# TurakhiaLab/TWILIGHT

Hardware: AMD Instinct MI355X
Metric: DP band cells/s, TALCO-XDrop progressive profile-profile alignment (bit-exact vs reference CPU path) (higher is better)
Workload: dtype f32

## Files before the change

### include/twl_align.h

```cpp
#ifndef TWL_ALIGN_H
#define TWL_ALIGN_H

#include <stdint.h>

#ifdef __cplusplus
extern "C" {
#endif

#define TWL_MAX_MATRIX 21
#define TWL_MAX_MARKER 1024

enum twl_status {
    TWL_OK = 0,
    TWL_ERR_NOT_INITIALIZED = -1,
    TWL_ERR_BAD_ARGUMENT = -2,
    TWL_ERR_HIP = -3,
    TWL_ERR_UNSUPPORTED = -4
};

typedef struct twl_params {
    int32_t P;
    float   matrix[TWL_MAX_MATRIX * TWL_MAX_MATRIX];
    float   gap_open;
    float   gap_extend;
    float   gap_boundary;
    float   gap_char;
    int32_t xdrop;
    int32_t flen;
    int32_t marker;
} twl_params;

typedef struct twl_stats {
    uint64_t band_cells;
    uint64_t nominal_cells;
    double   kernel_ms;
    double   pack_ms;
    double   total_ms;
    int32_t  n_launches;
    int32_t  n_relaunched;
    int32_t  window;
    int32_t  grid;
    int32_t  matrix_mode;
    int32_t  speculative;
    int32_t  mt_tiles_predicted;
    int32_t  mt_tiles_inline;
    int32_t  mt_scouts_failed;
    int32_t  reserved;
    char     kernel[160];
} twl_stats;

int  twl_init(const int *device_ids, int n_devices);
void twl_shutdown(void);
const char *twl_last_error(void);
const char *twl_version(void);

int twl_align_batch(const twl_params *p, int32_t n_pairs, int32_t seq_len,
                    const float *freq, const float *gap_open, const float *gap_extend,
                    const int32_t *len, const int32_t *num,
                    int8_t *aln_out, int32_t *aln_len_out, int16_t *err_out);

int twl_align_batch_device(int device, void *stream, const twl_params *p, int32_t n_pairs, int32_t seq_len,
                           const float *d_freq, const float *d_gap_open, const float *d_gap_extend,
                           const int32_t *d_len, const int32_t *d_num,
                           int8_t *d_aln_out, int32_t *d_aln_len_out, int16_t *d_err_out);

void *twl_host_alloc(uint64_t bytes);
void  twl_host_free(void *p);

int twl_copy_to_device(int device, void *dst_dev, const void *src, uint64_t bytes);
int twl_copy_from_device(int device, void *dst, const void *src_dev, uint64_t bytes);
int twl_copy_rows_from_device(int device, void *dst, uint64_t dst_pitch, const void *src_dev, uint64_t src_pitch, uint64_t width, uint64_t rows);

int twl_get_stats(int device, twl_stats *out);

int twl_get_pair_cells(int device, uint64_t *cells_out, int32_t n);

int twl_column_scores(const twl_params *p, int32_t seq_len, const float *freq, const int32_t *len, const int32_t *num, float *out);

int twl_dp_column_scores(const twl_params *p, int32_t seq_len, const float *freq, const float *gap_open, const float *gap_extend,
                         const int32_t *len, const int32_t *num, float *out);

#define TWL_MT_REC_WORDS 12
typedef struct twl_mt_dims {
    int32_t n_run, slots, sp_pitch, segcap;
    int32_t n_scout, n_tile, rounds;
    int32_t lead2, marg, anchors;
    int32_t thr, small_tiles, marker;
    int32_t reserved[3];
} twl_mt_dims;
int twl_mt_tables(int device, twl_mt_dims *dims, int32_t *order, int32_t *anchor, int32_t *spath, int32_t *chain, int32_t *rec, int8_t *seg, int32_t *front);

#define TWL_COMM_ID_BYTES 128
int twl_comm_unique_id(void *id128);
int twl_comm_init(int device, int rank, int world, const void *id128);
int twl_comm_all_gather(int device, const void *d_send, void *d_recv, int64_t bytes_per_rank);
int twl_comm_all_gather_host(int device, const void *send, void *recv, int64_t bytes_per_rank);
int twl_comm_destroy(int device);

enum twl_knob { TWL_KNOB_MT_PERTURB = 1, TWL_KNOB_MT_MAX_PAIRS = 2, TWL_KNOB_MT_MIN_MARKER = 3, TWL_KNOB_MT_LEAD = 4, TWL_KNOB_MT_MARGIN = 5,
                TWL_KNOB_MT_ROUNDS = 6, TWL_KNOB_MT_THR_JOBS = 7, TWL_KNOB_FAIL_ROW_ALLOCS = 8,
                TWL_KNOB_PROT_MODE = 9, TWL_KNOB_ASSUME_ONEHOT_QUERY = 10, TWL_KNOB_MT_TAIL_PCT = 11, TWL_KNOB_MT_WIDE = 12, TWL_KNOB_NO_SPEC = 13, TWL_KNOB_SCOUT_XDROP_PCT = 14, TWL_KNOB_THR_SMALL = 15, TWL_KNOB_FORCE_GLOBAL = 16, TWL_KNOB_LEAF_STEP = 17, TWL_KNOB_POISON_TB = 18, TWL_KNOB_MT_ANCHOR = 19, TWL_KNOB_MT_LEAD2 = 20, TWL_KNOB_PROT_CORRIDOR = 21 };
int twl_set_knob(int key, int value);
int twl_plan_describe(const twl_params *p, int32_t n_pairs, const int32_t *len, int32_t num_cu, int32_t qry_onehot, int32_t wide_streak, char *out, int32_t cap);

#ifdef __cplusplus
}
#endif
#endif
```

### twilight_amd/api.py

```python
from __future__ import annotations

import ctypes as C
import os

import numpy as np

_HERE = os.path.dirname(os.path.abspath(__file__))
LIB_PATH = os.environ.get("TWL_LIB") or os.path.join(_HERE, "libtwl_align.so")
TWL_MAX_MATRIX = 21

_lib = None


class TwlError(RuntimeError):
    pass


class TwlParams(C.Structure):
    _fields_ = [("P", C.c_int32), ("matrix", C.c_float * (TWL_MAX_MATRIX * TWL_MAX_MATRIX)), ("gap_open", C.c_float),
                ("gap_extend", C.c_float), ("gap_boundary", C.c_float), ("gap_char", C.c_float), ("xdrop", C.c_int32),
                ("flen", C.c_int32), ("marker", C.c_int32)]


class TwlStats(C.Structure):
# ... 44 lines not shown
        lib.twl_shutdown.restype = None
        lib.twl_set_knob.restype = C.c_int
        lib.twl_mt_tables.restype = C.c_int
        _lib = lib
    return _lib


def _check(rc):
    if rc != 0:
        raise TwlError(f"libtwl_align error {rc}: {load_library().twl_last_error().decode()}")


def make_params(matrix, *, gap_open=-50.0, gap_extend=-5.0, gap_boundary=None, gap_char=None, xdrop=None, flen=4096,
                marker=1024) -> TwlParams:
    m = np.asarray(matrix, dtype=np.float32)
    n = m.shape[0]
    p = TwlParams()
    p.P = n + 1
    flat = np.zeros(TWL_MAX_MATRIX * TWL_MAX_MATRIX, dtype=np.float32)
    flat[: n * n] = m.reshape(-1)
    p.matrix[:] = flat.tolist()
    p.gap_open = gap_open
    p.gap_extend = gap_extend
    p.gap_boundary = gap_extend if gap_boundary is None else gap_boundary
    p.gap_char = gap_extend if gap_char is None else gap_char
    p.xdrop = int(1000 * -gap_extend) if xdrop is None else int(xdrop)
    p.flen = flen
    p.marker = marker
    return p


def init(device_ids=None):
    lib = load_library()
    if device_ids is None:
        _check(lib.twl_init(None, 0))
    else:
        arr = (C.c_int * len(device_ids))(*device_ids)
        _check(lib.twl_init(arr, len(device_ids)))


def shutdown():
    load_library().twl_shutdown()


def _ptr(a, ty):
    return a.ctypes.data_as(C.POINTER(ty))


def align_batch(params: TwlParams, batch):
    lib = load_library()
    n, sl = batch.n_pairs, batch.seq_len
    freq = np.ascontiguousarray(batch.freq, dtype=np.float32)
    go = np.ascontiguousarray(batch.gap_open, dtype=np.float32)
    ge = np.ascontiguousarray(batch.gap_extend, dtype=np.float32)
    ln = np.ascontiguousarray(batch.len, dtype=np.int32)
    nm = np.ascontiguousarray(batch.num, dtype=np.int32)
    aln = np.zeros((n, 2 * sl), dtype=np.int8)
    aln_len = np.zeros(n, dtype=np.int32)
    err = np.zeros(n, dtype=np.int16)
    _check(lib.twl_align_batch(C.byref(params), C.c_int32(n), C.c_int32(sl), _ptr(freq, C.c_float), _ptr(go, C.c_float),
                               _ptr(ge, C.c_float), _ptr(ln, C.c_int32), _ptr(nm, C.c_int32), _ptr(aln, C.c_int8),
                               _ptr(aln_len, C.c_int32), _ptr(err, C.c_int16)))
    return aln, aln_len, err


def align_batch_device(params: TwlParams, n_pairs, seq_len, d_freq, d_gop, d_gex, d_len, d_num, d_aln, d_aln_len, d_err,
                       device=0, stream=None):
    lib = load_library()
    vp = C.c_void_p
    _check(lib.twl_align_batch_device(C.c_int(device), vp(stream or 0), C.byref(params), C.c_int32(n_pairs), C.c_int32(seq_len),
                                      vp(d_freq), vp(d_gop), vp(d_gex), vp(d_len), vp(d_num), vp(d_aln), vp(d_aln_len),
                                      vp(d_err)))


KNOB_MT_PERTURB, KNOB_MT_MAX_PAIRS, KNOB_MT_MIN_MARKER, KNOB_MT_LEAD, KNOB_MT_MARGIN, KNOB_MT_ROUNDS, KNOB_MT_THR_JOBS, KNOB_FAIL_ROW_ALLOCS = 1, 2, 3, 4, 5, 6, 7, 8
KNOB_PROT_MODE, KNOB_ASSUME_ONEHOT_QUERY, KNOB_MT_TAIL_PCT, KNOB_MT_WIDE, KNOB_NO_SPEC, KNOB_SCOUT_XDROP_PCT = 9, 10, 11, 12, 13, 14
KNOB_THR_SMALL = 15
KNOB_FORCE_GLOBAL = 16
KNOB_LEAF_STEP = 17
KNOB_POISON_TB = 18
KNOB_MT_ANCHOR = 19
KNOB_PROT_CORRIDOR = 21
KNOB_MT_LEAD2 = 20
PROT_MODES = {"auto": 0, "dense": 1, "sparse": 2, "presim": 3, "r1": 4, "lean_sparse": 5, "lean_presim": 6}


def set_knob(key: int, value: int):
    _check(load_library().twl_set_knob(C.c_int(key), C.c_int(value)))


def plan_describe(params, lens, num_cu=256, qry_onehot=False, wide_streak=0, small_state=0) -> str:
    wide_streak = int(wide_streak) + (100000 * (32 + int(small_state)) if small_state else 0)
    lens = np.ascontiguousarray(lens, dtype=np.int32)
    buf = C.create_string_buffer(256)
    _check(load_library().twl_plan_describe(C.byref(params), C.c_int32(lens.shape[0]), _ptr(lens, C.c_int32), C.c_int32(num_cu), C.c_int32(int(qry_onehot)), C.c_int32(wide_streak), buf, C.c_int32(256)))
    return buf.value.decode()


def version() -> str:
    return load_library().twl_version().decode()


def get_stats(device=0) -> TwlStats:
    st = TwlStats()
    _check(load_library().twl_get_stats(C.c_int(device), C.byref(st)))
    return st


def get_pair_cells(n, device=0):
    out = np.zeros(n, dtype=np.uint64)
    _check(load_library().twl_get_pair_cells(C.c_int(device), _ptr(out, C.c_uint64), C.c_int32(n)))
    return out


def column_scores(params: TwlParams, ref: np.ndarray, qry: np.ndarray, ref_num: int, qry_num: int) -> np.ndarray:
    ref = np.ascontiguousarray(ref, dtype=np.float32)
    qry = np.ascontiguousarray(qry, dtype=np.float32)
    R, Q, P = ref.shape[0], qry.shape[0], ref.shape[1]
    sl = max(R, Q)
    freq = np.zeros((2, sl, P), dtype=np.float32)
    freq[0, :R] = ref
    freq[1, :Q] = qry
    ln = np.array([R, Q], dtype=np.int32)
    nm = np.array([ref_num, qry_num], dtype=np.int32)
    out = np.zeros((Q, R), dtype=np.float32)
    _check(load_library().twl_column_scores(C.byref(params), C.c_int32(sl), _ptr(freq, C.c_float), _ptr(ln, C.c_int32), _ptr(nm, C.c_int32), _ptr(out, C.c_float)))
    return out


def dp_column_scores(params: TwlParams, batch, pair: int = 0) -> np.ndarray:
    sl = batch.seq_len
    freq = np.ascontiguousarray(batch.freq[pair], dtype=np.float32)
    gop = np.ascontiguousarray(batch.gap_open[pair], dtype=np.float32)
    gex = np.ascontiguousarray(batch.gap_extend[pair], dtype=np.float32)
    ln = np.ascontiguousarray(batch.len[pair], dtype=np.int32)
    nm = np.ascontiguousarray(batch.num[pair], dtype=np.int32)
    out = np.zeros((int(ln[1]), int(ln[0])), dtype=np.float32)
    _check(load_library().twl_dp_column_scores(C.byref(params), C.c_int32(sl), _ptr(freq, C.c_float), _ptr(gop, C.c_float), _ptr(gex, C.c_float),
                                               _ptr(ln, C.c_int32), _ptr(nm, C.c_int32), _ptr(out, C.c_float)))
    return out


def mt_tables(device=0) -> dict:
    lib = load_library()
    dm = TwlMtDims()
    _check(lib.twl_mt_tables(C.c_int(device), C.byref(dm), None, None, None, None, None, None, None))
    n, s = dm.n_run, dm.slots
    order = np.zeros(n, dtype=np.int32)
    anchor = np.zeros((n, s), dtype=np.int32) if dm.anchors else None
    spath = np.zeros((n, dm.sp_pitch), dtype=np.int32)
    chain = np.zeros((n, s, 2), dtype=np.int32)
    rec = np.zeros((n, s, MT_REC_WORDS), dtype=np.int32)
    seg = np.zeros((n, s, dm.segcap), dtype=np.int8)
    front = np.zeros((n, 8), dtype=np.int32)
    _check(lib.twl_mt_tables(C.c_int(device), C.byref(dm), _ptr(order, C.c_int32), _ptr(anchor, C.c_int32) if dm.anchors else None, _ptr(spath, C.c_int32),
                             _ptr(chain, C.c_int32), _ptr(rec, C.c_int32), _ptr(seg, C.c_int8), _ptr(front, C.c_int32)))
    assert (dm.n_run, dm.slots) == (n, s), "another level ran between the two reads"
    dims = {k: int(getattr(dm, k)) for k, _ in TwlMtDims._fields_ if k != "reserved"}
    return {"dims": dims, "order": order, "anchor": anchor, "spath": spath, "chain": chain, "rec": rec, "seg": seg, "front": front}
```

### twilight_amd/csrc/talco_kernel.hip.h

```cpp
#pragma once
#include <hip/hip_runtime.h>
#include <stdint.h>
#include "talco_exit.hip.h"

namespace twl {

constexpr int kIB = -2;
constexpr int kDB = -3;
constexpr int kMaxMarker = 1024;
constexpr int kErrOverflow = -1;
constexpr int kErrGuard = -2;

struct KArgs {
    const float *cols;
    const int32_t *len;
    const int32_t *num;
    int8_t *aln;
    int32_t *aln_len;
    int16_t *err;
    unsigned long long *cells;
    uint32_t *tb;
    int32_t *queue;
    const int32_t *items;
    int32_t n_items;
    int32_t seq_len;
    int32_t tb_words;
    int32_t *dbg;
    int32_t n_pairs_total;
    int32_t *hb;
    int32_t step_slack;
    float gap_open, gap_extend, gap_char;
    const uint8_t *gc_zero;
    int32_t xdrop, flen, marker;
    float M[441];
    const float *sim;
    const long long *sim_off;
};

#ifdef TWL_KERNEL_STAMPS
#define TWL_STAMP(var) const unsigned long long var = __builtin_amdgcn_s_memtime()
#else
#define TWL_STAMP(var)
#endif

#ifdef TWL_KERNEL_DEBUG
__device__ __forceinline__ void heartbeat(const KArgs &a, int slot, int v)
{
    if (a.hb && blockIdx.x == 0 && threadIdx.x == 0) __hip_atomic_store(&a.hb[slot], v, __ATOMIC_RELAXED, __HIP_MEMORY_SCOPE_SYSTEM);
}
#else
__device__ __forceinline__ void heartbeat(const KArgs &, int, int) {}
#endif

__device__ __forceinline__ unsigned lds_off(const void *p)
{
    return (unsigned)(uintptr_t)(__attribute__((address_space(3))) const void *)p;
}
__device__ __forceinline__ void lds_max_i32(int *p, int v) { asm volatile("ds_max_i32 %0, %1" ::"v"(lds_off(p)), "v"(v) : "memory"); }
__device__ __forceinline__ void lds_min_i32(int *p, int v) { asm volatile("ds_min_i32 %0, %1" ::"v"(lds_off(p)), "v"(v) : "memory"); }
__device__ __forceinline__ void lds_or_b32(int *p, int v) { asm volatile("ds_or_b32 %0, %1" ::"v"(lds_off(p)), "v"(v) : "memory"); }

__device__ __forceinline__ float dpp_shr1_f(float from_prev_wave, float src)
{
    return __int_as_float(__builtin_amdgcn_update_dpp(__float_as_int(from_prev_wave), __float_as_int(src), 0x138, 0xf, 0xf, false));
}
__device__ __forceinline__ int dpp_shr1_i(int from_prev_wave, int src)
{
    return __builtin_amdgcn_update_dpp(from_prev_wave, src, 0x138, 0xf, 0xf, false);
}

__device__ __forceinline__ float wave_max_f32(float x)
{
#define TWL_DPP_MAX(ctrl, rmask, bmask) \
    x = fmaxf(x, __int_as_float(__builtin_amdgcn_update_dpp(__float_as_int(x), __float_as_int(x), ctrl, rmask, bmask, false)))
    TWL_DPP_MAX(0x111, 0xf, 0xf);
    TWL_DPP_MAX(0x112, 0xf, 0xf);
    TWL_DPP_MAX(0x114, 0xf, 0xf);
    TWL_DPP_MAX(0x118, 0xf, 0xf);
    TWL_DPP_MAX(0x142, 0xa, 0xf);
    TWL_DPP_MAX(0x143, 0xc, 0xf);
#undef TWL_DPP_MAX
    return __int_as_float(__builtin_amdgcn_readlane(__float_as_int(x), 63));
}

__device__ __forceinline__ int f2key(float f)
{
    int b = __float_as_int(f);
    if (b == (int)0x80000000) b = 0;
    return b >= 0 ? b : (b ^ 0x7fffffff);
}
__device__ __forceinline__ float key2f(int k)
{
    return __int_as_float(k >= 0 ? k : (k ^ 0x7fffffff));
}

template <int P, int W, int RPL, bool PRE, bool REFLDS, bool QREG = true>
struct Cfg {
    static_assert(P == 6 || P == 22, "profile width");
    static_assert(!(PRE && P != 6), "precomputed q*M rows exist for P=6 only");
    static constexpr int CW = P + 2;
    static constexpr int F4 = CW / 4;
    static constexpr int NV = W * RPL;
    static constexpr int WINDOW = 64 * NV;
    static constexpr int NB = NV + 2;
    static constexpr int CAP = 64 * NB;
    static constexpr int RING_F4 = REFLDS ? CAP * F4 : F4;
    static constexpr int THREADS = 64 * W;
};

template <int P, int W, int RPL, bool PRE, bool REFLDS, bool QREG = true, int MINW = 1, int MM = 0>
__global__ __launch_bounds__(64 * W, MINW) void talco_kernel(KArgs a)
{
    using C = Cfg<P, W, RPL, PRE, REFLDS, QREG>;
    constexpr int NV = C::NV, WINDOW = C::WINDOW, NB = C::NB, CAP = C::CAP, CW = C::CW, F4 = C::F4;
    constexpr int MS = P - 1;
// ... 707 lines not shown
```

### twilight_amd/csrc/talco_nuc.hip.h

```cpp
#pragma once
#include "talco_kernel.hip.h"

#if defined(TWL_EXP_NOPRIO)
#define TWL_SETPRIO(x) do {} while (0)
#else
#define TWL_SETPRIO(x) __builtin_amdgcn_s_setprio(x)
#endif

namespace twl {

struct NArgs {
    const float *cols;
    const int32_t *len;
    const int32_t *num;
    int8_t *aln;
    int32_t *aln_len;
    int16_t *err;
    unsigned long long *cells;
    uint32_t *tb;
    int32_t *queue;
    const int32_t *items;
    int32_t n_items;
    int32_t seq_len;
    int32_t tb_words;
    int32_t *dbg;
    int32_t n_pairs_total;
    int32_t step_slack;
    float gap_open, gap_extend, gap_char;
    const uint8_t *gc_zero;
    int32_t xdrop, flen, marker;
    float M[25];
    const float *M24;
    const float *sim;
    const long long *sim_off;
    unsigned long long *team;
    float *simdump;
    const int32_t *mt_jobs;
    int32_t *mt_chain;
    int32_t *mt_rec;
    int8_t *mt_seg;
    int32_t *mt_spath;
    unsigned long long *mt_stat;
    int32_t *mt_front;
    int32_t mt_slots, mt_segcap, mt_sp_pitch, mt_lead, mt_marg;
    const int32_t *mt_anchor;
    int32_t mt_lead2;
    int32_t mt_inline;
};

typedef float nuc_f4 __attribute__((ext_vector_type(4)));
typedef float nuc_f2 __attribute__((ext_vector_type(2)));
__device__ __forceinline__ float4 lds_ld128(unsigned addr)
{
    const nuc_f4 v = *reinterpret_cast<const __attribute__((address_space(3))) nuc_f4 *>((const __attribute__((address_space(3))) char *)nullptr + addr);
    return make_float4(v.x, v.y, v.z, v.w);
}
typedef int nuc_i2 __attribute__((ext_vector_type(2)));
typedef int nuc_i4 __attribute__((ext_vector_type(4)));
template <class T>
__device__ __forceinline__ T lds_ld(unsigned addr)
{
    return *reinterpret_cast<const __attribute__((address_space(3))) T *>((const __attribute__((address_space(3))) char *)nullptr + addr);
}
template <class T>
__device__ __forceinline__ void lds_st(unsigned addr, T v)
{
    *reinterpret_cast<__attribute__((address_space(3))) T *>((__attribute__((address_space(3))) char *)nullptr + addr) = v;
}
template <int OFF>
__device__ __forceinline__ void lds_max_u32_off(unsigned addr, unsigned v) { asm volatile("ds_max_u32 %0, %1 offset:%2" ::"v"(addr), "v"(v), "n"(OFF) : "memory"); }
template <int OFF>
__device__ __forceinline__ void lds_max_f32_off(unsigned addr, float v) { asm volatile("ds_max_f32 %0, %1 offset:%2" ::"v"(addr), "v"(v), "n"(OFF) : "memory"); }
#define TWL_LDS_ATOM(NAME)                                                                                                     \
    template <int OFF>                                                                                                         \
    __device__ __forceinline__ void NAME##_off(unsigned addr, int v) { asm volatile(#NAME " %0, %1 offset:%2" ::"v"(addr), "v"(v), "n"(OFF) : "memory"); }
TWL_LDS_ATOM(ds_min_i32)
TWL_LDS_ATOM(ds_max_i32)
TWL_LDS_ATOM(ds_or_b32)
#undef TWL_LDS_ATOM
__device__ __forceinline__ void wg_barrier_lds() { asm volatile("s_waitcnt lgkmcnt(0)\n\ts_barrier" ::: "memory"); }
__device__ __forceinline__ void lds_max_u32(unsigned addr, unsigned v) { asm volatile("ds_max_u32 %0, %1" ::"v"(addr), "v"(v) : "memory"); }
__device__ __forceinline__ void lds_max_f32(unsigned addr, float v) { asm volatile("ds_max_f32 %0, %1" ::"v"(addr), "v"(v) : "memory"); }

__device__ __forceinline__ float fast_div(float n, float d, float r)
{
    const float q0 = n * r;
    const float t0 = __builtin_fmaf(-d, q0, n);
    const float q1 = __builtin_fmaf(t0, r, q0);
    const float t1 = __builtin_fmaf(-d, q1, n);
    return __builtin_fmaf(t1, r, q1);
}
__device__ __forceinline__ float refined_rcp(float d)
{
    const float r0 = __builtin_amdgcn_rcpf(d);
    const float e = __builtin_fmaf(-d, r0, 1.0f);
    return __builtin_fmaf(e, r0, r0);
}
__device__ __forceinline__ bool div_guard_bad(float x)
{
    const float ax = __builtin_fabsf(x);
    return (x != 0.0f) && !(ax >= 9.5367431640625e-07f && ax <= 1073741824.0f);
}

constexpr unsigned kTeamLast = 1u, kTeamErr = 2u;
constexpr int kTeamWords = 16, kTeamGuess = 0, kTeamTruth = 4, kTeamPos = 8, kTeamStat = 12;
__device__ __forceinline__ unsigned long long team_word(unsigned tag, unsigned flags, unsigned hi, unsigned lo)
{
    return ((unsigned long long)(tag & 0xFFFFu) << 48) | ((unsigned long long)(flags & 0xFFFFu) << 32) | ((unsigned long long)(hi & 0xFFFFu) << 16) | (lo & 0xFFFFu);
}
__device__ __forceinline__ unsigned long long team_load(const unsigned long long *p) { return __hip_atomic_load(p, __ATOMIC_RELAXED, __HIP_MEMORY_SCOPE_AGENT); }
__device__ __forceinline__ void team_store(unsigned long long *p, unsigned long long v) { __hip_atomic_store(p, v, __ATOMIC_RELAXED, __HIP_MEMORY_SCOPE_AGENT); }
__device__ __forceinline__ unsigned long long team_wait(const unsigned long long *p, unsigned tag, const unsigned long long *alt = nullptr)
{
    for (int spin = 0; spin < (1 << 21); ++spin) {
        const unsigned long long v = team_load(p);
        if ((unsigned)(v >> 48) == tag) return v;
        if (alt) { const unsigned long long u = team_load(alt); if ((unsigned)(u >> 48) == tag) return u | (1ull << 47); }
        __builtin_amdgcn_s_sleep(16);
    }
    return 0ull;
}
__device__ __forceinline__ unsigned score_key(float f)
{
    const unsigned b = (unsigned)__float_as_int(f);
    return (b & 0x80000000u) ? ~b : (b | 0x80000000u);
}

constexpr int kMtRec = 12;

__global__ void mt_chain_kernel(const int32_t *spath, int sp_pitch, const int32_t *len, const int32_t *items, int n_items, int32_t *chain, int slots,
                                int marker, int perturb, const int32_t *front)
{
    const int it = blockIdx.x * blockDim.x + threadIdx.x;
    if (it >= n_items) return;
// ... 35 lines not shown
    q = min(q, Q - 1);
    r = d0 - q;
    if (r > R - 1) { r = R - 1; q = d0 - r; }
    return !(q > Q - 1 || r < 0);
}
__device__ __forceinline__ bool scout_anchor(const int32_t *an, int slot, int slots, int &o)
{
    const int w = __builtin_amdgcn_readfirstlane(an[slot]);
    if (w >= 0) { o = w - 128; return true; }
    int l = -1, r = -1, ol = 0, orr = 0;
    for (int u = 1; u <= kAnchorNear; ++u) {
        if (l < 0 && slot - u >= 1) { const int v = __builtin_amdgcn_readfirstlane(an[slot - u]); if (v >= 0) { l = slot - u; ol = v - 128; } }
        if (r < 0 && slot + u < slots) { const int v = __builtin_amdgcn_readfirstlane(an[slot + u]); if (v >= 0) { r = slot + u; orr = v - 128; } }
    }
    if (l < 0 || r < 0 || abs(orr - ol) > kAnchorJump * (r - l)) return false;
    o = ol + (orr - ol) * (slot - l) / (r - l);
    return true;
}
__device__ __forceinline__ bool scout_anchored_cell(int d0, int R, int Q, int o, int &r, int &q)
{
    int r0, q0;
    if (!scout_line_cell(d0, R, Q, r0, q0)) return false;
    q = q0 + (o >= 0 ? (o + 1) / 2 : -((-o + 1) / 2));
    r = d0 - q;
    if (q < 0) { q = 0; r = d0; }
    if (r < 0) { r = 0; q = d0; }
    return q < Q && r < R;
}

constexpr int kAnchorShift = 24, kAnchorShifts = 4, kAnchorPad = kAnchorShift * kAnchorShifts;
template <int P>
__global__ __launch_bounds__(256) void mt_anchor_kernel(const float *cols, const int32_t *len, int seq_len, const int32_t *jobs, int n_jobs, int32_t *anchor, int slots, int marker, int lead2)
{
    static_assert(kAnchorOffsets == 256 && 2 * kAnchorHalf + 2 * kAnchorPad == 256, "one thread per offset, one per staged reference letter");
    __shared__ unsigned char s_r[2 * kAnchorHalf + 2 * kAnchorPad], s_q[2 * kAnchorHalf + 2 * kAnchorPad + kAnchorOffsets];
    __shared__ int s_cnt[kAnchorOffsets], s_done;
    const int job = blockIdx.x;
    if (job >= n_jobs) return;
    const int pair = jobs[3 * job], slot = jobs[3 * job + 1], row = jobs[3 * job + 2];
    const int R = len[2 * pair], Q = len[2 * pair + 1];
    const int spLo = (marker - 1) * slot - 1;
    const int d0 = max(spLo - lead2, 0);
    int r0, q0;
    if (spLo > R + Q - 2 || R < 2 || Q < 2 || !scout_line_cell(d0, R, Q, r0, q0)) return;
    auto letter = [&](int side, int col, int n) -> unsigned char {
        if (col < 0 || col >= n) return (unsigned char)(100 + side);
        const float *pf = cols + (((size_t)pair * 2 + side) * (size_t)seq_len + col) * (P + 2);
        int best = 0; float bc = pf[0];
        for (int j = 1; j < P - 2; ++j) if (pf[j] > bc) { bc = pf[j]; best = j; }
        return (bc > 0.0f && bc >= pf[P - 1]) ? (unsigned char)best : (unsigned char)(100 + side);
    };
    const int t = threadIdx.x;
    s_r[t] = letter(0, r0 - kAnchorHalf - kAnchorPad + t, R);
    for (int u = t; u < 2 * kAnchorHalf + 2 * kAnchorPad + kAnchorOffsets; u += 256) s_q[u] = letter(1, q0 - kAnchorHalf - kAnchorPad - kAnchorOffsets / 2 + u, Q);
    if (t == 0) s_done = 0;
    __syncthreads();
    for (int sh = 0; sh <= 2 * kAnchorShifts; ++sh) {
        const int base = kAnchorPad + ((sh == 0) ? 0 : ((sh & 1) ? kAnchorShift * ((sh + 1) / 2) : -kAnchorShift * (sh / 2)));
        int c = 0;
        for (int i = 0; i < 2 * kAnchorHalf; ++i) c += (s_r[base + i] == s_q[base + i + t]) ? 1 : 0;
        s_cnt[t] = c;
        __syncthreads();
        if (t < 64) {
            int key = -1;
            for (int u = t; u < kAnchorOffsets; u += 64) {
                const int o = u - kAnchorOffsets / 2;
                const int rank = (o == 0) ? 0 : (o < 0 ? -2 * o - 1 : 2 * o);
                key = max(key, (s_cnt[u] << 16) | (0xFFFF - rank));
            }
            for (int m = 32; m >= 1; m >>= 1) key = max(key, __shfl_xor(key, m, 64));
            const int rank = 0xFFFF - (key & 0xFFFF);
            const int bo = (rank == 0) ? 0 : ((rank & 1) ? -(rank + 1) / 2 : rank / 2);
            int second = -1;
            for (int u = t; u < kAnchorOffsets; u += 64) if (abs(u - kAnchorOffsets / 2 - bo) > 2) second = max(second, s_cnt[u]);
            for (int m = 32; m >= 1; m >>= 1) second = max(second, __shfl_xor(second, m, 64));
            const int bc = key >> 16;
            if (t == 0 && bc >= kAnchorMinMatches && bc - second >= kAnchorMinGap) { anchor[(size_t)row * slots + slot] = 128 + bo; s_done = 1; }
        }
        __syncthreads();
        if (s_done) break;
    }
}

template <int W, int RPL>
struct NCfg {
    static constexpr int NV = W * RPL;
    static constexpr int WINDOW = 64 * NV;
    static constexpr int NB = NV + 2;
    static constexpr int CAP = 64 * NB;
    static constexpr int THREADS = 64 * W;
};

template <int P, int W, int RPL, int MM, int MINW, bool SPEC = false, bool DUMP = false, int MT = 0, int SP = 0>
__global__ __launch_bounds__(64 * W, MINW) void talco_lean_kernel(NArgs a)
{
    static_assert(SP == 0 || (SP == 1 && P == 6 && !SPEC && !DUMP && MM == 5), "the leaf x leaf step: nucleotide, one-letter query rows");
    static_assert((P == 6 && ((MM >= 0 && MM <= 2) || MM == 5)) || (P == 22 && (MM == 3 || MM == 4)), "profile width / column-score mode");
    static_assert(MT == 0 || (!SPEC && !DUMP), "the tile-parallel kernels are plain ones");
    constexpr bool GUESS = SPEC || MT == 2;
    using C = NCfg<W, RPL>;
    constexpr int NV = C::NV, WINDOW = C::WINDOW, NB = C::NB, CAP = C::CAP;
    constexpr int NQP = (MM == 2 || MM == 1) ? 8 : (MM == 0 ? 10 : (MM == 5 ? 2 : 1));
    constexpr int NQM = (MM == 0) ? 5 : 1;
#if defined(TWL_EXP_QPRE)
    constexpr bool QPRE = !(MM == 2) || TWL_EXP_QPRE;
#else
    constexpr bool QPRE = !((RPL >= 3 || MINW >= 5) && MM == 2);
#endif
    constexpr int F4 = (P + 2) / 4;
    constexpr bool SPARSE = (MM == 3), PRESIM = (MM == 4);
    constexpr int RP = PRESIM ? 1 : F4;
    constexpr int QN = PRESIM ? 1 : P;

    __shared__ float4 s_ring[RP * CAP];
    __shared__ uint32_t s_rmask[SPARSE ? CAP : 1];
    __shared__ float4 s_M4[SPARSE ? 21 * 6 : 1];
    struct ParBuf {
        int cd[WINDOW + 4];
        int4 exch[NV];
        unsigned red[4];
        int conv[4];
        int edge[2 * NV];
        int4 trash[64];
    };
    __shared__ ParBuf s_par[2];
    __shared__ int s_misc[8];
    __shared__ int8_t s_rev[2 * kMaxMarker + 16];
    __shared__ unsigned long long s_team[4];
    constexpr unsigned O_CD = (unsigned)offsetof(ParBuf, cd), O_EXCH = (unsigned)offsetof(ParBuf, exch), O_RED = (unsigned)offsetof(ParBuf, red),
                       O_CONV = (unsigned)offsetof(ParBuf, conv), O_TRASH = (unsigned)offsetof(ParBuf, trash), O_EDGE = (unsigned)offsetof(ParBuf, edge);

    const int lane = threadIdx.x & 63;
    const int w = __builtin_amdgcn_readfirstlane(threadIdx.x >> 6);
    uint32_t *tb = a.tb + (size_t)blockIdx.x * (size_t)a.tb_words;
    const float inf = (float)(2.0 * (double)a.xdrop + 1.0);
    const float xdropf = __int_as_float(__builtin_amdgcn_readfirstlane(__float_as_int((float)a.xdrop)));
    if constexpr (SPARSE) {
        for (int t = threadIdx.x; t < 21 * 6; t += C::THREADS) s_M4[t] = reinterpret_cast<const float4 *>(a.M24)[t];
    }

    int specRound = 0;
    for (;;) {
        int item;
        if constexpr (SPEC) {
            if (specRound++) break;
            item = (int)(blockIdx.x >> 1);
            __syncthreads();
        } else {
            if (threadIdx.x == 0) s_misc[0] = atomicAdd(a.queue, 1);
            __syncthreads();
            item = __builtin_amdgcn_readfirstlane(s_misc[0]);
        }
        if (item >= a.n_items) break;
        const int pair = __builtin_amdgcn_readfirstlane((MT == 1 || MT == 2) ? a.mt_jobs[3 * item] : a.items[item]);
        const int slot = (MT == 1 || MT == 2) ? __builtin_amdgcn_readfirstlane(a.mt_jobs[3 * item + 1]) : 0;
        const int mtx = (MT == 1 || MT == 2) ? __builtin_amdgcn_readfirstlane(a.mt_jobs[3 * item + 2]) : item;
        const int R = a.len[2 * pair], Q = a.len[2 * pair + 1];
        const float gc = (a.gc_zero && __builtin_amdgcn_readfirstlane((int)a.gc_zero[pair])) ? 0.0f : a.gap_char;
        const bool gcNZ = (gc != 0.0f);
        const unsigned long long gcMask = gcNZ ? ~0ull : 0ull;
        const int spLo = (a.marker - 1) * slot - 1, spHi = a.marker * slot + 1;
        int anchRef = -1, anchQry = -1;
        bool anchored = false;
        if constexpr (MT == 2) {
            if (a.mt_anchor && !(spLo > R + Q - 2 || R < 2 || Q < 2)) {
                int o = 0;
                if (scout_anchor(a.mt_anchor + (size_t)mtx * a.mt_slots, slot, a.mt_slots, o)) anchored = scout_anchored_cell(max(spLo - a.mt_lead2, 0), R, Q, o, anchRef, anchQry);
            }
        }
        const int scoutD0 = max(spLo - (anchored ? a.mt_lead2 : a.mt_lead), 0);
        const int marker = (MT == 2) ? min(spHi + a.mt_marg - scoutD0, kMaxMarker) : ((MT == 4) ? R + Q + 8 : a.marker);
        const float denom = (float)a.num[2 * pair] * (float)a.num[2 * pair + 1];
        const bool denomOne = (denom == 1.0f);
        const float rden = refined_rcp(denom);
        const float4 *colsR = reinterpret_cast<const float4 *>(a.cols + ((size_t)pair * 2 + 0) * (size_t)a.seq_len * (P + 2));
        const float4 *colsQ = reinterpret_cast<const float4 *>(a.cols + ((size_t)pair * 2 + 1) * (size_t)a.seq_len * (P + 2));
        const float *simP = PRESIM ? a.sim + a.sim_off[pair] : nullptr;
        const int simPitch = (Q + 63) & ~63;

        int ref_idx = 0, qry_idx = 0, tile = 0, pos = 0, err = 0;
        bool last_tile = (R <= 0 || Q <= 0);
        if constexpr (MT == 1) {
            if (slot > 0) {
                ref_idx = __builtin_amdgcn_readfirstlane(a.mt_chain[((size_t)mtx * a.mt_slots + slot) * 2]);
                qry_idx = __builtin_amdgcn_readfirstlane(a.mt_chain[((size_t)mtx * a.mt_slots + slot) * 2 + 1]);
                tile = 1;
                if (ref_idx < 0) last_tile = true;
            }
            const int32_t *fr = a.mt_front + (size_t)mtx * 8;
            const int fs = __builtin_amdgcn_readfirstlane(fr[0]), ft = __builtin_amdgcn_readfirstlane(fr[1]);
            const int32_t *rc = a.mt_rec + ((size_t)mtx * a.mt_slots + slot) * kMtRec;
            const int rv = __builtin_amdgcn_readfirstlane(rc[0]), rr = __builtin_amdgcn_readfirstlane(rc[1]), rq = __builtin_amdgcn_readfirstlane(rc[2]);
            if (fs == 2 || (fs == 1 && slot < ft) || (rv == 1 && rr == ref_idx && rq == qry_idx)) last_tile = true;
        }
        if constexpr (MT == 2) {
            tile = 1;
            if (spLo > R + Q - 2 || R < 2 || Q < 2) last_tile = true;
            else if (anchored) { ref_idx = anchRef; qry_idx = anchQry; }
            else if (!scout_line_cell(scoutD0, R, Q, ref_idx, qry_idx)) last_tile = true;
        }
        if constexpr (MT == 4) {
            if (R < 2 || Q < 2 || R + Q > 65000 || (size_t)(((R + Q) >> 3) + 2) * (size_t)WINDOW > (size_t)a.tb_words) last_tile = true;
        }
        const int jobRef = ref_idx, jobQry = qry_idx;
        int mtHits = 0, mtInline = 0;
        bool suspended = false, mtSkip = false;
        unsigned long long mtCells0 = 0;
        if constexpr (MT == 3) {
            const int32_t *fr = a.mt_front + (size_t)mtx * 8;
            const int fs = __builtin_amdgcn_readfirstlane(fr[0]);
            if (fs == 2) { mtSkip = true; last_tile = true; }
            else if (fs == 1) {
                tile = __builtin_amdgcn_readfirstlane(fr[1]); ref_idx = __builtin_amdgcn_readfirstlane(fr[2]); qry_idx = __builtin_amdgcn_readfirstlane(fr[3]);
                pos = __builtin_amdgcn_readfirstlane(fr[4]);
                mtCells0 = (unsigned long long)(unsigned)__builtin_amdgcn_readfirstlane(fr[6]) | ((unsigned long long)(unsigned)__builtin_amdgcn_readfirstlane(fr[7]) << 32);
            }
        }
        int8_t *out = (MT == 1) ? a.mt_seg + ((size_t)mtx * a.mt_slots + slot) * (size_t)a.mt_segcap : a.aln + (size_t)pair * 2 * (size_t)a.seq_len;
        unsigned long long cells = 0;
        long long steps_left = (long long)(R + Q + 2) * ((R + Q) / (max(marker, 2) - 1) + 4) + a.step_slack;
        if (SP == 1 && !last_tile && !denomOne) { err = kErrGuard; last_tile = true; }
        if (!last_tile && ((SPEC && (R > 65535 || Q > 65535)) || !(denom >= 1.0f && denom <= 1.0995116e12f))) { err = (denom >= 1.0f && denom <= 1.0995116e12f) ? kErrOverflow : kErrGuard; last_tile = true; }
        int dbg_lastk = 0, dbg_conv = 0, dbg_L = 0, dbg_U = 0;
        bool guardBad = false;
        unsigned long long *team = SPEC ? a.team + (size_t)item * kTeamWords : nullptr;
        const int role = SPEC ? (int)(blockIdx.x & 1) : 0;
        bool confirmed = true, teamExit = false, redo = false, iEnded = false, timedOut = false;
        if constexpr (SPEC) tile = role;
        auto bcast = [&](unsigned long long v) __attribute__((always_inline)) -> unsigned long long {
            if (threadIdx.x == 0) s_team[0] = v;
            __syncthreads();
            const unsigned long long r = s_team[0];
            __syncthreads();
            return (unsigned long long)__builtin_amdgcn_readfirstlane((int)(r & 0xFFFFFFFFu)) | ((unsigned long long)(unsigned)__builtin_amdgcn_readfirstlane((int)(r >> 32)) << 32);
        };
        auto settle = [&]() __attribute__((always_inline)) -> int {
            unsigned long long v = 0ull;
            if (threadIdx.x == 0) v = team_wait(&team[kTeamTruth + (tile & 3)], (unsigned)(tile + 1));
            v = bcast(v);
            if (v == 0ull) { err = kErrOverflow; timedOut = true; return 2; }
            const unsigned fl = (unsigned)(v >> 32) & 0xFFFFu;
            if (fl & (kTeamLast | kTeamErr)) return 2;
            const int tr = (int)((v >> 16) & 0xFFFFu), tq = (int)(v & 0xFFFFu);
            if (tr == ref_idx && tq == qry_idx) { if (threadIdx.x == 0) atomicAdd(&team[kTeamStat + 1], 1ull); return 0; }
            ref_idx = tr; qry_idx = tq;
            return 1;
        };
#ifdef TWL_KERNEL_STAMPS
        unsigned long long st_slots = 0, st_bar = 0, st_post = 0, st_n = 0, st_act = 0, st_exit = 0, st_setup = 0;
        const unsigned long long st_t0 = __builtin_amdgcn_s_memtime();
#endif

        while (!last_tile) {
#ifdef TWL_KERNEL_STAMPS
            const unsigned long long st_tile0 = __builtin_amdgcn_s_memtime();
#endif
            if constexpr (SPEC) {
                if (!redo && tile > 0) {
                    unsigned long long v = 0ull;
                    if (threadIdx.x == 0) v = team_wait(&team[kTeamTruth + (tile & 3)], (unsigned)(tile + 1), &team[kTeamGuess + (tile & 3)]);
                    v = bcast(v);
                    const unsigned fl = (unsigned)(v >> 32) & 0x7FFFu;
                    if (v == 0ull) { err = kErrOverflow; timedOut = true; teamExit = true; }
                    else if (!(v & (1ull << 47)) && (fl & (kTeamLast | kTeamErr))) teamExit = true;
                    else { ref_idx = (int)((v >> 16) & 0xFFFFu); qry_idx = (int)(v & 0xFFFFu); confirmed = !(v & (1ull << 47)); }
                }
                redo = false;
                if (teamExit) { last_tile = true; }
            }
            bool memoHit = false;
            if constexpr (MT == 3) {
                if (tile < a.mt_slots) {
                    const int32_t *rc = a.mt_rec + ((size_t)mtx * a.mt_slots + tile) * kMtRec;
                    const int rcValid = __builtin_amdgcn_readfirstlane(rc[0]), rcRef = __builtin_amdgcn_readfirstlane(rc[1]), rcQry = __builtin_amdgcn_readfirstlane(rc[2]);
                    memoHit = (rcValid == 1 && rcRef == ref_idx && rcQry == qry_idx);
                    if (rcValid == 2 && rcRef == ref_idx && rcQry == qry_idx && !(__builtin_amdgcn_readfirstlane(rc[10]) == kErrOverflow && __builtin_amdgcn_readfirstlane(rc[11]) < WINDOW)) {
                        err = __builtin_amdgcn_readfirstlane(rc[10]); if (err == 0) err = 3;
                        cells += (unsigned long long)(unsigned)__builtin_amdgcn_readfirstlane(rc[9]);
                    }
                    if (memoHit) {
                        const int cnt = __builtin_amdgcn_readfirstlane(rc[6]), tailDir = __builtin_amdgcn_readfirstlane(rc[7]), tailLen = __builtin_amdgcn_readfirstlane(rc[8]);
                        if (pos + cnt + tailLen > 2 * a.seq_len) err = 3;
                        else {
                            const int8_t *sg = a.mt_seg + ((size_t)mtx * a.mt_slots + tile) * (size_t)a.mt_segcap;
                            for (int t = threadIdx.x; t < cnt; t += C::THREADS) out[pos + t] = sg[t];
                            for (int t = threadIdx.x; t < tailLen; t += C::THREADS) out[pos + cnt + t] = (int8_t)tailDir;
                            pos += cnt + tailLen;
                            ref_idx = __builtin_amdgcn_readfirstlane(rc[3]); qry_idx = __builtin_amdgcn_readfirstlane(rc[4]);
                            last_tile = __builtin_amdgcn_readfirstlane(rc[5]) != 0;
                            cells += (unsigned long long)(unsigned)__builtin_amdgcn_readfirstlane(rc[9]);
                            mtHits += 1;
                            tile += 1;
                        }
                    }
                }
                if (err != 0) break;
                if (!memoHit && !a.mt_inline) { suspended = true; break; }
                if (!memoHit) mtInline += 1;
            }
            if (!(SPEC && teamExit) && !memoHit) {
            const int refLen = R - ref_idx, qLen = Q - qry_idx;
            const int fLen = min(a.flen, min(refLen, qLen));
            const int fcap = min(fLen, 64 * (NV - 2));
            float vmA = a.M[0], vmB = a.M[2], vmC = a.M[1];
            asm volatile("" : "+v"(vmA), "+v"(vmB), "+v"(vmC));
            float S1[RPL], I1[RPL], D1[RPL], LS2[RPL];
            int CS1[RPL], CI1[RPL], CD1[RPL], LCS2[RPL];
            float qv[RPL][QN], gopq[RPL], gexq[RPL], qM[RPL][NQM];
            nuc_f2 qP[QPRE ? RPL : 1][NQP];
            float simNext[RPL];
            int simFor[RPL];
            const int simK0 = ref_idx + qry_idx;
            int b0[RPL];
            unsigned ra[RPL];
            uint32_t tbacc[RPL];
            bool q5any[RPL];

            auto load_q = [&](int r) __attribute__((always_inline)) {
                const int i = b0[r] + lane;
                const bool ok = qry_idx + i < Q;
                if constexpr (PRESIM) {
                    float4 c = make_float4(0.f, 0.f, 0.f, 0.f);
                    if (ok) c = colsQ[F4 * (size_t)(qry_idx + i) + (F4 - 1)];
                    gopq[r] = c.z; gexq[r] = c.w;
                    q5any[r] = false;
                    simFor[r] = -1;
                } else {
                    float cb[4 * F4];
#pragma unroll
                    for (int t = 0; t < F4; ++t) {
                        float4 c = make_float4(0.f, 0.f, 0.f, 0.f);
                        if (ok) c = colsQ[F4 * (size_t)(qry_idx + i) + t];
                        cb[4 * t] = c.x; cb[4 * t + 1] = c.y; cb[4 * t + 2] = c.z; cb[4 * t + 3] = c.w;
                    }
#pragma unroll
                    for (int t = 0; t < P; ++t) qv[r][t] = cb[t];
                    gopq[r] = cb[P]; gexq[r] = cb[P + 1];
                    if constexpr (MM == 2 && !QPRE) {}
                    else if constexpr (MM == 2) {
                        const float mA = a.M[0], mB = a.M[2], mC = a.M[1];
#pragma unroll
                        for (int m = 0; m < 4; ++m)
#pragma unroll
                            for (int h = 0; h < 2; ++h) {
                                const int l0 = 2 * h, l1 = 2 * h + 1;
                                qP[r][2 * m + h] = nuc_f2{qv[r][m] * ((l0 == m) ? mA : (((l0 ^ m) == 2) ? mB : mC)), qv[r][m] * ((l1 == m) ? mA : (((l1 ^ m) == 2) ? mB : mC))};
                            }
                    } else if constexpr (MM == 1) {
#pragma unroll
                        for (int m = 0; m < 4; ++m)
#pragma unroll
                            for (int h = 0; h < 2; ++h) qP[r][2 * m + h] = nuc_f2{qv[r][m] * a.M[5 * (2 * h) + m], qv[r][m] * a.M[5 * (2 * h + 1) + m]};
                    } else if constexpr (MM == 5) {
                        float qT[4];
#pragma unroll
                        for (int l = 0; l < 4; ++l) qT[l] = ((qv[r][0] * a.M[5 * l + 0] + qv[r][1] * a.M[5 * l + 1]) + qv[r][2] * a.M[5 * l + 2]) + qv[r][3] * a.M[5 * l + 3];
                        qP[r][0] = nuc_f2{qT[0], qT[1]};
                        qP[r][1] = nuc_f2{qT[2], qT[3]};
                    } else if constexpr (MM == 0) {
#pragma unroll
                        for (int m = 0; m < 5; ++m) {
#pragma unroll
                            for (int h = 0; h < 2; ++h) qP[r][2 * m + h] = nuc_f2{qv[r][m] * a.M[5 * (2 * h) + m], qv[r][m] * a.M[5 * (2 * h + 1) + m]};
                            qM[r][m] = qv[r][m] * a.M[20 + m];
                        }
                    }
                    if constexpr (SP == 1) q5any[r] = false;
                    else q5any[r] = gcNZ && __builtin_amdgcn_ballot_w64(cb[P - 1] != 0.0f) != 0ull;
                    bool bad = false;
                    if constexpr (SP == 1) bad = (cb[P - 1] != 0.0f);
#pragma unroll
                    for (int t = 0; t < P; ++t) bad = bad | div_guard_bad(cb[t]);
                    guardBad = guardBad | (__builtin_amdgcn_ballot_w64(bad) != 0ull);
                }
            };
            auto load_ring_block = [&](int B) __attribute__((always_inline)) {
                const int col = 64 * B + lane;
                const int slot = (B % NB) * 64 + lane;
                const bool ok = col < refLen;
                if constexpr (PRESIM) {
                    float4 c = make_float4(0.f, 0.f, 0.f, 0.f);
                    if (ok) c = colsR[F4 * (size_t)(ref_idx + col) + (F4 - 1)];
                    s_ring[slot] = c;
                } else {
                    bool bad = false;
                    uint32_t mk = 0;
#pragma unroll
                    for (int t = 0; t < F4; ++t) {
                        float4 c = make_float4(0.f, 0.f, 0.f, 0.f);
                        if (ok) c = colsR[F4 * (size_t)(ref_idx + col) + t];
                        s_ring[t * CAP + slot] = c;
                        const float f[4] = {c.x, c.y, c.z, c.w};
#pragma unroll
                        for (int u = 0; u < 4; ++u) {
                            if (4 * t + u < P) bad = bad | div_guard_bad(f[u]);
                            if (SP == 1 && 4 * t + u == P - 1) bad = bad | (f[u] != 0.0f);
                            if (SPARSE && 4 * t + u < 21) mk |= (f[u] != 0.0f) ? (1u << (4 * t + u)) : 0u;
                        }
                    }
                    if constexpr (SPARSE) s_rmask[slot] = mk;
                    guardBad = guardBad | (__builtin_amdgcn_ballot_w64(bad) != 0ull);
                }
            };
            auto ring_addr = [&](int r, int k) __attribute__((always_inline)) {
                int rs = (k - b0[r] - lane) % CAP;
                rs += (rs < 0) ? CAP : 0;
                ra[r] = (unsigned)rs * 16u + lds_off(s_ring);
            };

#pragma unroll
            for (int r = 0; r < RPL; ++r) {
                b0[r] = 64 * (r * W + w);
                ring_addr(r, 0);
                tbacc[r] = 0;
                S1[r] = I1[r] = D1[r] = LS2[r] = -1.0f;
                load_q(r);
            }
            int hiBlk = 1;
            if (w == 0 % W) load_ring_block(0);
            if (w == 1 % W) load_ring_block(1);
            for (int t = threadIdx.x; t < WINDOW + 4; t += C::THREADS) { s_par[0].cd[t] = kDB; s_par[1].cd[t] = kDB; }
            if (threadIdx.x == 0) {
                s_par[0].red[0] = s_par[1].red[0] = (unsigned)__float_as_int(-inf);
                s_par[0].red[1] = s_par[0].red[2] = s_par[1].red[1] = s_par[1].red[2] = 0u;
                for (int t = 0; t < 2; ++t) { s_par[t].conv[0] = 0x7fffffff; s_par[t].conv[1] = (int)0x80000000; s_par[t].conv[2] = 0; }
                s_team[1] = 0ull; s_team[2] = 0ull; s_team[3] = 0ull;
                s_misc[4] = 0;
            }
            __syncthreads();

            int vL = 0, vU = 0, vlo1 = 0x3fffffff, vlo2p = 0x3fffffff;
            unsigned vw1 = 0, vw2 = 0;
            int vwid1 = 0;
            unsigned vcells = 0;
            int Lk = 0, Wk = 0, Lm63 = -63, W64 = 64;
            int kStop = 0;
            int kHook = 8;
            float msp = -inf, convf = 0.0f;
            bool converged = false;
            int conv_value = 0, prev_conv_s = -1;
            const int kEnd = refLen + qLen - 1;
            int k = 0;
            int tile_err = 0;
            bool go = true, conv_logic = false, aborted = false;
            bool spec = true;
            bool tbPending = false;
            unsigned tbOff = (unsigned)lane * 4u;
            int tbL0 = 0, tbU0 = 0;
            unsigned tbMust = 0u;
            constexpr unsigned PARX = (unsigned)sizeof(ParBuf);
            unsigned vcur = lds_off(&s_par[0]), vprev = lds_off(&s_par[1]);
            const unsigned parx = lds_off(&s_par[0]) ^ lds_off(&s_par[1]);
            (void)PARX;
            const unsigned relTrashRed = O_TRASH + (unsigned)lane * 4u - O_RED;
            unsigned mbRel[RPL], exRel[RPL];
#pragma unroll
            for (int r = 0; r < RPL; ++r) {
                const int vw = r * W + w;
                mbRel[r] = (lane == 63) ? O_EXCH + 16u * (unsigned)vw : O_TRASH + (unsigned)lane * 16u;
                exRel[r] = O_EXCH + 16u * (unsigned)((vw + NV - 1) % NV);
            }

            auto stop_tile = [&]() __attribute__((always_inline)) { go = false; kStop = (int)0x80000000; };
            auto hook = [&](auto PHtag) __attribute__((always_inline)) {
                constexpr int PH = decltype(PHtag)::value;
                constexpr bool TB = (PH != 2);
                const int Uk = Lk + Wk;
                if constexpr (TB) {
#pragma unroll
                    for (int r = 0; r < RPL; ++r) {
                        const int bb = b0[r];
#if defined(TWL_TB_ALWAYS)
                        (void)bb;
#else
                        if (((tbMust >> r) & 1u) != 0u || (bb + 63 >= tbL0 && bb <= tbU0 + 8))
#endif
                            *reinterpret_cast<uint32_t *>(reinterpret_cast<char *>(tb) + tbOff + (unsigned)(256 * (r * W + w))) = tbacc[r];
                        tbacc[r] = 0;
                    }
                    tbMust = 0u; tbL0 = Lk; tbU0 = Uk;
                    tbOff += (unsigned)WINDOW * 4u;
                    tbPending = false;
                }
                const int need_hi = ((k + 10 - Lk) >> 6) + 1;
                if (hiBlk < need_hi) { ++hiBlk; if (w == hiBlk % W) load_ring_block(hiBlk); }
            };
            auto step = [&](auto PHtag, auto GENtag) __attribute__((always_inline)) {
                constexpr int PH = decltype(PHtag)::value;
                constexpr bool GEN = decltype(GENtag)::value;
                constexpr bool TB = (PH != 2), CONV = (PH != 0);
                asm volatile("; TWL_STEP PH=%c0 GEN=%c1 (a comment: tools/isa_block_step.py finds the diagonal loops by it)" ::"n"(PH), "n"((int)GEN));
                TWL_STAMP(t_head);
#if defined(TWL_EXP_SALU)
                { int xs = k; 
#pragma unroll
                  for (int t = 0; t < 24; ++t) asm volatile("s_add_u32 %0, %0, 1" : "+s"(xs));
                  asm volatile("" :: "s"(xs)); }
#elif defined(TWL_EXP_VALU)
                { int xv = lane;
#pragma unroll
                  for (int t = 0; t < 24; ++t) asm volatile("v_add_u32 %0, %0, 1" : "+v"(xv));
                  asm volatile("" :: "v"(xv)); }
#endif
                const unsigned kk16 = (unsigned)(k + 1) << 16;
                const unsigned vwidth1 = (unsigned)(vU - vL);
                vcells += vwidth1 + 1u;
                float thr;
                { const float m0 = __int_as_float(max(__float_as_int(msp), 0)); asm("v_subrev_f32_e32 %0, %1, %2" : "=v"(thr) : "s"(xdropf), "v"(m0)); }
                bool special = false;
                if constexpr (GEN) {
                    if (__builtin_expect(spec, 0)) {
                        special = (k == 0) | ((tile == 0) && (Lk == 0 || Lk + Wk == k));
                        spec = special;
                    }
                }
                int staleCD = kDB;
                if constexpr (PH == 2) staleCD = lds_ld<int>(vprev + 4u * (unsigned)vwid1 + O_CD);
                const unsigned vTrashRed = vcur + relTrashRed;

#pragma unroll
                for (int r = 0; r < RPL; ++r) {
                    const int b = b0[r];
                    const int u = b - Lm63;
                    if ((unsigned)u <= (unsigned)W64) {
                        if constexpr (MT == 0 && RPL >= 2) { if (r == 0) TWL_SETPRIO(2); else TWL_SETPRIO(3); }
                        else TWL_SETPRIO(2);
                        const int i = b + lane;
                        float eS, eI; int eCS = 0, eCI = 0;
                        if constexpr (CONV) {
                            const nuc_i4 e = lds_ld<nuc_i4>(vprev + exRel[r]);
                            eS = __int_as_float(e.x); eI = __int_as_float(e.y); eCS = e.z; eCI = e.w;
                        } else {
                            const nuc_i2 e = lds_ld<nuc_i2>(vprev + exRel[r]);
                            eS = __int_as_float(e.x); eI = __int_as_float(e.y);
                        }
                        const bool inband = (unsigned)(i - vL) <= vwidth1;
                        float numer = 0.0f, rg, gopr, gexr;
                        if constexpr (P == 6) {
                            const float4 c0 = lds_ld128(ra[r]);
                            const float4 c1 = lds_ld128(ra[r] + CAP * 16);
                            const float rc[5] = {c0.x, c0.y, c0.z, c0.w, c1.x};
                            rg = c1.y; gopr = c1.z; gexr = c1.w;
                            constexpr int NM = (MM == 0) ? 5 : (MM == 5 ? 1 : 4);
                            const nuc_f2 r01 = nuc_f2{c0.x, c0.y}, r23 = nuc_f2{c0.z, c0.w};
                            nuc_f2 s01, s23;
                            if constexpr (QPRE) {
                                s01 = qP[r][0] * r01; s23 = qP[r][1] * r23;
#pragma unroll
                                for (int m = 1; m < NM; ++m) { s01 = s01 + qP[r][2 * m] * r01; s23 = s23 + qP[r][2 * m + 1] * r23; }
#if defined(TWL_EXP_PACKED_SCORE)
                            } else if constexpr (true) {
                                const float mA = a.M[0], mB = a.M[2], mC = a.M[1];
                                auto fp = [&](int m, int h) __attribute__((always_inline)) {
                                    const int l0 = 2 * h, l1 = 2 * h + 1;
                                    return nuc_f2{qv[r][m] * ((l0 == m) ? mA : (((l0 ^ m) == 2) ? mB : mC)), qv[r][m] * ((l1 == m) ? mA : (((l1 ^ m) == 2) ? mB : mC))};
                                };
                                s01 = fp(0, 0) * r01; s23 = fp(0, 1) * r23;
#pragma unroll
                                for (int m = 1; m < 4; ++m) { s01 = s01 + fp(m, 0) * r01; s23 = s23 + fp(m, 1) * r23; }
#endif
                            } else {
                                auto mv = [&](int l, int m) __attribute__((always_inline)) { return (l == m) ? vmA : (((l ^ m) == 2) ? vmB : vmC); };
                                float sl[4];
#pragma unroll
                                for (int l = 0; l < 4; ++l) {
                                    sl[l] = (qv[r][0] * mv(l, 0)) * rc[l];
#pragma unroll
                                    for (int m = 1; m < 4; ++m) sl[l] = sl[l] + (qv[r][m] * mv(l, m)) * rc[l];
                                }
                                s01 = nuc_f2{sl[0], sl[1]}; s23 = nuc_f2{sl[2], sl[3]};
                            }
                            numer = ((s01.x + s01.y) + s23.x) + s23.y;
                            if constexpr (MM == 0) {
                                float s4 = qM[r][0] * rc[4];
#pragma unroll
                                for (int m = 1; m < 5; ++m) s4 = s4 + qM[r][m] * rc[4];
                                numer = numer + s4;
                            }
                            if (q5any[r]) {
#pragma unroll
                                for (int l = 0; l < 5; ++l) numer += (rc[l] * qv[r][5]) * gc;
                            }
                            bool rgAny;
                            if constexpr (SP == 1) rgAny = false;
                            else rgAny = (__builtin_amdgcn_ballot_w64(inband) & __builtin_amdgcn_ballot_w64(rg != 0.0f) & gcMask) != 0ull;
                            if (rgAny) {
#pragma unroll
                                for (int m = 0; m < 5; ++m) numer += (rg * qv[r][m]) * gc;
                            }
                        } else if constexpr (SPARSE) {
                            const float4 cl = lds_ld128(ra[r] + (F4 - 1) * CAP * 16);
                            rg = cl.y; gopr = cl.z; gexr = cl.w;
                            const unsigned slotOff = ra[r] - lds_off(s_ring);
                            const uint32_t rmask = inband ? lds_ld<uint32_t>(lds_off(s_rmask) + (slotOff >> 2)) : 0u;
                            uint32_t mk = rmask;
                            while (__builtin_amdgcn_ballot_w64(mk != 0u) != 0ull) {
                                if (mk != 0u) {
                                    const int l = __builtin_ctz(mk);
                                    mk &= mk - 1u;
                                    const float rl = lds_ld<float>(ra[r] + (unsigned)(l >> 2) * (CAP * 16) + (unsigned)(l & 3) * 4u);
                                    float Mr[24];
#pragma unroll
                                    for (int t = 0; t < 6; ++t) {
                                        const float4 c = s_M4[l * 6 + t];
                                        Mr[4 * t] = c.x; Mr[4 * t + 1] = c.y; Mr[4 * t + 2] = c.z; Mr[4 * t + 3] = c.w;
                                    }
#pragma unroll
                                    for (int m = 16; m < 21; ++m) numer += (rl * qv[r][m]) * Mr[m];
                                    float v[8];
#pragma unroll
                                    for (int t = 0; t < 8; ++t) v[t] = (qv[r][t] * Mr[t]) * rl + (qv[r][8 + t] * Mr[8 + t]) * rl;
                                    numer += ((((((v[0] + v[1]) + v[2]) + v[3]) + v[4]) + v[5]) + v[6]) + v[7];
                                }
                            }
                            if (q5any[r]) {
                                mk = rmask;
                                while (__builtin_amdgcn_ballot_w64(mk != 0u) != 0ull) {
                                    if (mk != 0u) {
                                        const int l = __builtin_ctz(mk);
                                        mk &= mk - 1u;
                                        numer += (lds_ld<float>(ra[r] + (unsigned)(l >> 2) * (CAP * 16) + (unsigned)(l & 3) * 4u) * qv[r][P - 1]) * gc;
                                    }
                                }
                            }
                            if ((__builtin_amdgcn_ballot_w64(inband) & __builtin_amdgcn_ballot_w64(rg != 0.0f)) != 0ull) {
#pragma unroll
                                for (int m = 0; m < P - 1; ++m) numer += (rg * qv[r][m]) * gc;
                            }
                        } else {
                            const float4 cl = lds_ld128(ra[r]);
                            rg = cl.y; gopr = cl.z; gexr = cl.w;
                            (void)rg;
                        }
                        float sim = numer;
                        if constexpr (PRESIM) {
                            const size_t col = (size_t)(qry_idx + i);
                            const bool colOk = (qry_idx + i) < simPitch;
                            if (simFor[r] == k) sim = simNext[r];
                            else sim = colOk ? simP[(size_t)(k + simK0) * (size_t)simPitch + col] : 0.0f;
                            simNext[r] = (colOk && k + 1 < kEnd) ? simP[(size_t)(k + 1 + simK0) * (size_t)simPitch + col] : 0.0f;
                            simFor[r] = k + 1;
                            guardBad = guardBad | (__builtin_amdgcn_ballot_w64(inband && sim != sim) != 0ull);
                        } else if (SP == 0 && !denomOne) {
                            sim = fast_div(numer, denom, rden);
                            asm volatile("" : "+v"(sim));
                        }

                        if constexpr (DUMP) {
                            if (inband) a.simdump[(size_t)(qry_idx + i) * (size_t)R + (size_t)(ref_idx + k - i)] = sim;
                        }
                        const float LS1 = dpp_shr1_f(eS, S1[r]);
                        const float LI1 = dpp_shr1_f(eI, I1[r]);
                        int LCS1 = 0, LCI1 = 0;
                        if constexpr (CONV) { LCS1 = dpp_shr1_i(eCS, CS1[r]); LCI1 = dpp_shr1_i(eCI, CI1[r]); }
                        const unsigned t1 = (unsigned)(i - vlo1);
                        const bool up_ok = t1 <= vw1;
                        const bool left_ok = (t1 - 1u) <= vw1;
                        const bool diag_ok = (unsigned)(i - vlo2p) <= vw2;
                        float match = diag_ok ? LS2[r] + sim : -inf;
                        if (__builtin_expect(special, 0)) {
                            const int j = k - i;
                            if (k == 0) match = sim;
                            else if (i == 0 || j == 0) {
                                int far = max(i, j) - 1; far = far < 0 ? 0 : far;
                                match = (sim + a.gap_open) + a.gap_extend * (float)far;
                            }
                        }
                        const float delOp = S1[r] + gopr, delExt = D1[r] + gexr;
                        const float insOp = LS1 + gopq[r], insExt = LI1 + gexq[r];
                        const bool dGE = delExt >= delOp, iGE = insExt >= insOp;
                        const bool Dptr = !up_ok | dGE;
                        const bool Iptr = !left_ok | iGE;
                        const float Dv = up_ok ? (dGE ? delExt : delOp) : -inf;
                        const float Iv = left_ok ? (iGE ? insExt : insOp) : -inf;
                        const bool gapIsI = Iv > Dv;
                        const float Gv = gapIsI ? Iv : Dv;
                        const bool isM = match >= Gv;
                        float Sv = isM ? match : Gv;
                        Sv = (Sv < thr) ? -inf : Sv;

                        if constexpr (CONV) {
                            int CSn, CIn, CDn;
                            const int i16 = i & 0xFFFF;
                            if (PH == 1 && k == marker - 1) { CSn = (3 << 16) | i16; CIn = CI1[r]; CDn = CD1[r]; }
                            else if (PH == 1) { CSn = i16; CIn = (1 << 16) | i16; CDn = (2 << 16) | i16; }
                            else {
                                const int viaS = (LCS1 != -1) ? LCS1 : kIB;
                                CIn = left_ok ? (Iptr ? LCI1 : viaS) : kIB;
                                const int cdUp = up_ok ? CD1[r] : staleCD;
                                CDn = Dptr ? cdUp : ((CS1[r] != -1) ? CS1[r] : kDB);
                                const int viaGap = gapIsI ? CIn : CDn;
                                CSn = isM ? (diag_ok ? LCS2[r] : -1) : viaGap;
                            }
                            CS1[r] = CSn; CI1[r] = CIn; CD1[r] = CDn;
                            if (PH == 2 || k == marker) { if (inband) lds_st<int>(vcur + 4u * (unsigned)(i - vL) + O_CD, CDn); }
                        }
                        S1[r] = Sv; I1[r] = Iv; D1[r] = Dv;
                        if constexpr (GUESS && PH == 1) {
                            if (inband && Sv > -inf) {
                                const unsigned long long key = ((unsigned long long)score_key(Sv) << 32) | (unsigned)i;
                                asm volatile("ds_max_u64 %0, %1" ::"v"(lds_off(&s_team[(k == marker) ? 3 : 2])), "v"(key) : "memory");
                            }
                        }
                        const float Sin = inband ? Sv : -inf;
                        lds_max_f32_off<O_RED>((Sin > msp) ? vcur : vTrashRed, Sin);
                        const unsigned long long vm = __builtin_amdgcn_ballot_w64(Sin > -inf);
                        const int below = (int)__builtin_amdgcn_mbcnt_hi((unsigned)(vm >> 32), __builtin_amdgcn_mbcnt_lo((unsigned)vm, 0u));
                        const int rank = (Sin > -inf) ? below : -2;
                        const int nValid1 = (int)__builtin_popcountll(vm) - 1;
                        lds_max_u32_off<O_RED + 4>((rank == 0) ? vcur : vTrashRed, kk16 + (0xFFFFu - (unsigned)i));
                        lds_max_u32_off<O_RED + 8>((rank == nValid1) ? vcur : vTrashRed, kk16 + (unsigned)i);
                        if constexpr (CONV) lds_st<nuc_i4>(vcur + mbRel[r], nuc_i4{__float_as_int(Sv), __float_as_int(Iv), CS1[r], CI1[r]});
                        else lds_st<nuc_i2>(vcur + mbRel[r], nuc_i2{__float_as_int(Sv), __float_as_int(Iv)});
                        if constexpr (PH == 2) {
                            const unsigned trashE = vcur + O_TRASH + (unsigned)lane * 16u + 8u;
                            lds_st<int>((rank == 0) ? vcur + O_EDGE + 8u * (unsigned)(r * W + w) : trashE, CS1[r]);
                            lds_st<int>((rank == nValid1) ? vcur + O_EDGE + 8u * (unsigned)(r * W + w) + 4u : trashE + 4u, CS1[r]);
                        }
                        if constexpr (TB) {
                            const uint32_t nib = (isM ? 0u : (gapIsI ? 1u : 2u)) | (Iptr ? 4u : 0u) | (Dptr ? 8u : 0u);
                            tbacc[r] |= nib << (4 * (k & 7));
                        }
                        LS2[r] = LS1;
                        if constexpr (CONV) LCS2[r] = LCS1;
                    }
                    if (__builtin_expect(u < 0, 0)) {
                        while (b0[r] + 63 < Lk) b0[r] += 64 * NV;
                        ring_addr(r, k);
                        load_q(r);
                        tbMust |= 1u << r;
                    }
                    ra[r] += 16u;
                    if (ra[r] == lds_off(s_ring) + CAP * 16u) ra[r] = lds_off(s_ring);
                }
                if constexpr (TB) tbPending = true;
                TWL_STAMP(t_slots);
                TWL_SETPRIO(0);
                wg_barrier_lds();
                if constexpr (W == 16) {
                    bool anyBlk = false;
#pragma unroll
                    for (int r = 0; r < RPL; ++r) anyBlk |= ((unsigned)(b0[r] - Lm63) <= (unsigned)W64);
                    if (anyBlk) TWL_SETPRIO(2);
                }
                TWL_STAMP(t_bar);

                const nuc_i4 rd = lds_ld<nuc_i4>(vcur + O_RED);
                { const float g = __int_as_float(rd.x); msp = (g > msp) ? g : msp; }
                const int newL = (int)((kk16 + 0xFFFFu) - (unsigned)rd.y);
                const int newU = (int)((unsigned)rd.z - kk16);

                if constexpr (CONV) {
                    if (!converged && k < kEnd - 1) {
                        int conv_S = -1;
                        bool all3 = false;
                        if constexpr (PH == 1) {
                            const int sL = __builtin_amdgcn_readfirstlane(newL), sU = __builtin_amdgcn_readfirstlane(newU);
                            if (k == marker - 1) conv_S = (sL == sU) ? ((3 << 16) | (sL & 0xFFFF)) : -1;
                            else conv_S = (sL == sU) ? (sL & 0xFFFF) : -1;
                        } else {
                            if (threadIdx.x == 0) {
                                int c0 = 0x7fffffff, c1 = (int)0x80000000, c2 = 0;
                                asm volatile("" : "+v"(c0), "+v"(c1), "+v"(c2));
                                lds_st<nuc_i4>(vprev + O_CONV, nuc_i4{c0, c1, c2, c2});
                            }
                            const int cLo = lds_ld<int>(vcur + O_EDGE + 8u * (((unsigned)newL >> 6) % (unsigned)NV));
                            const int cHi = lds_ld<int>(vcur + O_EDGE + 8u * (((unsigned)newU >> 6) % (unsigned)NV) + 4u);
                            const bool maybe = __builtin_amdgcn_ballot_w64(newL <= newU && cLo == cHi) != 0ull;
                            if (maybe) {
                            const unsigned cw = (unsigned)(newU - newL);
#pragma unroll
                            for (int r = 0; r < RPL; ++r) {
                                const int i = b0[r] + lane;
                                const bool inr = (unsigned)(i - newL) <= cw;
                                const unsigned long long rm = __builtin_amdgcn_ballot_w64(inr);
                                if (rm) {
                                    const int fl = (int)__builtin_ctzll(rm);
                                    const int v = __builtin_amdgcn_readlane(CS1[r], fl);
                                    const bool badS = __builtin_amdgcn_ballot_w64(inr && CS1[r] != v) != 0ull;
                                    const bool badID = __builtin_amdgcn_ballot_w64(inr && (CI1[r] != v || CD1[r] != v)) != 0ull;
                                    if (lane == 0) {
                                        ds_min_i32_off<O_CONV>(vcur, v);
                                        ds_max_i32_off<O_CONV + 4>(vcur, v);
                                        if (badS || badID) ds_or_b32_off<O_CONV + 8>(vcur, (badS ? 1 : 0) | (badID ? 2 : 0));
                                    }
                                }
                            }
                            wg_barrier_lds();
                            const nuc_i4 cv = lds_ld<nuc_i4>(vcur + O_CONV);
                            const int vmin = __builtin_amdgcn_readfirstlane(cv.x);
                            const int vmax = __builtin_amdgcn_readfirstlane(cv.y);
                            const int fl = __builtin_amdgcn_readfirstlane(cv.z);
                            if (vmin == vmax && !(fl & 1)) { conv_S = vmin; all3 = !(fl & 2); }
                            }
                        }
                        if (all3 && prev_conv_s == conv_S && conv_S != -1) { converged = true; conv_value = prev_conv_s; convf = msp; }
                        prev_conv_s = conv_S;
                    }
                }
                {
                    vlo2p = vlo1 + 1; vw2 = vw1;
                    vlo1 = vL; vw1 = vwidth1; vwid1 = (int)vwidth1 + 1;
                    vL = max(max(newL, k + 2 - refLen), 0);
                    vU = min(newU + 1, qLen - 1);
                    Lk = __builtin_amdgcn_readfirstlane(vL);
                    Wk = __builtin_amdgcn_readfirstlane(vU - vL);
                    Lm63 = Lk - 63; W64 = Wk + 64;
                    vcur ^= parx; vprev ^= parx;
                }
#ifdef TWL_KERNEL_STAMPS
                {
                    const unsigned long long t_end = __builtin_amdgcn_s_memtime();
                    st_slots += t_slots - t_head; st_bar += t_bar - t_slots; st_post += t_end - t_bar; st_n += 1;
                    st_act += (b0[0] <= Lk + Wk + 1 && b0[0] + 63 >= Lk) ? 1 : 0;
                    const int tlw = (k >= 600 && k < 696) ? k - 600 : ((k >= a.marker + 100 && k < a.marker + 196) ? 96 + k - a.marker - 100 : -1);
                    if (a.dbg && pair == 0 && tile == 4 && tlw >= 0 && lane == 0) {
                        long long *g = reinterpret_cast<long long *>(a.dbg + 16 * (size_t)a.n_pairs_total) + 256 + ((size_t)w * 192 + tlw) * 4;
                        g[0] = (long long)t_head; g[1] = (long long)t_slots; g[2] = (long long)t_bar; g[3] = (long long)t_end;
                    }
                }
#endif
                bool ended = false;
                if constexpr (CONV) {
                    if (converged) {
                        if (__builtin_amdgcn_ballot_w64(__int_as_float(max(__float_as_int(msp), 0)) > convf) != 0ull) { conv_logic = true; stop_tile(); ended = true; }
                    }
                }
                if (!ended) {
                    ++k;
                    if (k == kHook || (PH == 1 && k == marker + 1)) { hook(PHtag); kHook = (k & ~7) + 8; }
                    if (__builtin_expect((unsigned)Wk >= (unsigned)fcap, 0)) {
                        const int Uk = Lk + Wk;
                        if (k >= kEnd) {}
                        else if (Lk > Uk) { tile_err = 1; stop_tile(); }
                        else if (Uk - Lk + 1 > fLen) { tile_err = 2; stop_tile(); }
                        else if ((Uk >> 6) - (Lk >> 6) >= NV) { tile_err = kErrOverflow; stop_tile(); }
                        else {
#pragma unroll
                            for (int r = 0; r < RPL; ++r)
                                if (b0[r] + 63 < Lk) { while (b0[r] + 63 < Lk) b0[r] += 64 * NV; ring_addr(r, k); load_q(r); tbMust |= 1u << r; }
                        }
                    }
                }
            };

            if (steps_left < 0) { tile_err = 3; go = false; }
#ifdef TWL_KERNEL_STAMPS
            st_setup += __builtin_amdgcn_s_memtime() - st_tile0;
#endif
            {
                using T0 = std::integral_constant<int, 0>; using T1 = std::integral_constant<int, 1>; using T2 = std::integral_constant<int, 2>;
                auto run = [&](auto PHtag, int kLim) __attribute__((always_inline)) {
                    constexpr int PH = decltype(PHtag)::value;
                    if constexpr (PH == 1) { while (go && k < kLim) step(PHtag, std::true_type{}); }
                    else {
                        while (go && spec && k < kLim) step(PHtag, std::true_type{});
                        kStop = go ? kLim : (int)0x80000000;
                        while (k < kStop) step(PHtag, std::false_type{});
                    }
                };
                const int kA = min(kEnd, marker - 1);
                auto poll = [&]() __attribute__((always_inline)) {
                    if (threadIdx.x == 0) {
                        const unsigned long long pv = team_load(&team[kTeamTruth + (tile & 3)]);
                        unsigned long long d = 0ull;
                        if ((unsigned)(pv >> 48) == (unsigned)(tile + 1)) {
                            const unsigned fl = (unsigned)(pv >> 32) & 0xFFFFu;
                            d = ((fl & (kTeamLast | kTeamErr)) || (int)((pv >> 16) & 0xFFFFu) != ref_idx || (int)(pv & 0xFFFFu) != qry_idx) ? 2ull : 1ull;
                        }
                        s_team[1] = d;
                        if (d == 1ull) atomicAdd(&team[kTeamStat + 1], 1ull);
                    }
                    __syncthreads();
                    const int d = __builtin_amdgcn_readfirstlane((int)s_team[1]);
                    __syncthreads();
                    confirmed = confirmed | (d == 1);
                    go = go & (d != 2);
                    aborted = aborted | (d == 2);
                };
                if constexpr (SPEC) {
                    while (go && k < kA) {
                        const int kc = confirmed ? kA : min(kA, (k | 31) + 1);
                        run(T0{}, kc);
                        if (go && !confirmed) poll();
                    }
                } else run(T0{}, kA);
                const int kB = min(kEnd, marker + 1);
#pragma unroll
                for (int r = 0; r < RPL; ++r) { CS1[r] = -1; CI1[r] = kIB; CD1[r] = kDB; LCS2[r] = -1; }
                int sres = -1;
                if constexpr (SPEC) {
                    if (go && !confirmed && k < kB) {
                        sres = settle();
                        if (sres == 0) confirmed = true; else { go = false; aborted = true; }
                    }
                }
                run(T1{}, kB);
                if constexpr (SPEC) {
                    if (go && k == marker + 1 && k < kEnd) {
                        if (threadIdx.x == 0) {
                            const unsigned long long b0 = s_team[2], b1 = s_team[3];
                            const bool onMarker = (unsigned)(b1 >> 32) >= (unsigned)(b0 >> 32);
                            const int gq = (int)((onMarker ? b1 : b0) & 0xFFFFFFFFu), gr = (onMarker ? marker : marker - 1) - gq;
#ifdef TWL_SPEC_DEBUG
                            printf("tile %d start %d %d: best(marker-1) key %x row %d, best(marker) key %x row %d -> guess +%d +%d\n", tile, ref_idx, qry_idx, (unsigned)(b0 >> 32), (int)(b0 & 0xFFFFFFFFu), (unsigned)(b1 >> 32), (int)(b1 & 0xFFFFFFFFu), gr, gq);
#endif
                            if ((b0 | b1) != 0ull && gr >= 0 && ref_idx + gr < 65536 && qry_idx + gq < 65536) {
                                team_store(&team[kTeamGuess + ((tile + 1) & 3)], team_word((unsigned)(tile + 2), 0u, (unsigned)(ref_idx + gr), (unsigned)(qry_idx + gq)));
                                atomicAdd(&team[kTeamStat + 0], 1ull);
                            }
                        }
                    }
                }
                if constexpr (MT == 2) {
                    if (go && k == marker + 1 && k < kEnd) {
                        const unsigned long long b0 = s_team[2], b1 = s_team[3];
                        const unsigned k0 = (unsigned)__builtin_amdgcn_readfirstlane((int)(b0 >> 32)), k1 = (unsigned)__builtin_amdgcn_readfirstlane((int)(b1 >> 32));
                        const int i0 = __builtin_amdgcn_readfirstlane((int)(b0 & 0xFFFFFFFFu)), i1 = __builtin_amdgcn_readfirstlane((int)(b1 & 0xFFFFFFFFu));
                        if ((k0 | k1) != 0u) { conv_value = (k1 >= k0) ? (i1 & 0xFFFF) : ((3 << 16) | (i0 & 0xFFFF)); conv_logic = true; }
                        else tile_err = 1;
                        go = false;
                    }
                }
                const int kCap = min(kEnd, 65534);
                run(T2{}, kCap);
                if (go && k < kEnd) { tile_err = kErrOverflow; go = false; }
                if constexpr (SPEC) {
                    if (aborted || !confirmed) {
                        if (sres < 0 || sres == 0) sres = settle();
                        if (sres == 1) { redo = true; confirmed = true; }
                        else if (sres == 2) { teamExit = true; last_tile = true; }
                        else confirmed = true;
                    } else sres = 0;
                    aborted = (sres != 0);
                }
            }
#ifdef TWL_KERNEL_STAMPS
            const unsigned long long st_exit0 = __builtin_amdgcn_s_memtime();
#endif
            if (!(SPEC && aborted)) {
            const int last_k = conv_logic ? k : k - 1;
            steps_left -= (long long)(last_k + 1);
            const unsigned tile_cells = (unsigned)__builtin_amdgcn_readfirstlane((int)vcells);
            const int lo1 = __builtin_amdgcn_readfirstlane(vlo1);

            cells += tile_cells;
            dbg_lastk = last_k; dbg_conv = conv_value; dbg_L = Lk; dbg_U = Lk + Wk;
            if (tile_err != 0) { err = tile_err; break; }
            if (PRESIM || SP == 1 || !denomOne) {
                if (guardBad) s_misc[4] = 1;
                __syncthreads();
                guardBad = __builtin_amdgcn_readfirstlane(s_misc[4]) != 0;
                if (guardBad) { err = kErrGuard; break; }
            }

            if (tbPending) {
#pragma unroll
                for (int r = 0; r < RPL; ++r)
                    *reinterpret_cast<uint32_t *>(reinterpret_cast<char *>(tb) + tbOff + (unsigned)(256 * (r * W + w))) = tbacc[r];
            }

            int conv_q = 0, conv_r = 0, tb_state = 0, start_k = 0;
            bool bad = false;
            if (!conv_logic && last_k >= marker) {
                const int Llast = lo1;
#pragma unroll
                for (int r = 0; r < RPL; ++r) {
                    const int b = b0[r];
                    if (Llast >= b && Llast <= b + 63 && lane == Llast - b) s_misc[1] = CS1[r];
                }
                __syncthreads();
                conv_value = __builtin_amdgcn_readfirstlane(s_misc[1]);
            }
            if (conv_logic || last_k >= marker) {
                conv_q = conv_value & 0xFFFF;
                tb_state = (conv_value >> 16) & 0xFFFF;
                if (tb_state > 3) bad = true;
                else {
                    conv_r = marker - conv_q - ((tb_state == 3) ? 1 : 0);
                    start_k = (tb_state == 3) ? marker - 1 : marker;
                    if (conv_r < 0) bad = true;
                }
            } else {
                conv_q = qLen - 1; conv_r = refLen - 1; start_k = last_k; tb_state = 0; last_tile = true;
            }
            if (bad) { err = 3; break; }
#ifdef TWL_SPEC_DEBUG
            if (threadIdx.x == 0) printf("tile %d start %d %d: true +%d +%d state %d last_k %d conv_logic %d\n", tile, ref_idx, qry_idx, conv_r, conv_q, tb_state, last_k, (int)conv_logic);
#endif
            ref_idx += conv_r; qry_idx += conv_q;
            if (R - ref_idx < 0 || Q - qry_idx < 0) { err = 3; break; }
            int tailDir = 0, tailLen = 0;
            if (ref_idx == R - 1 && qry_idx < Q - 1) { tailDir = 1; tailLen = Q - qry_idx - 1; last_tile = true; }
            if (qry_idx == Q - 1 && ref_idx < R - 1) { tailDir = 2; tailLen = R - ref_idx - 1; last_tile = true; }
            if (ref_idx == R - 1 && qry_idx == Q - 1) last_tile = true;
            if constexpr (SPEC) {
                if (threadIdx.x == 0)
                    team_store(&team[kTeamTruth + ((tile + 1) & 3)], team_word((unsigned)(tile + 2), last_tile ? kTeamLast : 0u, (unsigned)ref_idx, (unsigned)qry_idx));
            }

            __syncthreads();
            if (w == 0) {
                if constexpr (SPEC) {
                    if (tile > 0) {
                        unsigned long long pv = 0ull;
                        if (lane == 0) pv = team_wait(&team[kTeamPos + (tile & 3)], (unsigned)(tile + 1));
                        pos = __builtin_amdgcn_readfirstlane((int)(pv & 0xFFFFFFFFu));
                        if (__builtin_amdgcn_readfirstlane((int)(pv >> 32)) == 0) { err = kErrOverflow; timedOut = true; }
                    }
                }
                int n = 0;
                {
                    constexpr int PG = 16;
                    static_assert(sizeof(s_ring) >= PG * 64 * sizeof(uint32_t), "traceback patch lives in the ring");
                    uint32_t *s_patch = reinterpret_cast<uint32_t *>(s_ring);
                    int kk2 = start_k, ii = conv_q, qi = conv_q, ri = conv_r, st = tb_state % 3;
                    const bool first = (tile == 0);
                    bool done = (kk2 < 0), walkBad = false;
                    while (!done) {
                        const int g0 = kk2 >> 3, i0 = ii;
                        const int row = i0 - 63 + lane;
#pragma unroll
                        for (int t = 0; t < PG; ++t) {
                            uint32_t word = 0u;
                            if (g0 - t >= 0 && row >= 0)
                                word = __hip_atomic_load(&tb[(size_t)(g0 - t) * WINDOW + (size_t)((unsigned)row % (unsigned)WINDOW)], __ATOMIC_RELAXED, __HIP_MEMORY_SCOPE_AGENT);
                            s_patch[t * 64 + lane] = word;
                        }
                        asm volatile("s_waitcnt lgkmcnt(0)" ::: "memory");
                        if (lane == 0) {
// ... 148 lines not shown
```

### twilight_amd/csrc/twl_align.hip

```cpp
#include "../../include/twl_align.h"
#include "../../include/twl_level.h"
#include "../../include/twl_place.h"
#include "../../include/twl_merge.h"
#include "../../include/twl_subtree.h"
#include "../../include/twl_guide.h"
#include "../../include/twl_retree.h"
#include "level_kernels.hip.h"
#include "restore_kernels.hip.h"
#include "place_kernels.hip.h"
#include "merge_kernels.hip.h"
#include "subtree_kernels.hip.h"
#include "guide_kernels.hip.h"
#include "retree_kernels.hip.h"
#include "talco_kernel.hip.h"
#include "talco_nuc.hip.h"
#include "talco_global.hip.h"

#include <hip/hip_runtime.h>
#include <dlfcn.h>

#include <algorithm>
#include <atomic>
#include <chrono>
#include <cmath>
// ... 11 lines not shown
struct FillJob { void *p; unsigned long long bytes; unsigned int val; };
struct FillArgs { FillJob j[8]; int n; };
__global__ void __launch_bounds__(256) fill_kernel(FillArgs a)
{
    const size_t t = (size_t)blockIdx.x * 256 + threadIdx.x, nt = (size_t)gridDim.x * 256;
    for (int r = 0; r < a.n; ++r) {
        const size_t nw = a.j[r].bytes >> 4;
        uint4 *w = reinterpret_cast<uint4 *>(a.j[r].p);
        const unsigned v = a.j[r].val;
        for (size_t i = t; i < nw; i += nt) w[i] = make_uint4(v, v, v, v);
        const size_t tail = a.j[r].bytes & 15;
        if (t < tail) reinterpret_cast<unsigned char *>(a.j[r].p)[(nw << 4) + t] = (unsigned char)v;
    }
}
__global__ void __launch_bounds__(256) collect_kernel(int n, const int16_t *err, const int32_t *aln_len, const unsigned long long *cells,
                                                      const unsigned long long *mt_stat, unsigned long long *out)
{
    const int i = blockIdx.x * 256 + threadIdx.x;
    unsigned long long *oc = out + 4;
    int32_t *ol = reinterpret_cast<int32_t *>(oc + n);
    int16_t *oe = reinterpret_cast<int16_t *>(ol + n);
    if (i < 4) out[i] = mt_stat ? mt_stat[i] : 0ull;
    if (i < n) { oc[i] = cells[i]; ol[i] = aln_len[i]; oe[i] = err[i]; }
    __threadfence_system();
}
}

namespace {

thread_local std::string g_err;
std::mutex g_mu;

static bool dbg_on() { static const bool v = getenv("TWL_DEBUG") != nullptr; return v; }
#define TRACE(...) do { if (dbg_on()) { fprintf(stderr, "[twl trace] " __VA_ARGS__); fputc('\n', stderr); fflush(stderr); } } while (0)

#define HIP_TRY(expr)                                                                                          \
    do {                                                                                                       \
        hipError_t e_ = (expr);                                                                                \
        if (e_ != hipSuccess) {                                                                                \
            g_err = std::string(#expr) + ": " + hipGetErrorString(e_);                                         \
            return TWL_ERR_HIP;                                                                                \
        }                                                                                                      \
    } while (0)


#include "twl_policy.inc.hip"

struct Buf {
    void *p = nullptr;
    size_t cap = 0;
    int ensure(size_t bytes)
    {
        if (bytes <= cap) return TWL_OK;
        if (p) (void)hipFree(p);
        p = nullptr; cap = 0;
        size_t want = bytes + bytes / 8 + 256;
        HIP_TRY(hipMalloc(&p, want));
        cap = want;
        return TWL_OK;
    }
    void release() { if (p) (void)hipFree(p); p = nullptr; cap = 0; }
};

struct Device {
    int id = 0;
    hipStream_t stream = nullptr;
    hipStream_t stream2 = nullptr;
    hipEvent_t ev2[2] = {};
    hipEvent_t ev[8] = {};
    int num_cu = 0;
    Buf cols, tb, cells, queue, items, errs, dbg;
    Buf gtb;
    Buf sim, sim_off, blk_off, m24;
    Buf team;
    Buf mt_chain, mt_rec, mt_seg, mt_spath, mt_stat, mt_jobs, mt_anchor;
    Buf simdump;
    bool dump_on = false;
    std::vector<int32_t> dbg_host;
    std::vector<int32_t> mt_jobs_host;
    twl_mt_dims mt_dims{};
    std::vector<int32_t> mt_order;
    bool mt_seen = false;
    Buf gc_zero;
    std::vector<uint8_t> gc_zero_host;
    std::vector<int16_t> last_err;
    void *probe_h = nullptr; size_t probe_cap = 0;
    PassMemory mem;
    int live_stores = 0;
    void *comm = nullptr;
    int comm_world = 0, comm_rank = 0;
    Buf comm_send, comm_recv;
    int mt_launch = 0;
    char kname[160] = {0};
    Buf h2d_freq, h2d_gop, h2d_gex, h2d_len, h2d_num, d_aln, d_alnlen, d_err;
    twl_stats stats{};
    std::vector<uint64_t> pair_cells;
    twl::FillArgs fills{};
    char *res_h = nullptr; size_t res_cap = 0;
    std::vector<int32_t> last_alnlen;
    std::mutex mu;
};

std::vector<Device *> g_devs;
bool g_init = false;

int find_dev(int device, Device **out)
{
    for (auto *d : g_devs) if (d->id == device) { *out = d; return TWL_OK; }
    g_err = "device not selected in twl_init";
    return TWL_ERR_BAD_ARGUMENT;
}

int flush_fills(Device *d, hipStream_t st)
{
    if (d->fills.n == 0) return TWL_OK;
    unsigned long long most = 0;
    for (int r = 0; r < d->fills.n; ++r) most = std::max(most, d->fills.j[r].bytes);
    const unsigned blocks = (unsigned)std::max<unsigned long long>(1, std::min<unsigned long long>((most / 16 + 255) / 256, (unsigned long long)d->num_cu * 8));
    hipLaunchKernelGGL(twl::fill_kernel, dim3(blocks), dim3(256), 0, st, d->fills);
    d->fills.n = 0;
    HIP_TRY(hipGetLastError());
    return TWL_OK;
}
int queue_fill(Device *d, hipStream_t st, void *p, size_t bytes, unsigned char v)
{
    if (!bytes) return TWL_OK;
    if (((size_t)p & 15) != 0) { HIP_TRY(hipMemsetAsync(p, v, bytes, st)); return TWL_OK; }
    if (d->fills.n == 8) { const int rc = flush_fills(d, st); if (rc) return rc; }
    d->fills.j[d->fills.n++] = twl::FillJob{p, (unsigned long long)bytes, 0x01010101u * v};
    return TWL_OK;
}
#define FILL_TRY(expr) do { const int rc_ = (expr); if (rc_) return rc_; } while (0)

int check_params(const twl_params *p)
{
    if (!p) { g_err = "params is null"; return TWL_ERR_BAD_ARGUMENT; }
    if (p->P != 6 && p->P != 22) { g_err = "profile width P must be 6 (nucleotide) or 22 (protein)"; return TWL_ERR_UNSUPPORTED; }
    if (p->marker < 2 || p->marker > TWL_MAX_MARKER) { g_err = "marker outside [2, TWL_MAX_MARKER]"; return TWL_ERR_UNSUPPORTED; }
    if (p->flen < 1) { g_err = "flen < 1"; return TWL_ERR_UNSUPPORTED; }
    if (p->xdrop < 0) { g_err = "xdrop < 0"; return TWL_ERR_BAD_ARGUMENT; }
    return TWL_OK;
}

#include "twl_knobs.inc.hip"
#include "twl_launch.inc.hip"
#include "twl_run.inc.hip"

}

static void twl_level_pool_release(Device *d);
namespace { extern int g_fail_next_row_allocs; void comm_destroy_raw(void *comm); }

extern "C" {

const char *twl_last_error(void) { return g_err.c_str(); }
#ifndef TWL_SOURCE_HASH
#define TWL_SOURCE_HASH "unstamped"
#endif
#ifndef TWL_BUILD_STAMP
#define TWL_BUILD_STAMP "unstamped"
#endif
__attribute__((used)) static const char twl_build_stamp[] = "TWLSTAMP:" TWL_BUILD_STAMP ";";
const char *twl_version(void) { return "twilight_amd 0.5 (gfx950) src " TWL_SOURCE_HASH; }

int twl_init(const int *device_ids, int n_devices)
{
    std::lock_guard<std::mutex> lk(g_mu);
    if (g_init) return TWL_OK;
    int count = 0;
    HIP_TRY(hipGetDeviceCount(&count));
    if (count < 1) { g_err = "no HIP device"; return TWL_ERR_HIP; }
    std::vector<int> ids;
    if (!device_ids || n_devices <= 0) ids.push_back(0);
    else ids.assign(device_ids, device_ids + n_devices);
    std::vector<Device *> devs;
    auto fail = [&](int rc) {
        for (auto *d : devs) {
            for (auto &e : d->ev) if (e) (void)hipEventDestroy(e);
            if (d->stream) (void)hipStreamDestroy(d->stream);
            if (d->stream2) (void)hipStreamDestroy(d->stream2);
            for (auto &e : d->ev2) if (e) (void)hipEventDestroy(e);
            delete d;
        }
        return rc;
    };
    for (int id : ids) {
        if (id < 0 || id >= count) { g_err = "device id out of range"; return fail(TWL_ERR_BAD_ARGUMENT); }
        auto *d = new Device();
        d->id = id;
        devs.push_back(d);
        hipDeviceProp_t prop;
        hipError_t e = hipSetDevice(id);
        if (e == hipSuccess) e = hipGetDeviceProperties(&prop, id);
        if (e == hipSuccess) { d->num_cu = prop.multiProcessorCount; e = hipStreamCreateWithFlags(&d->stream, hipStreamNonBlocking); if (e == hipSuccess) { int least = 0, greatest = 0; (void)hipDeviceGetStreamPriorityRange(&least, &greatest); e = hipStreamCreateWithPriority(&d->stream2, hipStreamNonBlocking, least); } }
        for (auto &ev : d->ev2) if (e == hipSuccess) e = hipEventCreate(&ev);
        for (auto &ev : d->ev) if (e == hipSuccess) e = hipEventCreate(&ev);
        if (e != hipSuccess) { g_err = std::string("twl_init: ") + hipGetErrorString(e); return fail(TWL_ERR_HIP); }
    }
    g_devs = devs;
    g_init = true;
#ifdef TWL_DEV
    static const struct { const char *env; int knob; } kEnvKnobs[] = {{"TWL_MT_MAX_PAIRS", TWL_KNOB_MT_MAX_PAIRS}, {"TWL_MT_LEAD", TWL_KNOB_MT_LEAD}, {"TWL_MT_MARGIN", TWL_KNOB_MT_MARGIN},
        {"TWL_MT_PERTURB", TWL_KNOB_MT_PERTURB}, {"TWL_MT_ROUNDS", TWL_KNOB_MT_ROUNDS}, {"TWL_MT_THR_JOBS", TWL_KNOB_MT_THR_JOBS}, {"TWL_MT_TAIL_PCT", TWL_KNOB_MT_TAIL_PCT}};
    for (const auto &k : kEnvKnobs) if (const char *v = getenv(k.env)) (void)twl_set_knob(k.knob, atoi(v));
#endif
    return TWL_OK;
}

void twl_shutdown(void)
{
    std::lock_guard<std::mutex> lk(g_mu);
    for (auto *d : g_devs) {
        std::lock_guard<std::mutex> dl(d->mu);
        if (d->live_stores > 0) {
            fprintf(stderr, "twl_shutdown: %d store(s) still alive on device %d; the library stays initialised (twl_store_destroy them first)\n", d->live_stores, d->id);
            return;
        }
    }
    for (auto *d : g_devs) {
        (void)hipSetDevice(d->id);
        (void)hipStreamSynchronize(d->stream);
        (void)hipStreamSynchronize(d->stream2);
        twl_level_pool_release(d);
        if (d->comm) { comm_destroy_raw(d->comm); d->comm = nullptr; }
        d->comm_send.release(); d->comm_recv.release();
        for (Buf *b : {&d->cols, &d->tb, &d->gtb, &d->cells, &d->queue, &d->items, &d->errs, &d->dbg, &d->sim, &d->sim_off, &d->blk_off, &d->m24, &d->team, &d->simdump, &d->mt_chain, &d->mt_rec, &d->mt_seg, &d->mt_spath, &d->mt_stat, &d->mt_jobs, &d->mt_anchor, &d->gc_zero,
                       &d->h2d_freq, &d->h2d_gop, &d->h2d_gex, &d->h2d_len, &d->h2d_num, &d->d_aln, &d->d_alnlen, &d->d_err})
            b->release();
        for (auto &e : d->ev) if (e) (void)hipEventDestroy(e);
        if (d->stream) (void)hipStreamDestroy(d->stream);
        if (d->stream2) (void)hipStreamDestroy(d->stream2);
        for (auto &e : d->ev2) if (e) (void)hipEventDestroy(e);
        if (d->res_h) (void)hipHostFree(d->res_h);
        if (d->probe_h) (void)hipHostFree(d->probe_h);
        delete d;
    }
    g_devs.clear();
    g_init = false;
}

int twl_align_batch_device(int device, void *stream, const twl_params *p, int32_t n_pairs, int32_t seq_len, const float *d_freq,
                           const float *d_gap_open, const float *d_gap_extend, const int32_t *d_len, const int32_t *d_num,
                           int8_t *d_aln_out, int32_t *d_aln_len_out, int16_t *d_err_out)
{
    if (!g_init) { g_err = "twl_init not called"; return TWL_ERR_NOT_INITIALIZED; }
    int rc = check_params(p);
    if (rc) return rc;
    if (n_pairs < 0 || seq_len < 1) { g_err = "bad n_pairs/seq_len"; return TWL_ERR_BAD_ARGUMENT; }
    Device *d = nullptr;
    if ((rc = find_dev(device, &d))) return rc;
    std::lock_guard<std::mutex> lk(d->mu);
    hipStream_t st = stream ? (hipStream_t)stream : d->stream;
    return run_device(d, st, p, n_pairs, seq_len, d_freq, d_gap_open, d_gap_extend, d_len, d_num, d_aln_out, d_aln_len_out,
                      d_err_out, nullptr);
}

static int run_host_slice(Device *d, const twl_params *p, const std::vector<int32_t> &ids, int32_t seq_len, const float *freq,
                          const float *gop, const float *gex, const int32_t *len, const int32_t *num, int8_t *aln_out,
                          int32_t *aln_len_out, int16_t *err_out)
{
    std::lock_guard<std::mutex> lk(d->mu);
    HIP_TRY(hipSetDevice(d->id));
    const int32_t n = (int32_t)ids.size();
    d->stats = twl_stats{};
    d->pair_cells.clear();
    if (n == 0) return TWL_OK;
    const size_t P = (size_t)p->P, sl = (size_t)seq_len;
    int rc;
    if ((rc = d->h2d_freq.ensure((size_t)n * 2 * sl * P * sizeof(float)))) return rc;
    if ((rc = d->h2d_gop.ensure((size_t)n * 2 * sl * sizeof(float)))) return rc;
    if ((rc = d->h2d_gex.ensure((size_t)n * 2 * sl * sizeof(float)))) return rc;
    if ((rc = d->h2d_len.ensure((size_t)n * 2 * sizeof(int32_t)))) return rc;
    if ((rc = d->h2d_num.ensure((size_t)n * 2 * sizeof(int32_t)))) return rc;
    if ((rc = d->d_aln.ensure((size_t)n * 2 * sl))) return rc;
    if ((rc = d->d_alnlen.ensure((size_t)n * sizeof(int32_t)))) return rc;
    if ((rc = d->d_err.ensure((size_t)n * sizeof(int16_t)))) return rc;
    hipStream_t st = d->stream;
    std::vector<int32_t> hl((size_t)n * 2), hn((size_t)n * 2);
    HIP_TRY(hipEventRecord(d->ev[5], st));
    bool contiguous = true;
    for (int32_t t = 0; t < n; ++t) contiguous = contiguous && ids[t] == ids[0] + t;
    for (int32_t t = 0; t < n; ++t) {
        const size_t s = (size_t)ids[t];
        hl[2 * t] = len[2 * s]; hl[2 * t + 1] = len[2 * s + 1];
        hn[2 * t] = num[2 * s]; hn[2 * t + 1] = num[2 * s + 1];
    }
    if (contiguous) {
        const size_t s0 = (size_t)ids[0];
        HIP_TRY(hipMemcpyAsync(d->h2d_freq.p, freq + s0 * 2 * sl * P, (size_t)n * 2 * sl * P * sizeof(float), hipMemcpyHostToDevice, st));
        HIP_TRY(hipMemcpyAsync(d->h2d_gop.p, gop + s0 * 2 * sl, (size_t)n * 2 * sl * sizeof(float), hipMemcpyHostToDevice, st));
        HIP_TRY(hipMemcpyAsync(d->h2d_gex.p, gex + s0 * 2 * sl, (size_t)n * 2 * sl * sizeof(float), hipMemcpyHostToDevice, st));
    } else {
        for (int32_t t = 0; t < n; ++t) {
            const size_t s = (size_t)ids[t];
            HIP_TRY(hipMemcpyAsync((float *)d->h2d_freq.p + (size_t)t * 2 * sl * P, freq + s * 2 * sl * P, 2 * sl * P * sizeof(float), hipMemcpyHostToDevice, st));
            HIP_TRY(hipMemcpyAsync((float *)d->h2d_gop.p + (size_t)t * 2 * sl, gop + s * 2 * sl, 2 * sl * sizeof(float), hipMemcpyHostToDevice, st));
            HIP_TRY(hipMemcpyAsync((float *)d->h2d_gex.p + (size_t)t * 2 * sl, gex + s * 2 * sl, 2 * sl * sizeof(float), hipMemcpyHostToDevice, st));
        }
    }
    HIP_TRY(hipMemcpyAsync(d->h2d_len.p, hl.data(), hl.size() * sizeof(int32_t), hipMemcpyHostToDevice, st));
    HIP_TRY(hipMemcpyAsync(d->h2d_num.p, hn.data(), hn.size() * sizeof(int32_t), hipMemcpyHostToDevice, st));
    rc = run_device(d, st, p, n, seq_len, (const float *)d->h2d_freq.p, (const float *)d->h2d_gop.p, (const float *)d->h2d_gex.p,
                    (const int32_t *)d->h2d_len.p, (const int32_t *)d->h2d_num.p, (int8_t *)d->d_aln.p, (int32_t *)d->d_alnlen.p,
                    (int16_t *)d->d_err.p, hl.data());
    if (rc) return rc;
    std::vector<int32_t> alen((size_t)n);
    std::vector<int16_t> aerr((size_t)n);
    HIP_TRY(hipMemcpyAsync(alen.data(), d->d_alnlen.p, alen.size() * sizeof(int32_t), hipMemcpyDeviceToHost, st));
    HIP_TRY(hipMemcpyAsync(aerr.data(), d->d_err.p, aerr.size() * sizeof(int16_t), hipMemcpyDeviceToHost, st));
// ... 145 lines not shown
}

int twl_debug_read(int device, long long *out, int32_t n)
{
    Device *d = nullptr;
    if (find_dev(device, &d)) return TWL_ERR_BAD_ARGUMENT;
    const size_t base = d->pair_cells.size() * 16 * sizeof(int32_t);
    if (!d->dbg.p || base + (size_t)n * 8 > d->dbg.cap) return TWL_ERR_BAD_ARGUMENT;
    return hipMemcpy(out, (const char *)d->dbg.p + base, (size_t)n * 8, hipMemcpyDeviceToHost) == hipSuccess ? TWL_OK : TWL_ERR_HIP;
}

void *twl_host_alloc(uint64_t bytes)
{
    void *p = nullptr;
    if (!g_init || bytes == 0) return nullptr;
    if (hipHostMalloc(&p, (size_t)bytes, hipHostMallocDefault) != hipSuccess) { (void)hipGetLastError(); return nullptr; }
    return p;
}

void twl_host_free(void *p)
{
    if (p) (void)hipHostFree(p);
}

int twl_copy_to_device(int device, void *dst_dev, const void *src, uint64_t bytes)
{
    if (!g_init) { g_err = "twl_init not called"; return TWL_ERR_NOT_INITIALIZED; }
    Device *d = nullptr;
    int rc = find_dev(device, &d);
    if (rc) return rc;
    if (bytes == 0) return TWL_OK;
    if (!dst_dev || !src) { g_err = "bad argument"; return TWL_ERR_BAD_ARGUMENT; }
    HIP_TRY(hipSetDevice(d->id));
    HIP_TRY(hipMemcpy(dst_dev, src, (size_t)bytes, hipMemcpyHostToDevice));
    return TWL_OK;
}

int twl_copy_from_device(int device, void *dst, const void *src_dev, uint64_t bytes)
{
    if (!g_init) { g_err = "twl_init not called"; return TWL_ERR_NOT_INITIALIZED; }
    Device *d = nullptr;
    int rc = find_dev(device, &d);
    if (rc) return rc;
    if (bytes == 0) return TWL_OK;
    if (!dst || !src_dev) { g_err = "bad argument"; return TWL_ERR_BAD_ARGUMENT; }
    HIP_TRY(hipSetDevice(d->id));
    HIP_TRY(hipMemcpy(dst, src_dev, (size_t)bytes, hipMemcpyDeviceToHost));
    return TWL_OK;
}

int twl_copy_rows_from_device(int device, void *dst, uint64_t dst_pitch, const void *src_dev, uint64_t src_pitch, uint64_t width, uint64_t rows)
{
    if (!g_init) { g_err = "twl_init not called"; return TWL_ERR_NOT_INITIALIZED; }
    Device *d = nullptr;
    int rc = find_dev(device, &d);
    if (rc) return rc;
    if (width == 0 || rows == 0) return TWL_OK;
    if (!dst || !src_dev || dst_pitch < width || src_pitch < width) { g_err = "bad argument"; return TWL_ERR_BAD_ARGUMENT; }
    HIP_TRY(hipSetDevice(d->id));
    HIP_TRY(hipMemcpy2D(dst, (size_t)dst_pitch, src_dev, (size_t)src_pitch, (size_t)width, (size_t)rows, hipMemcpyDeviceToHost));
    return TWL_OK;
}

int twl_set_knob(int key, int value)
{
    std::lock_guard<std::mutex> lk(g_mu);
    switch (key) {
    case TWL_KNOB_MT_PERTURB: g_mt_perturb = std::max(0, value); return TWL_OK;
    case TWL_KNOB_MT_MAX_PAIRS: g_mt_max_pairs = std::max(0, value); return TWL_OK;
    case TWL_KNOB_MT_MIN_MARKER: g_mt_min_marker = std::max(2, value); return TWL_OK;
    case TWL_KNOB_MT_LEAD: g_mt_lead = std::max(16, value); return TWL_OK;
    case TWL_KNOB_MT_MARGIN: if (value < 0) { g_mt_marg = 40; g_mt_marg_lat = 64; } else g_mt_marg = g_mt_marg_lat = std::max(2, value); return TWL_OK;
    case TWL_KNOB_MT_ROUNDS: g_mt_rounds = std::max(1, std::min(7, value)); return TWL_OK;
    case TWL_KNOB_MT_THR_JOBS: g_mt_thr_jobs = std::max(0, value); return TWL_OK;
    case TWL_KNOB_FAIL_ROW_ALLOCS: g_fail_next_row_allocs = std::max(0, value); return TWL_OK;
    case TWL_KNOB_PROT_MODE: if (value < 0 || value > 6) { g_err = "protein mode 0..6"; return TWL_ERR_BAD_ARGUMENT; } g_prot_mode = value; return TWL_OK;
    case TWL_KNOB_ASSUME_ONEHOT_QUERY: g_assume_onehot_query = value ? 1 : 0; return TWL_OK;
    case TWL_KNOB_MT_TAIL_PCT: g_mt_tail_pct = std::max(0, std::min(100, value)); return TWL_OK;
    case TWL_KNOB_MT_WIDE: g_mt_wide = value ? 1 : 0; return TWL_OK;
    case TWL_KNOB_NO_SPEC: g_no_spec = value ? 1 : 0; return TWL_OK;
    case TWL_KNOB_FORCE_GLOBAL: g_force_global = value ? 1 : 0; return TWL_OK;
    case TWL_KNOB_LEAF_STEP: g_leaf_step = value ? 1 : 0; return TWL_OK;
    case TWL_KNOB_POISON_TB: g_poison_tb = value ? 1 : 0; return TWL_OK;
    case TWL_KNOB_MT_ANCHOR: g_mt_anchor = value ? 1 : 0; return TWL_OK;
    case TWL_KNOB_MT_LEAD2: if (value < 0) { g_mt_lead2 = 96; g_mt_lead2_lat = 128; } else g_mt_lead2 = g_mt_lead2_lat = std::max(16, value); return TWL_OK;
    case TWL_KNOB_PROT_CORRIDOR: g_prot_corridor = std::max(0, value); for (auto *d : g_devs) d->mem.forget_corridor(); return TWL_OK;
    case TWL_KNOB_SCOUT_XDROP_PCT: g_scout_xdrop_pct = std::max(10, std::min(100, value)); return TWL_OK;
    case TWL_KNOB_THR_SMALL: g_thr_small = std::max(0, std::min(2, value)); for (auto *d : g_devs) d->mem.forget_small(); return TWL_OK;
    default: g_err = "unknown knob"; return TWL_ERR_BAD_ARGUMENT;
    }
}

#include "twl_comm.inc.hip"

int twl_plan_describe(const twl_params *p, int32_t n_pairs, const int32_t *len, int32_t num_cu, int32_t qry_onehot, int32_t wide_streak, char *out, int32_t cap)
{
    if (!p || (p->P != 6 && p->P != 22) || n_pairs < 0 || (n_pairs > 0 && !len) || num_cu < 1 || !out || cap < 64) { g_err = "bad argument (nucleotide or protein parameters, a buffer of 64+ bytes)"; return TWL_ERR_BAD_ARGUMENT; }
    const PassMemory mem = memory_from_code(wide_streak);
    std::vector<int32_t> order;
    for (int32_t n = 0; n < n_pairs; ++n) if (len[2 * n] > 0 && len[2 * n + 1] > 0) order.push_back(n);
    std::stable_sort(order.begin(), order.end(), [&](int32_t x, int32_t y) { return (int64_t)len[2 * x] + len[2 * x + 1] > (int64_t)len[2 * y] + len[2 * y + 1]; });
    const int ms = p->P - 1;
    std::vector<float> M(p->matrix, p->matrix + ms * ms);
    if (p->P == 22) {
        ProtFacts pf;
        pf.n_run = (int)order.size(); pf.n_pairs = n_pairs; pf.num_cu = num_cu; pf.marker = p->marker; pf.M = M.data(); pf.gap_char = p->gap_char;
        pf.corridor_lost = mem.corridor_lost; pf.h_len = len; pf.order = order.data();
        const ProtPlan pl = plan_protein(pf, current_knobs());
        const int w = snprintf(out, (size_t)cap, "%s; mode %d; window %d", prot_first_name(pl.first), pl.mm, prot_first_window(pl.first));
        if (pl.presim && w > 0 && w < cap) snprintf(out + w, (size_t)(cap - w), "; %zu scores precomputed, corridor %d", pl.simFloats, pl.corridor);
        return TWL_OK;
    }
    NucFacts nf;
    nf.n_run = (int)order.size(); nf.num_cu = num_cu; nf.marker = p->marker; nf.M = M.data(); nf.gap_char = p->gap_char; nf.qry_onehot = qry_onehot != 0;
    nf.remember(mem); nf.h_len = len; nf.order = order.data();
    const NucPlan pl = plan_nucleotide(nf, current_knobs());
    snprintf(out, (size_t)cap, "%s; mode %d; window %d%s; bulk %d tail %d", nuc_first_name(pl.first), pl.mm5 ? 5 : pl.mm,
             pl.first == NucFirst::WideMt ? 3072 : ((pl.first == NucFirst::Throughput && pl.small) ? 512 : ((pl.first == NucFirst::Throughput && pl.four) ? 768 : 1024)), pl.probe ? " or 768 (a sample of the level decides)" : "", pl.bulk, pl.tail);
    return TWL_OK;
}

int twl_get_pair_cells(int device, uint64_t *cells_out, int32_t n)
{
    if (!g_init) { g_err = "twl_init not called"; return TWL_ERR_NOT_INITIALIZED; }
    Device *d = nullptr;
    int rc = find_dev(device, &d);
    if (rc) return rc;
    if (!cells_out || n < 0 || (size_t)n > d->pair_cells.size()) { g_err = "bad argument"; return TWL_ERR_BAD_ARGUMENT; }
    for (int32_t i = 0; i < n; ++i) cells_out[i] = d->pair_cells[i];
    return TWL_OK;
}

int twl_mt_tables(int device, twl_mt_dims *dims, int32_t *order, int32_t *anchor, int32_t *spath, int32_t *chain, int32_t *rec, int8_t *seg, int32_t *front)
{
    if (!g_init) { g_err = "twl_init not called"; return TWL_ERR_NOT_INITIALIZED; }
    Device *d = nullptr;
    int rc = find_dev(device, &d);
    if (rc) return rc;
    std::lock_guard<std::mutex> lk(d->mu);
    return read_mt_tables(d, dims, order, anchor, spath, chain, rec, seg, front);
}

}

#include "twl_level_plan.inc.hip"
#include "twl_store.inc.hip"
#include "twl_level.inc.hip"
#include "twl_place.inc.hip"
#include "twl_merge.inc.hip"
#include "twl_subtree.inc.hip"
#include "twl_guide.inc.hip"
#include "twl_guide_set.inc.hip"
#include "twl_retree.inc.hip"
```

### twilight_amd/csrc/twl_knobs.inc.hip

```cpp

int g_prot_corridor = 448;
int g_mt_perturb = 0;
int g_mt_lead = 320, g_mt_marg = 40;
int g_mt_marg_lat = 64, g_mt_lead2_lat = 128;
int g_mt_anchor = 1, g_mt_lead2 = 96;
int g_mt_max_pairs = 1024, g_mt_min_marker = 512, g_mt_rounds = 2, g_mt_thr_jobs = 256;
int g_scout_xdrop_pct = 100;
int g_no_spec = 0;
int g_thr_small = 0;
int g_mt_wide = 1;
int g_mt_tail_pct = 70;
int g_prot_mode = 0;
int g_force_global = 0;
int g_assume_onehot_query = 0;
int g_leaf_step = 1;
int g_poison_tb = 0;
Knobs current_knobs()
{
    return Knobs{g_mt_max_pairs, g_mt_min_marker, g_mt_tail_pct, g_mt_wide, g_assume_onehot_query, g_no_spec, g_thr_small, (ProtMode)g_prot_mode, g_prot_corridor,
                 g_mt_thr_jobs, g_mt_rounds, g_mt_anchor, g_mt_lead, g_mt_marg, g_mt_marg_lat, g_mt_lead2, g_mt_lead2_lat};
}
```

### twilight_amd/csrc/twl_launch.inc.hip

```cpp

template <class CfgT>
size_t tb_words_for(int marker) { return ((size_t)(marker >> 3) + 1) * (size_t)CfgT::WINDOW; }
int ensure_tb(Buf &b, hipStream_t st, size_t words, int grid)
{
    const size_t bytes = words * sizeof(uint32_t) * (size_t)grid;
    if (const int rc = b.ensure(bytes)) return rc;
    if (g_poison_tb) HIP_TRY(hipMemsetAsync(b.p, 0xFF, bytes, st));
    return TWL_OK;
}
template <auto Kernel, int THREADS>
int resident_per_cu(int *out)
{
    static std::atomic<int> cached{0};
    if (cached.load() == 0) {
        int nb = 0;
        HIP_TRY(hipOccupancyMaxActiveBlocksPerMultiprocessor(&nb, Kernel, THREADS, 0));
        cached.store(std::max(1, nb));
    }
    *out = cached.load();
    return TWL_OK;
}
twl::NArgs lean_args(const Device *d, const twl::KArgs &base)
{
    twl::NArgs a{};
    a.cols = base.cols; a.len = base.len; a.num = base.num; a.aln = base.aln; a.aln_len = base.aln_len; a.err = base.err;
    a.cells = base.cells; a.seq_len = base.seq_len; a.n_pairs_total = base.n_pairs_total;
    a.step_slack = base.step_slack; a.gap_open = base.gap_open; a.gap_extend = base.gap_extend; a.gap_char = base.gap_char; a.gc_zero = base.gc_zero;
    a.xdrop = base.xdrop; a.flen = base.flen; a.marker = base.marker;
    for (int t = 0; t < 25; ++t) a.M[t] = base.M[t];
    a.M24 = (const float *)d->m24.p; a.sim = base.sim; a.sim_off = base.sim_off;
    return a;
}

template <int P, int W, int RPL, bool PRE, bool REFLDS, bool QREG = true, int MINW = 1, int MM = 0>
int launch_dp(Device *d, hipStream_t st, const twl::KArgs &base, const int32_t *d_items, int n_items, int blocks_per_cu, int *grid_out,
              int *window_out = nullptr)
{
    using CfgT = twl::Cfg<P, W, RPL, PRE, REFLDS, QREG>;
    int rc;
    if (blocks_per_cu <= 0 && (rc = resident_per_cu<twl::talco_kernel<P, W, RPL, PRE, REFLDS, QREG, MINW, MM>, CfgT::THREADS>(&blocks_per_cu))) return rc;
    if (window_out) *window_out = CfgT::WINDOW;
    int grid = std::min(n_items, d->num_cu * std::max(1, blocks_per_cu));
    if (grid < 1) grid = 1;
    const size_t tbw = tb_words_for<CfgT>(base.marker);
    if ((rc = ensure_tb(d->tb, st, tbw, grid))) return rc;
    twl::KArgs a = base;
    a.tb = (uint32_t *)d->tb.p;
    a.tb_words = (int32_t)tbw;
    a.items = d_items;
    a.n_items = n_items;
    FILL_TRY(queue_fill(d, st, d->queue.p, sizeof(int32_t), 0));
    int32_t *hb = nullptr;
#ifdef TWL_KERNEL_DEBUG
    if (dbg_on()) {
        HIP_TRY(hipHostMalloc((void **)&hb, 16 * sizeof(int32_t), hipHostMallocMapped));
        for (int i = 0; i < 16; ++i) hb[i] = -777;
        a.hb = hb;
    }
#endif
    TRACE("launch dp W=%d RPL=%d grid=%d threads=%d n_items=%d tb_words=%zu", W, RPL, grid, CfgT::THREADS, n_items, tbw);
    if (!d->kname[0]) snprintf(d->kname, sizeof d->kname, "talco_kernel<%d, %d, %d, %s, %s, %s, %d, %d>", P, W, RPL, PRE ? "true" : "false", REFLDS ? "true" : "false", QREG ? "true" : "false", MINW, MM);
    FILL_TRY(flush_fills(d, st));
    hipLaunchKernelGGL((twl::talco_kernel<P, W, RPL, PRE, REFLDS, QREG, MINW, MM>), dim3(grid), dim3(CfgT::THREADS), 0, st, a);
    HIP_TRY(hipGetLastError());
    if (hb) {
        for (int t = 0; t < 200; ++t) {
            if (hipStreamQuery(st) == hipSuccess) break;
            std::this_thread::sleep_for(std::chrono::milliseconds(100));
            if (t % 10 == 9)
                TRACE("hb: start %d item %d tile %d k %d preB %d postB %d preTB %d postTB %d n %d err %d done %d", hb[0], hb[1], hb[2], hb[3],
                      hb[4], hb[5], hb[6], hb[7], hb[8], hb[9], hb[10]);
        }
        TRACE("hb final: start %d item %d tile %d k %d preB %d postB %d preTB %d postTB %d n %d err %d done %d", hb[0], hb[1], hb[2], hb[3],
              hb[4], hb[5], hb[6], hb[7], hb[8], hb[9], hb[10]);
    }
    *grid_out = grid;
    return TWL_OK;
}

template <int P>
int launch_global(Device *d, hipStream_t st, const twl::KArgs &base, const int32_t *d_items, int n_items, int32_t seq_len, int *grid_out, int *window_out)
{
    const size_t rowcap = (size_t)std::min(std::max(base.flen, 1), std::max(seq_len, 1)) + 2;
    const size_t words = 14 * rowcap + (((size_t)base.marker + 2) * rowcap + 3) / 4;
    const size_t budget = (size_t)4 << 30;
    if (words * sizeof(uint32_t) > budget) { g_err = "a pair whose band needs more than 4 GiB of scratch in the global-memory kernel"; return TWL_ERR_UNSUPPORTED; }
    int grid = (int)std::max<size_t>(1, std::min<size_t>((size_t)n_items, budget / (words * sizeof(uint32_t))));
    grid = std::min(grid, d->num_cu);
    const int rc = ensure_tb(d->gtb, st, words, grid);
    if (rc) return rc;
    twl::GArgs g;
    g.k = base;
    g.k.tb = (uint32_t *)d->gtb.p;
    g.k.tb_words = (int32_t)words;
    if ((size_t)g.k.tb_words != words) { g_err = "a pair too long for the global-memory kernel's scratch index"; return TWL_ERR_UNSUPPORTED; }
    g.k.items = d_items;
    g.k.n_items = n_items;
    g.rowcap = (int32_t)rowcap;
    FILL_TRY(queue_fill(d, st, d->queue.p, sizeof(int32_t), 0));
    FILL_TRY(flush_fills(d, st));
    TRACE("launch global P=%d grid=%d n_items=%d rowcap=%zu words=%zu", P, grid, n_items, rowcap, words);
    hipLaunchKernelGGL((twl::talco_global_kernel<P>), dim3(grid), dim3(1024), 0, st, g);
    HIP_TRY(hipGetLastError());
    *grid_out = grid;
    if (window_out) *window_out = (int)rowcap - 2;
    return TWL_OK;
}

template <int P, int W, int RPL, int MM, int MINW, bool SPEC = false, bool DUMP = false, int SP = 0>
int launch_lean(Device *d, hipStream_t st, const twl::KArgs &base, const int32_t *d_items, int n_items, int *grid_out, int *window_out)
// ... 193 lines not shown
```

### twilight_amd/csrc/twl_level.inc.hip

```cpp

namespace {

static_assert(sizeof(SideRow) == sizeof(twl::SideDesc) && offsetof(SideRow, weight) == offsetof(twl::SideDesc, weight) &&
              offsetof(SideRow, cache_slot) == offsetof(twl::SideDesc, cache_slot) && offsetof(SideRow, store_slot) == offsetof(twl::SideDesc, store_slot),
              "SideRow (twl_level_plan.inc.hip) is uploaded as twl::SideDesc");


int register_stored(twl_store *s, const PreparePlan &pp)
{
    std::vector<CacheEntry> fresh(pp.newIds.size());
    for (size_t k = 0; k < fresh.size(); ++k) {
        const int rc = fresh[k].take(s->d, pp.newLens[k], std::max<size_t>((size_t)pp.newLens[k] * (size_t)s->P * sizeof(float), 16));
        if (rc) return rc;
    }
    for (size_t k = 0; k < fresh.size(); ++k) s->cache[pp.newIds[k]] = std::move(fresh[k]);
    return TWL_OK;
}

int upload_prepare(twl_store *s, hipStream_t st, const PreparePlan &pp, const float *member_weight)
{
    LevelBufs *lv = s->lv;
    std::vector<float *> tab(pp.slotIds.size());
    for (size_t k = 0; k < tab.size(); ++k) tab[k] = (float *)s->cache.find(pp.slotIds[k])->second.buf.p;
    const size_t ns = pp.dsides.size();
// ... 342 lines not shown
        HIP_TRY(hipStreamSynchronize(st));
    }
    return TWL_OK;
}

}

extern "C" {

int twl_level_prepare(twl_store *s, const twl_params *p, float gappy_threshold, int32_t n_pairs, const twl_side *sides, const int32_t *members,
                      const float *member_weight, int32_t seq_len, int32_t *len_out, uint8_t *colinfo_out)
{
    if (!s) { g_err = "store is null"; return TWL_ERR_BAD_ARGUMENT; }
    int rc = check_params(p);
    if (rc) return rc;
    if (p->P != s->P) { g_err = "params.P does not match the store's sequence type"; return TWL_ERR_BAD_ARGUMENT; }
    if (n_pairs < 0 || seq_len < 1 || (n_pairs > 0 && (!sides || !len_out))) { g_err = "bad argument"; return TWL_ERR_BAD_ARGUMENT; }
    s->prepared = false;
    s->n_pairs = n_pairs;
    s->seq_len = seq_len;
    if (n_pairs == 0) { s->prepared = true; return TWL_OK; }
    DEVICE_CALL(call, s->d);
    Device *d = call.d;
    hipStream_t st = call.st;
    if (!s->lv) s->lv = acquire_level(d);
    const char *why = check_sides(n_pairs, sides, seq_len, members, member_weight, s->n_seqs, s->len.data(), [&](int32_t id) {
        const auto it = s->cache.find(id);
        return it == s->cache.end() ? -1 : it->second.len;
    });
    if (why) { g_err = why; return TWL_ERR_BAD_ARGUMENT; }
    PreparePlan pp = plan_prepare(n_pairs, sides, members, s->plane.data());
    const size_t ns = (size_t)n_pairs * 2;
    s->sides.assign(sides, sides + ns);
    s->members.assign(members, members + pp.nm);
    s->h_num.swap(pp.h_num);
    if ((rc = register_stored(s, pp))) return rc;
    if (pp.readsRows && (rc = wait_rows(s, st))) return rc;
    HIP_TRY(hipEventRecord(d->ev[0], st));
    if ((rc = upload_prepare(s, st, pp, member_weight))) return rc;
    const dim3 grid((unsigned)ns, (unsigned)((pp.maxLen + 1023) / 1024));
    if ((rc = size_prepare(s->lv, ns, (size_t)seq_len, (size_t)s->P, grid.y))) return rc;
    if ((rc = launch_prepare(s, st, prepare_args(s, p, gappy_threshold, (int32_t)grid.y), grid))) return rc;
    HIP_TRY(hipEventRecord(d->ev[1], st));
    if ((rc = read_back_prepare(s, st, ns, len_out, colinfo_out))) return rc;
    float ms = 0.f;
    HIP_TRY(hipEventElapsedTime(&ms, d->ev[0], d->ev[1]));
    s->prepare_ms = ms;
    s->prepared = true;
    return TWL_OK;
}

int twl_level_read_colinfo(twl_store *s, int32_t pair, int32_t side, uint8_t *out)
{
    if (!s || !s->prepared || !out || pair >= s->n_pairs || side < 0 || side > 1) { g_err = "bad argument"; return TWL_ERR_BAD_ARGUMENT; }
    DEVICE_CALL(call, s->d);
    if (pair < 0) {
        HIP_TRY(hipMemcpy(out, s->lv->d_colinfo.p, (size_t)s->n_pairs * 2 * (size_t)s->seq_len, hipMemcpyDeviceToHost));
        return TWL_OK;
    }
    const size_t idx = (size_t)pair * 2 + (size_t)side;
    const size_t len = (size_t)std::max(0, s->sides[idx].len);
    if (len) HIP_TRY(hipMemcpy(out, (const uint8_t *)s->lv->d_colinfo.p + idx * (size_t)s->seq_len, len, hipMemcpyDeviceToHost));
    return TWL_OK;
}

int twl_level_align(twl_store *s, const twl_params *p, const uint8_t *run_mask, int8_t *aln_out, int32_t *aln_len_out, int16_t *err_out)
{
    return twl_level_align_mixed(s, p, run_mask, nullptr, aln_out, aln_len_out, err_out);
}

int twl_level_align_mixed(twl_store *s, const twl_params *p, const uint8_t *run_mask, const uint8_t *zero_gap, int8_t *aln_out, int32_t *aln_len_out, int16_t *err_out)
{
    if (!s || !s->prepared) { g_err = "twl_level_prepare has not been called"; return TWL_ERR_BAD_ARGUMENT; }
    int rc = check_params(p);
    if (rc) return rc;
    if (p->P != s->P) { g_err = "params.P does not match the store's sequence type"; return TWL_ERR_BAD_ARGUMENT; }
    const int32_t n = s->n_pairs;
    if (n == 0) return TWL_OK;
    if (!aln_len_out || !err_out) { g_err = "bad argument"; return TWL_ERR_BAD_ARGUMENT; }
    DEVICE_CALL(call, s->d);
    Device *d = call.d;
    hipStream_t st = call.st;
    LevelBufs *lv = s->lv;
    const AlignPlan ap = plan_align(n, s->h_len, s->sides.data(), run_mask, g_leaf_step);
    if ((rc = upload_align(lv, st, ap.lm))) return rc;
    if ((rc = size_align(lv, (size_t)n, (size_t)s->seq_len))) return rc;
    HIP_TRY(hipEventRecord(d->ev[5], st));
    rc = run_device(d, st, p, n, s->seq_len, nullptr, nullptr, nullptr, lv->d_lenmask.as<const int32_t>(), lv->d_num.as<const int32_t>(), (int8_t *)lv->d_aln.p,
                    (int32_t *)lv->d_alnlen.p, (int16_t *)lv->d_err.p, ap.lm.data(), (const float *)lv->d_cols.p, ap.qryOneHot, zero_gap, ap.shape);
    if (rc) return rc;
    return read_back_align(s, d, st, aln_out, aln_len_out, err_out);
}

int twl_level_read_path(twl_store *s, int32_t pair, int8_t *out, int32_t len)
{
    if (!s || !s->prepared || !out || pair < 0 || pair >= s->n_pairs || len < 0 || len > 2 * s->seq_len || !s->lv || !s->lv->d_aln.p) { g_err = "bad argument"; return TWL_ERR_BAD_ARGUMENT; }
    DEVICE_CALL(call, s->d);
    if (len) HIP_TRY(hipMemcpy(out, (const int8_t *)s->lv->d_aln.p + (size_t)pair * 2 * (size_t)s->seq_len, (size_t)len, hipMemcpyDeviceToHost));
    return TWL_OK;
}

int twl_level_read_colinfo_many(twl_store *s, int32_t n_sel, const int32_t *pairs, uint8_t *out)
{
    if (!s || !s->prepared || n_sel < 0 || (n_sel > 0 && (!pairs || !out || !s->lv))) { g_err = "bad argument"; return TWL_ERR_BAD_ARGUMENT; }
    DEVICE_CALL(call, s->d);
    const size_t sl = (size_t)s->seq_len;
    for (int32_t t = 0; t < n_sel; ++t) {
        if (pairs[t] < 0 || pairs[t] >= s->n_pairs) { g_err = "pair index out of range"; return TWL_ERR_BAD_ARGUMENT; }
        HIP_TRY(hipMemcpyAsync(out + (size_t)t * 2 * sl, (const uint8_t *)s->lv->d_colinfo.p + (size_t)pairs[t] * 2 * sl, 2 * sl, hipMemcpyDeviceToHost, call.st));
    }
    HIP_TRY(hipStreamSynchronize(call.st));
    return TWL_OK;
}

int twl_level_read_paths(twl_store *s, int32_t n_sel, const int32_t *pairs, const int32_t *lens, int8_t *out, int32_t out_stride)
{
    if (!s || !s->prepared || n_sel < 0 || (n_sel > 0 && (!pairs || !lens || !out || !s->lv || !s->lv->d_aln.p)) || out_stride < 0) { g_err = "bad argument"; return TWL_ERR_BAD_ARGUMENT; }
    DEVICE_CALL(call, s->d);
    const size_t sl = (size_t)s->seq_len;
    for (int32_t t = 0; t < n_sel; ++t) {
        if (pairs[t] < 0 || pairs[t] >= s->n_pairs || lens[t] < 0 || lens[t] > out_stride || (size_t)lens[t] > 2 * sl) { g_err = "bad selection"; return TWL_ERR_BAD_ARGUMENT; }
        if (lens[t]) HIP_TRY(hipMemcpyAsync(out + (size_t)t * (size_t)out_stride, (const int8_t *)s->lv->d_aln.p + (size_t)pairs[t] * 2 * sl, (size_t)lens[t], hipMemcpyDeviceToHost, call.st));
    }
    HIP_TRY(hipStreamSynchronize(call.st));
    return TWL_OK;
}

int twl_level_restore(twl_store *s, const twl_params *p, int32_t n_sel, const int32_t *pairs, int32_t out_stride, int32_t *final_len_out)
{
    if (!s || !s->prepared || !s->lv || (n_sel > 0 && !s->lv->d_aln.p)) { g_err = "twl_level_align has not been called"; return TWL_ERR_BAD_ARGUMENT; }
    int rc = check_params(p);
    if (rc) return rc;
    const int32_t n = s->n_pairs;
    if (n_sel < 0 || (n_sel > 0 && (!pairs || !final_len_out)) || out_stride < 1) { g_err = "bad argument"; return TWL_ERR_BAD_ARGUMENT; }
    for (int32_t t = 0; t < n_sel; ++t) if (pairs[t] < 0 || pairs[t] >= n) { g_err = "pair index out of range"; return TWL_ERR_BAD_ARGUMENT; }
    DEVICE_CALL(call, s->d);
    if (s->staged_stride && s->staged_stride != out_stride) { g_err = "twl_level_restore: one row pitch per level"; return TWL_ERR_BAD_ARGUMENT; }
    if ((rc = s->lv->d_paths.ensure((size_t)n * (size_t)out_stride))) return rc;
    s->staged_stride = out_stride;
    constexpr int32_t kBatch = 4096;
    for (int32_t at = 0; at < n_sel; at += kBatch)
        if ((rc = restore_batch(s, p, std::min(kBatch, n_sel - at), pairs + at, out_stride, final_len_out + at))) return rc;
    return TWL_OK;
}

int twl_level_exchange_buffers(twl_store *s, int64_t send_bytes, int64_t recv_bytes, void **send_dev, void **recv_dev)
{
    if (!s || !s->prepared || !s->lv || send_bytes < 0 || recv_bytes < 0 || !send_dev || !recv_dev) { g_err = "bad argument"; return TWL_ERR_BAD_ARGUMENT; }
    DEVICE_CALL(call, s->d);
    int rc;
    if ((rc = s->lv->x_send.ensure(std::max<size_t>((size_t)send_bytes, 64)))) return rc;
    if ((rc = s->lv->x_recv.ensure(std::max<size_t>((size_t)recv_bytes, 64)))) return rc;
    *send_dev = s->lv->x_send.p; *recv_dev = s->lv->x_recv.p;
    return TWL_OK;
}

int twl_level_paths_to_block(twl_store *s, int32_t n_sel, const int32_t *pairs, const int32_t *lens, const uint8_t *where, void *blk_dev, const int64_t *blk_off)
{
    return level_rows_block(s, true, n_sel, pairs, lens, where, blk_dev, blk_off);
}

int twl_level_paths_from_block(twl_store *s, int32_t n_sel, const int32_t *pairs, const int32_t *lens, const void *blk_dev, const int64_t *blk_off)
{
    return level_rows_block(s, false, n_sel, pairs, lens, nullptr, const_cast<void *>(blk_dev), blk_off);
}

int twl_level_write_final(twl_store *s, int32_t pair, const int8_t *path, int32_t len)
{
    if (!s || !s->prepared || !s->lv || !s->staged_stride || pair < 0 || pair >= s->n_pairs || len < 0 || len > s->staged_stride || (len > 0 && !path)) { g_err = "bad argument (twl_level_restore first)"; return TWL_ERR_BAD_ARGUMENT; }
    DEVICE_CALL(call, s->d);
    if (len) HIP_TRY(hipMemcpy((int8_t *)s->lv->d_paths.p + (size_t)pair * (size_t)s->staged_stride, path, (size_t)len, hipMemcpyHostToDevice));
    return TWL_OK;
// ... 81 lines not shown
```

### twilight_amd/csrc/twl_level_plan.inc.hip

```cpp
#include <algorithm>
#include <cstdint>
#include <unordered_map>
#include <vector>
#include "../../include/twl_level.h"

struct SideRow { int32_t n_members, member_off, len, num; float weight; int32_t cache_slot, store_slot, pad; };

template <class CacheLen>
const char *check_sides(int32_t n_pairs, const twl_side *sides, int32_t seq_len, const int32_t *members, const float *member_weight, int32_t n_seqs,
                        const int32_t *row_len, CacheLen cacheLen)
{
    const size_t ns = (size_t)n_pairs * 2;
    size_t nm = 0;
    for (size_t i = 0; i < ns; ++i) {
        const twl_side &sd = sides[i];
        if (sd.n_members < 0 || sd.member_off < 0 || sd.len < 0 || sd.len > seq_len || sd.num < 1) return "bad side descriptor";
        nm = std::max(nm, (size_t)sd.member_off + (size_t)sd.n_members);
    }
    if (nm > 0 && (!members || !member_weight)) return "member tables missing";
    std::unordered_map<int32_t, int32_t> stored;
    for (size_t i = 0; i < ns; ++i) {
        const twl_side &sd = sides[i];
        for (int32_t m = 0; m < sd.n_members; ++m) {
            const int32_t q = members[sd.member_off + m];
            if (q < 0 || q >= n_seqs) return "member sequence id out of range";
            if (row_len[q] != sd.len) return "member row length differs from the side's len";
        }
        if (sd.cache_id >= 0) {
            const auto it = stored.find(sd.cache_id);
            if ((it != stored.end() ? it->second : cacheLen(sd.cache_id)) != sd.len) return "cache id unknown or of another length";
        } else if (sd.store_id >= 0) {
            if (stored.count(sd.store_id) || cacheLen(sd.store_id) >= 0) return "store_id already in use";
            stored[sd.store_id] = sd.len;
        }
    }
    return nullptr;
}

struct PreparePlan {
    size_t nm = 0;
    std::vector<SideRow> dsides;
    std::vector<int32_t> slotIds;
    std::vector<int32_t> newIds, newLens;
    std::vector<uint8_t> mplane;
    std::vector<int32_t> h_num;
    bool readsRows = false;
    int32_t maxLen = 1;
};

inline PreparePlan plan_prepare(int32_t n_pairs, const twl_side *sides, const int32_t *members, const uint8_t *plane)
{
    PreparePlan pp;
    const size_t ns = (size_t)n_pairs * 2;
    for (size_t i = 0; i < ns; ++i) pp.nm = std::max(pp.nm, (size_t)sides[i].member_off + (size_t)sides[i].n_members);
    pp.mplane.assign(pp.nm, 0);
    pp.dsides.resize(ns);
    pp.h_num.resize(ns);
    std::unordered_map<int32_t, int32_t> slotOf;
    auto slot = [&](int32_t id) {
        const auto it = slotOf.find(id);
        if (it != slotOf.end()) return it->second;
        pp.slotIds.push_back(id);
        return slotOf[id] = (int32_t)pp.slotIds.size() - 1;
    };
    for (size_t i = 0; i < ns; ++i) {
        const twl_side &sd = sides[i];
        for (int32_t m = 0; m < sd.n_members; ++m) pp.mplane[sd.member_off + m] = plane[members[sd.member_off + m]];
        SideRow &ds = pp.dsides[i];
        ds.n_members = sd.n_members; ds.member_off = sd.member_off; ds.len = sd.len; ds.num = sd.num; ds.weight = sd.weight;
        ds.cache_slot = ds.store_slot = -1; ds.pad = 0;
        if (sd.cache_id >= 0) ds.cache_slot = slot(sd.cache_id);
        else if (sd.store_id >= 0) { pp.newIds.push_back(sd.store_id); pp.newLens.push_back(sd.len); ds.store_slot = slot(sd.store_id); }
        pp.h_num[i] = sd.num;
        pp.readsRows = pp.readsRows || (sd.cache_id < 0 && sd.n_members > 0);
        pp.maxLen = std::max(pp.maxLen, sd.len);
    }
    return pp;
}

struct AlignPlan {
    std::vector<int32_t> lm;
    bool qryOneHot = true;
    int shape = 0;
};

inline AlignPlan plan_align(int32_t n, const std::vector<int32_t> &h_len, const twl_side *sides, const uint8_t *run_mask, int leaf_step)
{
    AlignPlan ap;
    ap.lm = h_len;
    if (run_mask)
        for (int32_t i = 0; i < n; ++i) if (!run_mask[i]) ap.lm[2 * i] = ap.lm[2 * i + 1] = 0;
    auto runs = [&](int32_t i) { return ap.lm[2 * i] > 0 && ap.lm[2 * i + 1] > 0; };
    for (int32_t i = 0; i < n && ap.qryOneHot; ++i)
        if (runs(i)) ap.qryOneHot = sides[2 * (size_t)i + 1].n_members == 1 && sides[2 * (size_t)i + 1].cache_id < 0;
    if (leaf_step) {
        bool leaf = true, any = false;
        for (int32_t i = 0; i < n && leaf; ++i) {
            if (!runs(i)) continue;
            any = true;
            for (int side = 0; side < 2; ++side) {
                const twl_side &sd = sides[2 * (size_t)i + side];
                leaf = leaf && sd.n_members == 1 && sd.cache_id < 0 && sd.num == 1;
            }
        }
        ap.shape = (any && leaf) ? 2 : 0;
    }
    return ap;
}

inline const char *check_commit(int32_t n, int32_t seq_len, int32_t staged, bool haveDp, bool havePaths, const int32_t *path_len, int32_t path_stride,
                                const uint8_t *from_dp)
{
    if (n > 0 && ((!havePaths && !from_dp) || !path_len || path_stride < 1)) return "bad argument";
    if (staged && (!from_dp || staged != path_stride)) return "commit after twl_level_restore: from_dp and the restore's row pitch are required";
    if (from_dp && !staged) for (int32_t i = 0; i < n; ++i) if (from_dp[i] == 2) return "from_dp == 2 without twl_level_restore";
    if (from_dp) {
        for (int32_t i = 0; i < n; ++i) {
            if (from_dp[i] == 1 && (!haveDp || path_len[i] > 2 * seq_len)) return "from_dp without a DP output of this level";
            if (!from_dp[i] && path_len[i] > 0 && !havePaths) return "bad argument";
        }
    }
    for (int32_t i = 0; i < n; ++i) if (path_len[i] < 0 || path_len[i] > path_stride) return "path_len outside [0, path_stride]";
    return nullptr;
}

constexpr int kRowGroup = 64;

struct CommitPlan {
    int32_t maxPath = 0, nChunks = 0;
    std::vector<int32_t> work;
    std::vector<int32_t> merge;
    std::vector<float> mergew;
    std::vector<int32_t> mergeIds;
    std::vector<uint8_t> mplane;
    std::vector<int32_t> flips;
    bool hostRows = false;
    bool side = false;
    unsigned nWork() const { return (unsigned)(work.size() / 3); }
    unsigned nMerge() const { return (unsigned)(merge.size() / 4); }
};

inline int32_t max_path(int32_t n, const int32_t *path_len)
{
    int32_t m = 0;
    for (int32_t i = 0; i < n; ++i) m = std::max(m, path_len[i]);
    return m;
}

inline void plan_commit(CommitPlan &cp, int32_t n, const twl_side *sides, const std::vector<int32_t> &members, const uint8_t *plane, const int32_t *path_len,
                        const uint8_t *from_dp)
{
    cp.work.clear(); cp.merge.clear(); cp.mergew.clear(); cp.mergeIds.clear(); cp.flips.clear();
    cp.maxPath = max_path(n, path_len);
    cp.nChunks = (cp.maxPath + 255) / 256;
    cp.hostRows = !from_dp;
    for (int32_t i = 0; i < n; ++i) {
        if (path_len[i] == 0) continue;
        if (from_dp && !from_dp[i]) cp.hostRows = true;
        for (int sd = 0; sd < 2; ++sd) {
            const twl_side &x = sides[2 * (size_t)i + sd];
            for (int32_t m = 0; m < x.n_members; m += kRowGroup) { cp.work.push_back(2 * i + sd); cp.work.push_back(m); cp.work.push_back(std::min(kRowGroup, x.n_members - m)); }
            for (int32_t m = 0; m < x.n_members; ++m) { cp.flips.push_back(members[x.member_off + m]); cp.flips.push_back(path_len[i]); }
        }
        const twl_side &r = sides[2 * (size_t)i], &q = sides[2 * (size_t)i + 1];
        const int32_t rid = r.cache_id >= 0 ? r.cache_id : r.store_id, qid = q.cache_id >= 0 ? q.cache_id : q.store_id;
        if (rid >= 0 && qid >= 0) {
            const int32_t at = 3 * (int32_t)cp.nMerge();
            cp.merge.insert(cp.merge.end(), {i, at, at + 1, at + 2});
            cp.mergew.push_back(r.weight); cp.mergew.push_back(q.weight);
            cp.mergeIds.push_back(rid); cp.mergeIds.push_back(qid);
        }
    }
    cp.mplane.resize(members.size());
    for (size_t k = 0; k < members.size(); ++k) cp.mplane[k] = plane[members[k]];
    cp.side = cp.nWork() > 0 && n <= 32 && !cp.hostRows;
}
```

### twilight_amd/csrc/twl_run.inc.hip

```cpp

struct Call {
    Device *d; hipStream_t st; const twl_params *p;
    int32_t n_pairs, seq_len;
    const int32_t *d_len, *d_num; int32_t *d_alnlen; int16_t *d_err;
    const int32_t *h_len;
    std::vector<int32_t> len_host, order;
    int32_t n_run = 0;
    uint64_t nominal = 0;
    twl::KArgs a{};
    const int32_t *items() const { return (const int32_t *)d->items.p; }
    long long len_sum(int32_t pr) const { return (long long)h_len[2 * pr] + h_len[2 * pr + 1]; }
};
struct Results { std::vector<int16_t> err; std::vector<unsigned long long> cells; unsigned long long mt[4] = {0, 0, 0, 0}; };

int pinned_at_least(void **h, size_t *cap, size_t bytes)
{
    if (bytes <= *cap) return TWL_OK;
    if (*h) (void)hipHostFree(*h);
    *h = nullptr; *cap = 0;
    HIP_TRY(hipHostMalloc(h, bytes + bytes / 2, hipHostMallocDefault));
    *cap = bytes + bytes / 2;
    return TWL_OK;
}

template <int MM0, int... MMs, class F>
int with_mm(int mode, F &&f)
{
    if constexpr (sizeof...(MMs) == 0) return f(std::integral_constant<int, MM0>{});
    else return mode == MM0 ? f(std::integral_constant<int, MM0>{}) : with_mm<MMs...>(mode, f);
}
#define MM_OF(x) decltype(x)::value

int order_pairs(Call &c)
{
    const int32_t n_pairs = c.n_pairs;
    if (!c.h_len) {
        c.len_host.resize((size_t)n_pairs * 2);
        HIP_TRY(hipMemcpyAsync(c.len_host.data(), c.d_len, c.len_host.size() * sizeof(int32_t), hipMemcpyDeviceToHost, c.st));
        HIP_TRY(hipStreamSynchronize(c.st));
        c.h_len = c.len_host.data();
    }
    const int32_t *h_len = c.h_len;
    c.order.resize((size_t)n_pairs);
    std::iota(c.order.begin(), c.order.end(), 0);
    auto live = [h_len](int32_t x) { return h_len[2 * x] > 0 && h_len[2 * x + 1] > 0; };
    std::stable_sort(c.order.begin(), c.order.end(), [&](int32_t x, int32_t y) {
        if (live(x) != live(y)) return live(x);
        return (int64_t)h_len[2 * x] + h_len[2 * x + 1] > (int64_t)h_len[2 * y] + h_len[2 * y + 1];
    });
    for (int32_t n = 0; n < n_pairs; ++n) c.n_run += live(n) ? 1 : 0;
    for (int32_t n = 0; n < n_pairs; ++n) c.nominal += (uint64_t)std::max(0, h_len[2 * n]) * (uint64_t)std::max(0, h_len[2 * n + 1]);
    HIP_TRY(hipMemcpyAsync(c.d->items.p, c.order.data(), c.order.size() * sizeof(int32_t), hipMemcpyHostToDevice, c.st));
    return TWL_OK;
}

int prepare_args(Call &c, const float *d_freq, const float *d_gop, const float *d_gex, int8_t *d_aln, const float *d_packed, const uint8_t *h_gc_zero)
{
    Device *d = c.d; hipStream_t st = c.st; const twl_params *p = c.p; const int32_t n_pairs = c.n_pairs;
    int rc;
    TRACE("run_device n_pairs=%d seq_len=%d", n_pairs, c.seq_len);
    HIP_TRY(hipEventRecord(d->ev[0], st));
    if (!d_packed) {
        const size_t n_cols = (size_t)n_pairs * 2 * (size_t)c.seq_len;
        const int threads = 256;
        const int blocks = (int)std::min<size_t>((n_cols + threads - 1) / threads, (size_t)d->num_cu * 8);
        if (p->P == 22) hipLaunchKernelGGL(twl::pack_kernel<22>, dim3(std::max(blocks, 1)), dim3(threads), 0, st, d_freq, d_gop, d_gex, (float *)d->cols.p, n_cols);
        else hipLaunchKernelGGL(twl::pack_kernel<6>, dim3(std::max(blocks, 1)), dim3(threads), 0, st, d_freq, d_gop, d_gex, (float *)d->cols.p, n_cols);
        HIP_TRY(hipGetLastError());
    }
    HIP_TRY(hipEventRecord(d->ev[1], st));
    if (dbg_on()) { HIP_TRY(hipStreamSynchronize(st)); TRACE("pack done"); }

    twl::KArgs &a = c.a;
    a.cols = d_packed ? d_packed : (const float *)d->cols.p;
    a.len = c.d_len; a.num = c.d_num;
    a.aln = d_aln; a.aln_len = c.d_alnlen; a.err = c.d_err;
    a.cells = (unsigned long long *)d->cells.p;
    a.queue = (int32_t *)d->queue.p;
    a.seq_len = c.seq_len;
    a.n_pairs_total = n_pairs;
    a.gap_open = p->gap_open; a.gap_extend = p->gap_extend; a.gap_char = p->gap_char;
    a.gc_zero = nullptr;
    if (h_gc_zero && p->gap_char != 0.0f && std::any_of(h_gc_zero, h_gc_zero + n_pairs, [](uint8_t z) { return z != 0; })) {
        if ((rc = d->gc_zero.ensure((size_t)n_pairs))) return rc;
        d->gc_zero_host.assign(h_gc_zero, h_gc_zero + n_pairs);
        HIP_TRY(hipMemcpyAsync(d->gc_zero.p, d->gc_zero_host.data(), (size_t)n_pairs, hipMemcpyHostToDevice, st));
        a.gc_zero = (const uint8_t *)d->gc_zero.p;
    }
    a.xdrop = p->xdrop; a.flen = p->flen; a.marker = p->marker;
    a.step_slack = 1 << 16;
    a.dbg = nullptr;
    if (dbg_on()) {
        if ((rc = d->dbg.ensure((size_t)n_pairs * 16 * sizeof(int32_t) + 2048 + 16 * 192 * 32))) return rc;
        HIP_TRY(hipMemsetAsync(d->dbg.p, 0xff, (size_t)n_pairs * 16 * sizeof(int32_t), st));
        a.dbg = (int32_t *)d->dbg.p;
    }
    { const int ms = p->P - 1; for (int l = 0; l < ms; ++l) for (int m = 0; m < ms; ++m) a.M[ms * l + m] = p->matrix[ms * l + m]; }
    FILL_TRY(queue_fill(d, st, c.d_alnlen, (size_t)n_pairs * sizeof(int32_t), 0));
    FILL_TRY(queue_fill(d, st, c.d_err, (size_t)n_pairs * sizeof(int16_t), 0));
    FILL_TRY(queue_fill(d, st, d->cells.p, (size_t)n_pairs * sizeof(unsigned long long), 0));
    return TWL_OK;
}

int first_protein(Call &c, Ran &ran, int *grid, int *window)
{
    Device *d = c.d; hipStream_t st = c.st; twl::KArgs &a = c.a; const int32_t *items = c.items(), *h_len = c.h_len; const int32_t n_run = c.n_run, n_pairs = c.n_pairs;
    int rc;
    ProtFacts pf;
    pf.n_run = n_run; pf.n_pairs = n_pairs; pf.num_cu = d->num_cu; pf.marker = c.p->marker; pf.M = a.M; pf.gap_char = c.p->gap_char; pf.dump = d->dump_on;
    pf.corridor_lost = d->mem.corridor_lost_for(n_run); pf.h_len = h_len; pf.order = c.order.data();
    const ProtPlan pl = plan_protein(pf, current_knobs());
    TRACE("plan: %s, matrix mode %d", prot_first_name(pl.first), pl.mm);
    ran.mode = pl.mm; ran.spec = pl.spec; ran.ranMt = pl.first == ProtFirst::MtPresim;
    ran.start = pl.small ? Level::Mid : Level::Wide;
    if (pl.first == ProtFirst::R1) return launch_dp<22, 8, 1, false, true, true>(d, st, a, items, n_run, 0, grid, window);
    if (pl.first == ProtFirst::Dense) return launch_dp<22, 8, 2, false, true, true>(d, st, a, items, n_run, 0, grid, window);
    if ((rc = d->m24.ensure(21 * 24 * sizeof(float)))) return rc;
    std::vector<float> m24(21 * 24, 0.0f);
    for (int l = 0; l < 21; ++l) for (int m = 0; m < 21; ++m) m24[24 * l + m] = a.M[21 * l + m];
    HIP_TRY(hipMemcpyAsync(d->m24.p, m24.data(), m24.size() * sizeof(float), hipMemcpyHostToDevice, st));
    HIP_TRY(hipStreamSynchronize(st));
    if (pl.presim) {
        std::vector<long long> off((size_t)n_pairs, 0);
        std::vector<int32_t> blk((size_t)n_pairs + 1, 0);
        long long floats = 0;
        for (int32_t t = 0; t < n_run; ++t) {
            const long long R = h_len[2 * c.order[t]], Q = h_len[2 * c.order[t] + 1];
            off[c.order[t]] = floats;
            floats += (R + Q) * ((Q + 63) & ~63ll);
            blk[t + 1] = blk[t] + (int32_t)(((R + Q - 1 + 63) / 64) * ((Q + 63) / 64));
        }
        if ((rc = d->sim.ensure(pl.simFloats * sizeof(float)))) return rc;
        if ((rc = d->sim_off.ensure(off.size() * sizeof(long long)))) return rc;
        if ((rc = d->blk_off.ensure(blk.size() * sizeof(int32_t)))) return rc;
        HIP_TRY(hipMemcpyAsync(d->sim_off.p, off.data(), off.size() * sizeof(long long), hipMemcpyHostToDevice, st));
        HIP_TRY(hipMemcpyAsync(d->blk_off.p, blk.data(), blk.size() * sizeof(int32_t), hipMemcpyHostToDevice, st));
        HIP_TRY(hipStreamSynchronize(st));
        twl::ScoreArgs sa{};
        sa.cols = a.cols; sa.len = c.d_len; sa.num = c.d_num; sa.items = items; sa.blk_off = (const int32_t *)d->blk_off.p;
        sa.n_items = n_run; sa.seq_len = c.seq_len; sa.gap_char = c.p->gap_char; sa.gc_zero = a.gc_zero; sa.M24 = (const float *)d->m24.p;
        sa.sim = (float *)d->sim.p; sa.sim_off = (const long long *)d->sim_off.p;
        d->mem.begin_corridor_level(n_run);
        sa.corridor = pl.corridor;
        ran.usedCorridor = sa.corridor > 0;
        FILL_TRY(flush_fills(d, st));
        hipLaunchKernelGGL(twl::score_matrix_kernel<22>, dim3((unsigned)blk[n_run]), dim3(256), 0, st, sa);
        HIP_TRY(hipGetLastError());
        a.sim = (const float *)d->sim.p;
        a.sim_off = (const long long *)d->sim_off.p;
    }
    switch (pl.first) {
    case ProtFirst::MtPresim: return launch_mt<22, 4, 1>(d, st, a, items, c.order, n_run, h_len, grid, window);
    case ProtFirst::SpecShared: return launch_lean<22, 8, 1, 4, 4, true>(d, st, a, items, n_run, grid, window);
    case ProtFirst::Spec16: return launch_lean<22, 16, 1, 4, 1, true>(d, st, a, items, n_run, grid, window);
    case ProtFirst::Plain16: return launch_lean<22, 16, 1, 4, 1>(d, st, a, items, n_run, grid, window);
    case ProtFirst::Dump:
        if (!pl.lean || n_run != 1) { g_err = "score dump: one pair, matrix within the fast-division range"; return TWL_ERR_UNSUPPORTED; }
        return launch_lean<22, 16, 1, 3, 1, false, true>(d, st, a, items, n_run, grid, window);
    case ProtFirst::Thr512: return launch_lean<22, 8, 1, 3, 4>(d, st, a, items, n_run, grid, window);
    case ProtFirst::Sparse16: return launch_lean<22, 16, 1, 3, 1>(d, st, a, items, n_run, grid, window);
    default: return pl.presim ? launch_dp<22, 8, 2, false, true, true, 1, 4>(d, st, a, items, n_run, 0, grid, window)
                              : launch_dp<22, 8, 2, false, true, true, 1, 3>(d, st, a, items, n_run, 0, grid, window);
    }
}

int sample_small_window(Call &c, const NucPlan &pl, Ran &ran, int *grid, int *window, bool *small, int *done)
{
    Device *d = c.d; hipStream_t st = c.st; std::vector<int32_t> &order = c.order; const int bulk = pl.bulk;
    const int S = d->num_cu;
    std::vector<int32_t> front, rest;
// ... 103 lines not shown
    case Rung::MtStitch1024: return with_mm<5, 2>(ran.mode, [&](auto MM) { return launch_mt<6, MM_OF(MM), 3, false, 4>(d, st, a, it, redo, n, c.h_len, g, w); });
    case Rung::Lean1024:     return with_mm<5, 2>(ran.mode, [&](auto MM) { return launch_lean<6, 8, 2, MM_OF(MM), 4>(d, st, a, it, n, g, w); });
    case Rung::Prot16:       return launch_lean<22, 16, 1, 3, 1>(d, st, a, it, n, g, w);
    case Rung::Mt3072:       return launch_mt<6, 2, 3, true, 4>(d, st, a, it, redo, n, c.h_len, g, w);
    case Rung::Lean2048:     return launch_lean<6, 8, 4, 2, 2>(d, st, a, it, n, g, w);
    case Rung::Ieee16x2:     return launch_dp<6, 16, 2, false, true, true, 1, 0>(d, st, a, it, n, 0, g, w);
    case Rung::Wide4608:     return ran.prot ? launch_dp<22, 8, 9, false, false, false>(d, st, a, it, n, 1, g, w) : launch_dp<6, 8, 9, false, false, true>(d, st, a, it, n, 1, g, w);
    default:                 return ran.prot ? launch_global<22>(d, st, a, it, n, c.seq_len, g, w) : launch_global<6>(d, st, a, it, n, c.seq_len, g, w);
    }
}
int timed_rerun(Call &c, const Ran &ran, Rung rung, const std::vector<int32_t> &redo, float *ms_redo, int *window)
{
    Device *d = c.d;
    HIP_TRY(hipMemcpyAsync(d->items.p, redo.data(), redo.size() * sizeof(int32_t), hipMemcpyHostToDevice, c.st));
    HIP_TRY(hipEventRecord(d->ev[3], c.st));
    int grid2 = 0;
    TRACE("re-run: %d pairs on %s", (int)redo.size(), rung_name(rung));
    FILL_TRY(launch_rung(c, ran, rung, redo, &grid2, window));
    HIP_TRY(hipEventRecord(d->ev[4], c.st));
    HIP_TRY(hipStreamSynchronize(c.st));
    float ms = 0.f;
    HIP_TRY(hipEventElapsedTime(&ms, d->ev[3], d->ev[4]));
    *ms_redo += ms;
    d->stats.n_launches += 1;
    d->stats.n_relaunched += (int32_t)redo.size();
    return TWL_OK;
}
std::vector<int32_t> pairs_with(const std::vector<int16_t> &err, int16_t code, int16_t code2)
{
    std::vector<int32_t> v;
    for (int32_t n = 0; n < (int32_t)err.size(); ++n) if (err[n] == code || err[n] == code2) v.push_back(n);
    return v;
}

int climb_ladder(Call &c, const Ran &ran, Results &res, LadderOutcome &o, float *ms_redo)
{
    const Knobs k = current_knobs();
    int rc, w2 = 0;
    if ((rc = collect(c, ran.ranMt, res, true, ran.ranMt ? res.mt : nullptr))) return rc;
    TRACE("dp kernel done");
    o.firstInline = res.mt[1];
    for (Level at = ran.start; at != Level::Global;) {
        std::vector<int32_t> redo = pairs_with(res.err, twl::kErrGuard, twl::kErrGuard);
        const RedoKind kind = redo.empty() ? RedoKind::Overflow : RedoKind::Guard;
        if (kind == RedoKind::Overflow) redo = pairs_with(res.err, twl::kErrOverflow, twl::kErrOverflow);
        if (redo.empty()) break;
        RedoFacts f;
        f.count = (int)redo.size(); f.marker = c.p->marker; f.dump = c.d->dump_on;
        for (int32_t n : redo) f.sumLen += c.len_sum(n);
        const Step s = next_rung(ran, at, kind, f, k);
        if (kind == RedoKind::Guard) o.guardRound = true;
        else if (at == Level::From512) o.from512Pairs = f.count;
        if (s.rung == Rung::Mt3072 || s.rung == Rung::Lean2048) o.widePairs += f.count;
        if (s.rung == Rung::Mt3072 || s.rung == Rung::MtStitch1024) o.redoMt = true;
        if ((rc = timed_rerun(c, ran, s.rung, redo, ms_redo, &w2))) return rc;
        o.relaunched += f.count;
        at = s.next;
        if (at != Level::Global && (rc = collect(c, ran.ranMt || o.redoMt, res, false, nullptr))) return rc;
    }
    if (o.relaunched > 0) {
        unsigned long long now[4];
        if ((rc = collect(c, ran.ranMt || o.redoMt, res, true, now))) return rc;
        if (o.redoMt) for (int t = 0; t < 4; ++t) res.mt[t] += now[t];
    }
    return TWL_OK;
}

int global_stage(Call &c, const Ran &ran, Results &res, bool anyMt, float *ms_redo)
{
    const std::vector<int32_t> redo = pairs_with(res.err, twl::kErrOverflow, twl::kErrGuard);
    int rc, w2 = 0;
    if (!redo.empty()) {
        if ((rc = timed_rerun(c, ran, Rung::Global, redo, ms_redo, &w2))) return rc;
        c.d->stats.window = std::max(c.d->stats.window, w2);
        if ((rc = collect(c, anyMt, res, true, nullptr))) return rc;
    }
    if (!pairs_with(res.err, twl::kErrOverflow, twl::kErrGuard).empty()) { g_err = "internal: a re-run code survived the global-memory kernel"; return TWL_ERR_HIP; }
    return TWL_OK;
}

int run_device(Device *d, hipStream_t st, const twl_params *p, int32_t n_pairs, int32_t seq_len, const float *d_freq,
               const float *d_gop, const float *d_gex, const int32_t *d_len, const int32_t *d_num, int8_t *d_aln,
               int32_t *d_alnlen, int16_t *d_err, const int32_t *h_len, const float *d_packed = nullptr, bool qry_onehot = false,
               const uint8_t *h_gc_zero = nullptr, int shape = 0)
{
    HIP_TRY(hipSetDevice(d->id));
    d->stats = twl_stats{};
    d->kname[0] = 0;
    d->fills.n = 0;
    d->last_err.clear();
    d->last_alnlen.clear();
    d->pair_cells.assign((size_t)n_pairs, 0);
    if (n_pairs == 0) return TWL_OK;

    int rc;
    if (!d_packed && (rc = d->cols.ensure((size_t)n_pairs * 2 * (size_t)seq_len * (size_t)(p->P + 2) * sizeof(float)))) return rc;
    if ((rc = d->cells.ensure((size_t)n_pairs * sizeof(unsigned long long)))) return rc;
    if ((rc = d->queue.ensure(64))) return rc;
    if ((rc = d->items.ensure((size_t)n_pairs * sizeof(int32_t)))) return rc;
    Call c{d, st, p, n_pairs, seq_len, d_len, d_num, d_alnlen, d_err, h_len};
    if ((rc = order_pairs(c))) return rc;
    if ((rc = prepare_args(c, d_freq, d_gop, d_gex, d_aln, d_packed, h_gc_zero))) return rc;

    Ran ran;
    ran.prot = (p->P == 22);
    ran.start = ran.prot ? Level::Wide : Level::Mid;
    int grid = 0, window = 0;
    if (c.n_run == 0) rc = TWL_OK;
    else if (g_force_global) {
        rc = ran.prot ? launch_global<22>(d, st, c.a, c.items(), c.n_run, seq_len, &grid, &window) : launch_global<6>(d, st, c.a, c.items(), c.n_run, seq_len, &grid, &window);
        snprintf(d->kname, sizeof d->kname, "talco_global_kernel<%d>", ran.prot ? 22 : 6);
    }
    else rc = ran.prot ? first_protein(c, ran, &grid, &window) : first_nucleotide(c, qry_onehot, shape, ran, &grid, &window);
    if (rc) return rc;
    FILL_TRY(flush_fills(d, st));
    HIP_TRY(hipEventRecord(d->ev[2], st));
    d->stats.n_launches = 1;
    d->stats.grid = grid;
    d->stats.window = window;
    d->stats.matrix_mode = ran.mode;
    d->stats.speculative = ran.spec;
    memcpy(d->stats.kernel, d->kname, sizeof d->stats.kernel);

    Results res;
    res.err.resize((size_t)n_pairs); res.cells.resize((size_t)n_pairs);
    LadderOutcome o;
    float ms_redo = 0.f;
    FILL_TRY(pinned_at_least((void **)&d->res_h, &d->res_cap, 4 * sizeof(unsigned long long) + (size_t)n_pairs * (sizeof(unsigned long long) + sizeof(int32_t) + sizeof(int16_t))));
    if ((rc = climb_ladder(c, ran, res, o, &ms_redo))) return rc;
    d->mem.update(ran, o, c.n_run, c.n_run > 0 ? c.len_sum(c.order[0]) : 0, current_knobs());
    if ((rc = global_stage(c, ran, res, ran.ranMt || o.redoMt, &ms_redo))) return rc;

    uint64_t total = 0;
    for (int32_t n = 0; n < n_pairs; ++n) { d->pair_cells[n] = res.cells[n]; total += res.cells[n]; }
    if (ran.ranMt || o.redoMt) { d->stats.mt_tiles_predicted = (int32_t)res.mt[0]; d->stats.mt_tiles_inline = (int32_t)res.mt[1]; d->stats.mt_scouts_failed = (int32_t)res.mt[2]; }
    d->last_err = res.err;
    if (d->gtb.cap > ((size_t)256 << 20)) d->gtb.release();
    if (dbg_on()) {
        d->dbg_host.resize((size_t)n_pairs * 16);
        HIP_TRY(hipMemcpy(d->dbg_host.data(), d->dbg.p, d->dbg_host.size() * sizeof(int32_t), hipMemcpyDeviceToHost));
        for (int32_t n = 0; n < n_pairs && n < 64; ++n) {
            const int32_t *g = &d->dbg_host[(size_t)n * 16];
            fprintf(stderr, "[twl dbg] pair %d: tiles %d last_k %d conv 0x%x L %d U %d ref_idx %d qry_idx %d pos %d err %d steps_left %d R %d Q %d\n",
                    n, g[0], g[1], g[2], g[3], g[4], g[5], g[6], g[7], g[8], g[9], g[10], g[11]);
        }
    }
    float ms_pack = 0.f, ms_k = 0.f;
    HIP_TRY(hipEventElapsedTime(&ms_pack, d->ev[0], d->ev[1]));
    HIP_TRY(hipEventElapsedTime(&ms_k, d->ev[1], d->ev[2]));
    d->stats.band_cells = total;
    d->stats.nominal_cells = c.nominal;
    d->stats.pack_ms = ms_pack;
    d->stats.kernel_ms = ms_k + ms_redo;
    d->stats.total_ms = ms_pack + ms_k + ms_redo;
    return TWL_OK;
}
```

Baseline: 231.4 billion.

## Add per-pair single-sequence forms to specialize nucleotide DP scoring

Pairs where the query or reference side is a single uncached sequence are tagged on the host with a form code, uploaded per pair, and read uniformly in the nucleotide kernel. For form 1 (single query) the query substitution row is folded at load time. For form 2 (single reference) the ring block stores precomputed per-column matrix rows. Either way the per-cell score collapses to a short dot product instead of the full 4x4 profile product. Guard checks reject columns that are not one-hot. The cost is extra branching and register pressure in the inner step, LDS-loaded matrix values replacing pinned registers, and a small host upload.

```diff
diff --git a/include/twl_align.h b/include/twl_align.h
--- a/include/twl_align.h
+++ b/include/twl_align.h
@@ -99,7 +99,7 @@
 
 enum twl_knob { TWL_KNOB_MT_PERTURB = 1, TWL_KNOB_MT_MAX_PAIRS = 2, TWL_KNOB_MT_MIN_MARKER = 3, TWL_KNOB_MT_LEAD = 4, TWL_KNOB_MT_MARGIN = 5,
                 TWL_KNOB_MT_ROUNDS = 6, TWL_KNOB_MT_THR_JOBS = 7, TWL_KNOB_FAIL_ROW_ALLOCS = 8,
-                TWL_KNOB_PROT_MODE = 9, TWL_KNOB_ASSUME_ONEHOT_QUERY = 10, TWL_KNOB_MT_TAIL_PCT = 11, TWL_KNOB_MT_WIDE = 12, TWL_KNOB_NO_SPEC = 13, TWL_KNOB_SCOUT_XDROP_PCT = 14, TWL_KNOB_THR_SMALL = 15, TWL_KNOB_FORCE_GLOBAL = 16, TWL_KNOB_LEAF_STEP = 17, TWL_KNOB_POISON_TB = 18, TWL_KNOB_MT_ANCHOR = 19, TWL_KNOB_MT_LEAD2 = 20, TWL_KNOB_PROT_CORRIDOR = 21 };
+                TWL_KNOB_PROT_MODE = 9, TWL_KNOB_ASSUME_ONEHOT_QUERY = 10, TWL_KNOB_MT_TAIL_PCT = 11, TWL_KNOB_MT_WIDE = 12, TWL_KNOB_NO_SPEC = 13, TWL_KNOB_SCOUT_XDROP_PCT = 14, TWL_KNOB_THR_SMALL = 15, TWL_KNOB_FORCE_GLOBAL = 16, TWL_KNOB_LEAF_STEP = 17, TWL_KNOB_POISON_TB = 18, TWL_KNOB_MT_ANCHOR = 19, TWL_KNOB_MT_LEAD2 = 20, TWL_KNOB_PROT_CORRIDOR = 21, TWL_KNOB_PAIR_FORMS = 22, TWL_KNOB_ASSERT_PAIR_FORM = 23 };
 int twl_set_knob(int key, int value);
 int twl_plan_describe(const twl_params *p, int32_t n_pairs, const int32_t *len, int32_t num_cu, int32_t qry_onehot, int32_t wide_streak, char *out, int32_t cap);
 
diff --git a/twilight_amd/api.py b/twilight_amd/api.py
--- a/twilight_amd/api.py
+++ b/twilight_amd/api.py
@@ -150,6 +150,8 @@
 KNOB_MT_ANCHOR = 19
 KNOB_PROT_CORRIDOR = 21
 KNOB_MT_LEAD2 = 20
+KNOB_PAIR_FORMS = 22
+KNOB_ASSERT_PAIR_FORM = 23
 PROT_MODES = {"auto": 0, "dense": 1, "sparse": 2, "presim": 3, "r1": 4, "lean_sparse": 5, "lean_presim": 6}
 
 
diff --git a/twilight_amd/csrc/talco_kernel.hip.h b/twilight_amd/csrc/talco_kernel.hip.h
--- a/twilight_amd/csrc/talco_kernel.hip.h
+++ b/twilight_amd/csrc/talco_kernel.hip.h
@@ -31,6 +31,7 @@
     int32_t step_slack;
     float gap_open, gap_extend, gap_char;
     const uint8_t *gc_zero;
+    const uint8_t *pair_form;
     int32_t xdrop, flen, marker;
     float M[441];
     const float *sim;
diff --git a/twilight_amd/csrc/talco_nuc.hip.h b/twilight_amd/csrc/talco_nuc.hip.h
--- a/twilight_amd/csrc/talco_nuc.hip.h
+++ b/twilight_amd/csrc/talco_nuc.hip.h
@@ -28,6 +28,7 @@
     int32_t step_slack;
     float gap_open, gap_extend, gap_char;
     const uint8_t *gc_zero;
+    const uint8_t *pair_form;
     int32_t xdrop, flen, marker;
     float M[25];
     const float *M24;
@@ -50,6 +51,7 @@
 
 typedef float nuc_f4 __attribute__((ext_vector_type(4)));
 typedef float nuc_f2 __attribute__((ext_vector_type(2)));
+typedef float nuc_f3 __attribute__((ext_vector_type(3)));
 __device__ __forceinline__ float4 lds_ld128(unsigned addr)
 {
     const nuc_f4 v = *reinterpret_cast<const __attribute__((address_space(3))) nuc_f4 *>((const __attribute__((address_space(3))) char *)nullptr + addr);
@@ -251,6 +253,9 @@
     }
 }
 
+template <int F> struct FormC { static constexpr int value = F, tag = F; };
+struct FormRT { int value; static constexpr int tag = 3; };
+
 template <int W, int RPL>
 struct NCfg {
     static constexpr int NV = W * RPL;
@@ -276,6 +281,7 @@
 #else
     constexpr bool QPRE = !((RPL >= 3 || MINW >= 5) && MM == 2);
 #endif
+    constexpr bool FORMS = (P == 6 && MM == 2 && !QPRE && W == 4 && MT <= 2 && !SPEC && !DUMP && SP == 0);
     constexpr int F4 = (P + 2) / 4;
     constexpr bool SPARSE = (MM == 3), PRESIM = (MM == 4);
     constexpr int RP = PRESIM ? 1 : F4;
@@ -290,14 +296,14 @@
         unsigned red[4];
         int conv[4];
         int edge[2 * NV];
-        int4 trash[64];
+        int4 trash[64 + (FORMS ? 1 : 0)];
     };
     __shared__ ParBuf s_par[2];
     __shared__ int s_misc[8];
     __shared__ int8_t s_rev[2 * kMaxMarker + 16];
     __shared__ unsigned long long s_team[4];
     constexpr unsigned O_CD = (unsigned)offsetof(ParBuf, cd), O_EXCH = (unsigned)offsetof(ParBuf, exch), O_RED = (unsigned)offsetof(ParBuf, red),
-                       O_CONV = (unsigned)offsetof(ParBuf, conv), O_TRASH = (unsigned)offsetof(ParBuf, trash), O_EDGE = (unsigned)offsetof(ParBuf, edge);
+                       O_CONV = (unsigned)offsetof(ParBuf, conv), O_TRASH = (unsigned)offsetof(ParBuf, trash), O_EDGE = (unsigned)offsetof(ParBuf, edge), O_MV = O_TRASH + 64u * 16u;
 
     const int lane = threadIdx.x & 63;
     const int w = __builtin_amdgcn_readfirstlane(threadIdx.x >> 6);
@@ -328,6 +334,8 @@
         const float gc = (a.gc_zero && __builtin_amdgcn_readfirstlane((int)a.gc_zero[pair])) ? 0.0f : a.gap_char;
         const bool gcNZ = (gc != 0.0f);
         const unsigned long long gcMask = gcNZ ? ~0ull : 0ull;
+        int form = 0;
+        if constexpr (FORMS) { if (a.pair_form) form = __builtin_amdgcn_readfirstlane((int)a.pair_form[pair]); }
         const int spLo = (a.marker - 1) * slot - 1, spHi = a.marker * slot + 1;
         int anchRef = -1, anchQry = -1;
         bool anchored = false;
@@ -472,7 +480,7 @@
             const int fLen = min(a.flen, min(refLen, qLen));
             const int fcap = min(fLen, 64 * (NV - 2));
             float vmA = a.M[0], vmB = a.M[2], vmC = a.M[1];
-            asm volatile("" : "+v"(vmA), "+v"(vmB), "+v"(vmC));
+            if constexpr (!FORMS) asm volatile("" : "+v"(vmA), "+v"(vmB), "+v"(vmC));
             float S1[RPL], I1[RPL], D1[RPL], LS2[RPL];
             int CS1[RPL], CI1[RPL], CD1[RPL], LCS2[RPL];
             float qv[RPL][QN], gopq[RPL], gexq[RPL], qM[RPL][NQM];
@@ -485,7 +493,7 @@
             uint32_t tbacc[RPL];
             bool q5any[RPL];
 
-            auto load_q = [&](int r) __attribute__((always_inline)) {
+            auto load_q = [&](int r, int fm) __attribute__((always_inline)) {
                 const int i = b0[r] + lane;
                 const bool ok = qry_idx + i < Q;
                 if constexpr (PRESIM) {
@@ -538,12 +546,24 @@
                     else q5any[r] = gcNZ && __builtin_amdgcn_ballot_w64(cb[P - 1] != 0.0f) != 0ull;
                     bool bad = false;
                     if constexpr (SP == 1) bad = (cb[P - 1] != 0.0f);
+                    if constexpr (FORMS) {
+                        if (fm == 1) {
+                            const int nz = (cb[0] != 0.0f) + (cb[1] != 0.0f) + (cb[2] != 0.0f) + (cb[3] != 0.0f) + (cb[4] != 0.0f);
+                            bad = (nz > 1) | (cb[5] != 0.0f);
+                            auto mq = [&](int l, int m) __attribute__((always_inline)) { return (l == m) ? vmA : (((l ^ m) == 2) ? vmB : vmC); };
+#pragma unroll
+                            for (int l = 0; l < 4; ++l) qv[r][l] = ((cb[0] * mq(l, 0) + cb[1] * mq(l, 1)) + cb[2] * mq(l, 2)) + cb[3] * mq(l, 3);
+                            qv[r][4] = (((cb[0] + cb[1]) + cb[2]) + cb[3]) + cb[4];
+                            qv[r][5] = 0.0f;
+                            q5any[r] = false;
+                        }
+                    }
 #pragma unroll
                     for (int t = 0; t < P; ++t) bad = bad | div_guard_bad(cb[t]);
                     guardBad = guardBad | (__builtin_amdgcn_ballot_w64(bad) != 0ull);
                 }
             };
-            auto load_ring_block = [&](int B) __attribute__((always_inline)) {
+            auto load_ring_block = [&](int B, int fm) __attribute__((always_inline)) {
                 const int col = 64 * B + lane;
                 const int slot = (B % NB) * 64 + lane;
                 const bool ok = col < refLen;
@@ -551,6 +571,18 @@
                     float4 c = make_float4(0.f, 0.f, 0.f, 0.f);
                     if (ok) c = colsR[F4 * (size_t)(ref_idx + col) + (F4 - 1)];
                     s_ring[slot] = c;
+                } else if (FORMS && fm == 2) {
+                    float4 c0 = make_float4(0.f, 0.f, 0.f, 0.f), c1 = c0;
+                    if (ok) { c0 = colsR[F4 * (size_t)(ref_idx + col)]; c1 = colsR[F4 * (size_t)(ref_idx + col) + 1]; }
+                    const int nz = (c0.x != 0.0f) + (c0.y != 0.0f) + (c0.z != 0.0f) + (c0.w != 0.0f) + (c1.x != 0.0f);
+                    bool bad = (nz > 1) | (c1.y != 0.0f);
+                    bad = bad | div_guard_bad(c0.x) | div_guard_bad(c0.y) | div_guard_bad(c0.z) | div_guard_bad(c0.w) | div_guard_bad(c1.x) | div_guard_bad(c1.y);
+                    const bool n0 = (c0.x != 0.0f), n1 = (c0.y != 0.0f), n2 = (c0.z != 0.0f), n3 = (c0.w != 0.0f);
+                    auto pick = [&](float v0, float v1, float v2, float v3) __attribute__((always_inline)) { return n0 ? v0 : (n1 ? v1 : (n2 ? v2 : (n3 ? v3 : 0.0f))); };
+                    const float wv = (((c0.x + c0.y) + c0.z) + c0.w) + c1.x;
+                    s_ring[slot] = make_float4(pick(vmA, vmC, vmB, vmC), pick(vmC, vmA, vmC, vmB), pick(vmB, vmC, vmA, vmC), pick(vmC, vmB, vmC, vmA));
+                    s_ring[CAP + slot] = make_float4(wv, c1.y, c1.z, c1.w);
+                    guardBad = guardBad | (__builtin_amdgcn_ballot_w64(bad) != 0ull);
                 } else {
                     bool bad = false;
                     uint32_t mk = 0;
@@ -558,8 +590,9 @@
                     for (int t = 0; t < F4; ++t) {
                         float4 c = make_float4(0.f, 0.f, 0.f, 0.f);
                         if (ok) c = colsR[F4 * (size_t)(ref_idx + col) + t];
+                        const float f[4] = {c.x, c.y, c.z, c.w};
+                        if (FORMS && fm == 1 && t == 1) c.x = 1.0f;
                         s_ring[t * CAP + slot] = c;
-                        const float f[4] = {c.x, c.y, c.z, c.w};
 #pragma unroll
                         for (int u = 0; u < 4; ++u) {
                             if (4 * t + u < P) bad = bad | div_guard_bad(f[u]);
@@ -583,11 +616,11 @@
                 ring_addr(r, 0);
                 tbacc[r] = 0;
                 S1[r] = I1[r] = D1[r] = LS2[r] = -1.0f;
-                load_q(r);
+                load_q(r, form);
             }
             int hiBlk = 1;
-            if (w == 0 % W) load_ring_block(0);
-            if (w == 1 % W) load_ring_block(1);
+            if (w == 0 % W) load_ring_block(0, form);
+            if (w == 1 % W) load_ring_block(1, form);
             for (int t = threadIdx.x; t < WINDOW + 4; t += C::THREADS) { s_par[0].cd[t] = kDB; s_par[1].cd[t] = kDB; }
             if (threadIdx.x == 0) {
                 s_par[0].red[0] = s_par[1].red[0] = (unsigned)__float_as_int(-inf);
@@ -595,6 +628,7 @@
                 for (int t = 0; t < 2; ++t) { s_par[t].conv[0] = 0x7fffffff; s_par[t].conv[1] = (int)0x80000000; s_par[t].conv[2] = 0; }
                 s_team[1] = 0ull; s_team[2] = 0ull; s_team[3] = 0ull;
                 s_misc[4] = 0;
+                if constexpr (FORMS) { for (int t = 0; t < 2; ++t) s_par[t].trash[64 * (FORMS ? 1 : 0)] = make_int4(__float_as_int(a.M[0]), __float_as_int(a.M[2]), __float_as_int(a.M[1]), 0); }
             }
             __syncthreads();
 
@@ -631,8 +665,9 @@
             }
 
             auto stop_tile = [&]() __attribute__((always_inline)) { go = false; kStop = (int)0x80000000; };
-            auto hook = [&](auto PHtag) __attribute__((always_inline)) {
+            auto hook = [&](auto PHtag, auto FORMtag) __attribute__((always_inline)) {
                 constexpr int PH = decltype(PHtag)::value;
+                const int FORM = FORMtag.value;
                 constexpr bool TB = (PH != 2);
                 const int Uk = Lk + Wk;
                 if constexpr (TB) {
@@ -652,13 +687,15 @@
                     tbPending = false;
                 }
                 const int need_hi = ((k + 10 - Lk) >> 6) + 1;
-                if (hiBlk < need_hi) { ++hiBlk; if (w == hiBlk % W) load_ring_block(hiBlk); }
+                if (hiBlk < need_hi) { ++hiBlk; if (w == hiBlk % W) load_ring_block(hiBlk, FORM); }
             };
-            auto step = [&](auto PHtag, auto GENtag) __attribute__((always_inline)) {
+            auto step = [&](auto PHtag, auto GENtag, auto FORMtag) __attribute__((always_inline)) {
                 constexpr int PH = decltype(PHtag)::value;
                 constexpr bool GEN = decltype(GENtag)::value;
+                const unsigned FORM = (unsigned)FORMtag.value;
                 constexpr bool TB = (PH != 2), CONV = (PH != 0);
-                asm volatile("; TWL_STEP PH=%c0 GEN=%c1 (a comment: tools/isa_block_step.py finds the diagonal loops by it)" ::"n"(PH), "n"((int)GEN));
+                static_assert(decltype(FORMtag)::tag == 0 || FORMS, "only the kernels with the forms instantiate their steps");
+                asm volatile("; TWL_STEP PH=%c0 GEN=%c1 FORM=%c2 (a comment: tools/isa_block_step.py finds the diagonal loops by it)" ::"n"(PH), "n"((int)GEN), "n"(decltype(FORMtag)::tag));
                 TWL_STAMP(t_head);
 #if defined(TWL_EXP_SALU)
                 { int xs = k; 
@@ -694,7 +731,8 @@
                     if ((unsigned)u <= (unsigned)W64) {
                         if constexpr (MT == 0 && RPL >= 2) { if (r == 0) TWL_SETPRIO(2); else TWL_SETPRIO(3); }
                         else TWL_SETPRIO(2);
-                        const int i = b + lane;
+                        int i = b + lane;
+                        if constexpr (FORMS && MT == 1) i = b + (int)__builtin_amdgcn_mbcnt_hi(~0u, __builtin_amdgcn_mbcnt_lo(~0u, 0u));
                         float eS, eI; int eCS = 0, eCI = 0;
                         if constexpr (CONV) {
                             const nuc_i4 e = lds_ld<nuc_i4>(vprev + exRel[r]);
@@ -706,12 +744,19 @@
                         const bool inband = (unsigned)(i - vL) <= vwidth1;
                         float numer = 0.0f, rg, gopr, gexr;
                         if constexpr (P == 6) {
+                            nuc_f3 m3 = nuc_f3{0.0f, 0.0f, 0.0f};
+                            if constexpr (FORMS) m3 = *reinterpret_cast<const volatile __attribute__((address_space(3))) nuc_f3 *>((const __attribute__((address_space(3))) char *)nullptr + (vcur + O_MV));
                             const float4 c0 = lds_ld128(ra[r]);
                             const float4 c1 = lds_ld128(ra[r] + CAP * 16);
                             const float rc[5] = {c0.x, c0.y, c0.z, c0.w, c1.x};
                             rg = c1.y; gopr = c1.z; gexr = c1.w;
                             constexpr int NM = (MM == 0) ? 5 : (MM == 5 ? 1 : 4);
                             const nuc_f2 r01 = nuc_f2{c0.x, c0.y}, r23 = nuc_f2{c0.z, c0.w};
+                            if (__builtin_expect(FORM != 0u, 0)) {
+                                numer = (((qv[r][0] * rc[0]) * rc[4] + (qv[r][1] * rc[1]) * rc[4]) + (qv[r][2] * rc[2]) * rc[4]) + (qv[r][3] * rc[3]) * rc[4];
+                                if (q5any[r]) numer += (rc[4] * qv[r][5]) * gc;
+                                if ((__builtin_amdgcn_ballot_w64(inband) & __builtin_amdgcn_ballot_w64(rg != 0.0f) & gcMask) != 0ull) numer += (rg * qv[r][4]) * gc;
+                            } else {
                             nuc_f2 s01, s23;
                             if constexpr (QPRE) {
                                 s01 = qP[r][0] * r01; s23 = qP[r][1] * r23;
@@ -729,7 +774,9 @@
                                 for (int m = 1; m < 4; ++m) { s01 = s01 + fp(m, 0) * r01; s23 = s23 + fp(m, 1) * r23; }
 #endif
                             } else {
-                                auto mv = [&](int l, int m) __attribute__((always_inline)) { return (l == m) ? vmA : (((l ^ m) == 2) ? vmB : vmC); };
+                                float gA = vmA, gB = vmB, gC = vmC;
+                                if constexpr (FORMS) { gA = m3.x; gB = m3.y; gC = m3.z; }
+                                auto mv = [&](int l, int m) __attribute__((always_inline)) { return (l == m) ? gA : (((l ^ m) == 2) ? gB : gC); };
                                 float sl[4];
 #pragma unroll
                                 for (int l = 0; l < 4; ++l) {
@@ -756,6 +803,7 @@
                             if (rgAny) {
 #pragma unroll
                                 for (int m = 0; m < 5; ++m) numer += (rg * qv[r][m]) * gc;
+                            }
                             }
                         } else if constexpr (SPARSE) {
                             const float4 cl = lds_ld128(ra[r] + (F4 - 1) * CAP * 16);
@@ -896,7 +944,7 @@
                     if (__builtin_expect(u < 0, 0)) {
                         while (b0[r] + 63 < Lk) b0[r] += 64 * NV;
                         ring_addr(r, k);
-                        load_q(r);
+                        load_q(r, FORM);
                         tbMust |= 1u << r;
                     }
                     ra[r] += 16u;
@@ -997,7 +1045,7 @@
                 }
                 if (!ended) {
                     ++k;
-                    if (k == kHook || (PH == 1 && k == marker + 1)) { hook(PHtag); kHook = (k & ~7) + 8; }
+                    if (k == kHook || (PH == 1 && k == marker + 1)) { hook(PHtag, FORMtag); kHook = (k & ~7) + 8; }
                     if (__builtin_expect((unsigned)Wk >= (unsigned)fcap, 0)) {
                         const int Uk = Lk + Wk;
                         if (k >= kEnd) {}
@@ -1007,7 +1055,7 @@
                         else {
 #pragma unroll
                             for (int r = 0; r < RPL; ++r)
-                                if (b0[r] + 63 < Lk) { while (b0[r] + 63 < Lk) b0[r] += 64 * NV; ring_addr(r, k); load_q(r); tbMust |= 1u << r; }
+                                if (b0[r] + 63 < Lk) { while (b0[r] + 63 < Lk) b0[r] += 64 * NV; ring_addr(r, k); load_q(r, FORM); tbMust |= 1u << r; }
                         }
                     }
                 }
@@ -1019,14 +1067,24 @@
 #endif
             {
                 using T0 = std::integral_constant<int, 0>; using T1 = std::integral_constant<int, 1>; using T2 = std::integral_constant<int, 2>;
+                auto run_form = [&](auto PHtag, int kLim, auto FORMtag) __attribute__((always_inline)) {
+                    constexpr int PH = decltype(PHtag)::value;
+                    if constexpr (PH == 1) { while (go && k < kLim) step(PHtag, std::true_type{}, FORMtag); }
+                    else {
+                        while (go && spec && k < kLim) step(PHtag, std::true_type{}, FORMtag);
+                        kStop = go ? kLim : (int)0x80000000;
+                        while (k < kStop) step(PHtag, std::false_type{}, FORMtag);
+                    }
+                };
                 auto run = [&](auto PHtag, int kLim) __attribute__((always_inline)) {
-                    constexpr int PH = decltype(PHtag)::value;
-                    if constexpr (PH == 1) { while (go && k < kLim) step(PHtag, std::true_type{}); }
-                    else {
-                        while (go && spec && k < kLim) step(PHtag, std::true_type{});
-                        kStop = go ? kLim : (int)0x80000000;
-                        while (k < kStop) step(PHtag, std::false_type{});
-                    }
+                    if constexpr (!FORMS) run_form(PHtag, kLim, FormC<0>{});
+#if defined(TWL_EXP_FORM_LOOPS)
+                    else if (form == 1) run_form(PHtag, kLim, FormC<1>{});
+                    else if (form == 2) run_form(PHtag, kLim, FormC<2>{});
+                    else run_form(PHtag, kLim, FormC<0>{});
+#else
+                    else run_form(PHtag, kLim, FormRT{form});
+#endif
                 };
                 const int kA = min(kEnd, marker - 1);
                 auto poll = [&]() __attribute__((always_inline)) {
@@ -1115,6 +1173,14 @@
 
             cells += tile_cells;
             dbg_lastk = last_k; dbg_conv = conv_value; dbg_L = Lk; dbg_U = Lk + Wk;
+            if constexpr (FORMS) {
+                if (form != 0) {
+                    if (guardBad) s_misc[4] = 1;
+                    __syncthreads();
+                    guardBad = __builtin_amdgcn_readfirstlane(s_misc[4]) != 0;
+                    if (guardBad) { err = kErrGuard; break; }
+                }
+            }
             if (tile_err != 0) { err = tile_err; break; }
             if (PRESIM || SP == 1 || !denomOne) {
                 if (guardBad) s_misc[4] = 1;
diff --git a/twilight_amd/csrc/twl_align.hip b/twilight_amd/csrc/twl_align.hip
--- a/twilight_amd/csrc/twl_align.hip
+++ b/twilight_amd/csrc/twl_align.hip
@@ -117,6 +117,8 @@
     std::vector<int32_t> mt_order;
     bool mt_seen = false;
     Buf gc_zero;
+    Buf pair_form;
+    std::vector<uint8_t> pair_form_host;
     std::vector<uint8_t> gc_zero_host;
     std::vector<int16_t> last_err;
     void *probe_h = nullptr; size_t probe_cap = 0;
@@ -259,7 +261,7 @@
         twl_level_pool_release(d);
         if (d->comm) { comm_destroy_raw(d->comm); d->comm = nullptr; }
         d->comm_send.release(); d->comm_recv.release();
-        for (Buf *b : {&d->cols, &d->tb, &d->gtb, &d->cells, &d->queue, &d->items, &d->errs, &d->dbg, &d->sim, &d->sim_off, &d->blk_off, &d->m24, &d->team, &d->simdump, &d->mt_chain, &d->mt_rec, &d->mt_seg, &d->mt_spath, &d->mt_stat, &d->mt_jobs, &d->mt_anchor, &d->gc_zero,
+        for (Buf *b : {&d->cols, &d->tb, &d->gtb, &d->cells, &d->queue, &d->items, &d->errs, &d->dbg, &d->sim, &d->sim_off, &d->blk_off, &d->m24, &d->team, &d->simdump, &d->mt_chain, &d->mt_rec, &d->mt_seg, &d->mt_spath, &d->mt_stat, &d->mt_jobs, &d->mt_anchor, &d->gc_zero, &d->pair_form,
                        &d->h2d_freq, &d->h2d_gop, &d->h2d_gex, &d->h2d_len, &d->h2d_num, &d->d_aln, &d->d_alnlen, &d->d_err})
             b->release();
         for (auto &e : d->ev) if (e) (void)hipEventDestroy(e);
@@ -571,6 +573,8 @@
     case TWL_KNOB_FORCE_GLOBAL: g_force_global = value ? 1 : 0; return TWL_OK;
     case TWL_KNOB_LEAF_STEP: g_leaf_step = value ? 1 : 0; return TWL_OK;
     case TWL_KNOB_POISON_TB: g_poison_tb = value ? 1 : 0; return TWL_OK;
+    case TWL_KNOB_PAIR_FORMS: g_pair_forms = value & 3; return TWL_OK;
+    case TWL_KNOB_ASSERT_PAIR_FORM: if (value < 0 || value > 2) { g_err = "pair form 0..2"; return TWL_ERR_BAD_ARGUMENT; } g_assert_pair_form = value; return TWL_OK;
     case TWL_KNOB_MT_ANCHOR: g_mt_anchor = value ? 1 : 0; return TWL_OK;
     case TWL_KNOB_MT_LEAD2: if (value < 0) { g_mt_lead2 = 96; g_mt_lead2_lat = 128; } else g_mt_lead2 = g_mt_lead2_lat = std::max(16, value); return TWL_OK;
     case TWL_KNOB_PROT_CORRIDOR: g_prot_corridor = std::max(0, value); for (auto *d : g_devs) d->mem.forget_corridor(); return TWL_OK;
diff --git a/twilight_amd/csrc/twl_knobs.inc.hip b/twilight_amd/csrc/twl_knobs.inc.hip
--- a/twilight_amd/csrc/twl_knobs.inc.hip
+++ b/twilight_amd/csrc/twl_knobs.inc.hip
@@ -14,6 +14,8 @@
 int g_force_global = 0;
 int g_assume_onehot_query = 0;
 int g_leaf_step = 1;
+int g_pair_forms = 3;
+int g_assert_pair_form = 0;
 int g_poison_tb = 0;
 Knobs current_knobs()
 {
diff --git a/twilight_amd/csrc/twl_launch.inc.hip b/twilight_amd/csrc/twl_launch.inc.hip
--- a/twilight_amd/csrc/twl_launch.inc.hip
+++ b/twilight_amd/csrc/twl_launch.inc.hip
@@ -25,7 +25,7 @@
     twl::NArgs a{};
     a.cols = base.cols; a.len = base.len; a.num = base.num; a.aln = base.aln; a.aln_len = base.aln_len; a.err = base.err;
     a.cells = base.cells; a.seq_len = base.seq_len; a.n_pairs_total = base.n_pairs_total;
-    a.step_slack = base.step_slack; a.gap_open = base.gap_open; a.gap_extend = base.gap_extend; a.gap_char = base.gap_char; a.gc_zero = base.gc_zero;
+    a.step_slack = base.step_slack; a.gap_open = base.gap_open; a.gap_extend = base.gap_extend; a.gap_char = base.gap_char; a.gc_zero = base.gc_zero; a.pair_form = base.pair_form;
     a.xdrop = base.xdrop; a.flen = base.flen; a.marker = base.marker;
     for (int t = 0; t < 25; ++t) a.M[t] = base.M[t];
     a.M24 = (const float *)d->m24.p; a.sim = base.sim; a.sim_off = base.sim_off;
diff --git a/twilight_amd/csrc/twl_level.inc.hip b/twilight_amd/csrc/twl_level.inc.hip
--- a/twilight_amd/csrc/twl_level.inc.hip
+++ b/twilight_amd/csrc/twl_level.inc.hip
@@ -448,12 +448,13 @@
     Device *d = call.d;
     hipStream_t st = call.st;
     LevelBufs *lv = s->lv;
-    const AlignPlan ap = plan_align(n, s->h_len, s->sides.data(), run_mask, g_leaf_step);
+    const AlignPlan ap = plan_align(n, s->h_len, s->sides.data(), run_mask, g_leaf_step, g_pair_forms, g_assert_pair_form);
     if ((rc = upload_align(lv, st, ap.lm))) return rc;
     if ((rc = size_align(lv, (size_t)n, (size_t)s->seq_len))) return rc;
     HIP_TRY(hipEventRecord(d->ev[5], st));
     rc = run_device(d, st, p, n, s->seq_len, nullptr, nullptr, nullptr, lv->d_lenmask.as<const int32_t>(), lv->d_num.as<const int32_t>(), (int8_t *)lv->d_aln.p,
-                    (int32_t *)lv->d_alnlen.p, (int16_t *)lv->d_err.p, ap.lm.data(), (const float *)lv->d_cols.p, ap.qryOneHot, zero_gap, ap.shape);
+                    (int32_t *)lv->d_alnlen.p, (int16_t *)lv->d_err.p, ap.lm.data(), (const float *)lv->d_cols.p, ap.qryOneHot, zero_gap, ap.shape,
+                    (ap.form.empty() || ap.qryOneHot) ? nullptr : ap.form.data());
     if (rc) return rc;
     return read_back_align(s, d, st, aln_out, aln_len_out, err_out);
 }
diff --git a/twilight_amd/csrc/twl_level_plan.inc.hip b/twilight_amd/csrc/twl_level_plan.inc.hip
--- a/twilight_amd/csrc/twl_level_plan.inc.hip
+++ b/twilight_amd/csrc/twl_level_plan.inc.hip
@@ -78,13 +78,23 @@
     return pp;
 }
 
+inline uint8_t pair_form_of(const twl_side &ref, const twl_side &qry, int forms, int assert_form)
+{
+    if (assert_form == 1 || assert_form == 2) return (uint8_t)assert_form;
+    auto single = [](const twl_side &sd) { return sd.n_members == 1 && sd.cache_id < 0; };
+    if ((forms & 1) && single(qry)) return 1;
+    if ((forms & 2) && single(ref)) return 2;
+    return 0;
+}
+
 struct AlignPlan {
     std::vector<int32_t> lm;
+    std::vector<uint8_t> form;
     bool qryOneHot = true;
     int shape = 0;
 };
 
-inline AlignPlan plan_align(int32_t n, const std::vector<int32_t> &h_len, const twl_side *sides, const uint8_t *run_mask, int leaf_step)
+inline AlignPlan plan_align(int32_t n, const std::vector<int32_t> &h_len, const twl_side *sides, const uint8_t *run_mask, int leaf_step, int forms = 3, int assert_form = 0)
 {
     AlignPlan ap;
     ap.lm = h_len;
@@ -105,6 +115,11 @@
         }
         ap.shape = (any && leaf) ? 2 : 0;
     }
+    bool anyForm = false;
+    ap.form.assign((size_t)n, 0);
+    for (int32_t i = 0; i < n; ++i)
+        if (runs(i)) { ap.form[i] = pair_form_of(sides[2 * (size_t)i], sides[2 * (size_t)i + 1], forms, assert_form); anyForm = anyForm || ap.form[i] != 0; }
+    if (!anyForm) ap.form.clear();
     return ap;
 }
 
diff --git a/twilight_amd/csrc/twl_run.inc.hip b/twilight_amd/csrc/twl_run.inc.hip
--- a/twilight_amd/csrc/twl_run.inc.hip
+++ b/twilight_amd/csrc/twl_run.inc.hip
@@ -54,7 +54,7 @@
     return TWL_OK;
 }
 
-int prepare_args(Call &c, const float *d_freq, const float *d_gop, const float *d_gex, int8_t *d_aln, const float *d_packed, const uint8_t *h_gc_zero)
+int prepare_args(Call &c, const float *d_freq, const float *d_gop, const float *d_gex, int8_t *d_aln, const float *d_packed, const uint8_t *h_gc_zero, const uint8_t *h_pair_form)
 {
     Device *d = c.d; hipStream_t st = c.st; const twl_params *p = c.p; const int32_t n_pairs = c.n_pairs;
     int rc;
@@ -86,6 +86,13 @@
         d->gc_zero_host.assign(h_gc_zero, h_gc_zero + n_pairs);
         HIP_TRY(hipMemcpyAsync(d->gc_zero.p, d->gc_zero_host.data(), (size_t)n_pairs, hipMemcpyHostToDevice, st));
         a.gc_zero = (const uint8_t *)d->gc_zero.p;
+    }
+    a.pair_form = nullptr;
+    if (h_pair_form && std::any_of(h_pair_form, h_pair_form + n_pairs, [](uint8_t f) { return f != 0; })) {
+        if ((rc = d->pair_form.ensure((size_t)n_pairs))) return rc;
+        d->pair_form_host.assign(h_pair_form, h_pair_form + n_pairs);
+        HIP_TRY(hipMemcpyAsync(d->pair_form.p, d->pair_form_host.data(), (size_t)n_pairs, hipMemcpyHostToDevice, st));
+        a.pair_form = (const uint8_t *)d->pair_form.p;
     }
     a.xdrop = p->xdrop; a.flen = p->flen; a.marker = p->marker;
     a.step_slack = 1 << 16;
@@ -355,7 +362,7 @@
 int run_device(Device *d, hipStream_t st, const twl_params *p, int32_t n_pairs, int32_t seq_len, const float *d_freq,
                const float *d_gop, const float *d_gex, const int32_t *d_len, const int32_t *d_num, int8_t *d_aln,
                int32_t *d_alnlen, int16_t *d_err, const int32_t *h_len, const float *d_packed = nullptr, bool qry_onehot = false,
-               const uint8_t *h_gc_zero = nullptr, int shape = 0)
+               const uint8_t *h_gc_zero = nullptr, int shape = 0, const uint8_t *h_pair_form = nullptr)
 {
     HIP_TRY(hipSetDevice(d->id));
     d->stats = twl_stats{};
@@ -373,7 +380,7 @@
     if ((rc = d->items.ensure((size_t)n_pairs * sizeof(int32_t)))) return rc;
     Call c{d, st, p, n_pairs, seq_len, d_len, d_num, d_alnlen, d_err, h_len};
     if ((rc = order_pairs(c))) return rc;
-    if ((rc = prepare_args(c, d_freq, d_gop, d_gex, d_aln, d_packed, h_gc_zero))) return rc;
+    if ((rc = prepare_args(c, d_freq, d_gop, d_gex, d_aln, d_packed, h_gc_zero, h_pair_form))) return rc;
 
     Ran ran;
     ran.prot = (p->P == 22);
```

New measurement: 227.8 billion. 0.984x the previous value.
